# jinlong17/DA-Detect

Hardware: AMD Instinct MI355X
Metric: train images/sec, DA-Faster-RCNN R-50 Cityscapes->Foggy (higher is better)
Workload: dtype f32

## Files before the change

### da_detect_amd/_C.py

```python
import contextlib
import os
import ctypes
import time

import torch

from . import _lib
from . import amax as _amax
from ._lib import ConvDesc

CL = torch.channels_last

NMS_TIE_RULE = 0

PROFILER = None
_KNAME_CACHE = {}


class KernelProfiler(object):

    def __init__(self, pool=0, only=None):
        self.only = only
        self._pool = []
        for _ in range(pool):
# ... 216 lines not shown
                "%s must be a tensor on the HIP device: the da_detect_amd operators have no CPU path" % name)
        if t.dtype != dtype:
            raise _lib.DadetError("%s must be %s, got %s" % (name, dtype, t.dtype))
    det_box, gt_box, gt_area, gt_crowd = det_box.contiguous(), gt_box.contiguous(), gt_area.contiguous(), gt_crowd.contiguous()
    n_det, n_gt = int(det_box.shape[0]), int(gt_box.shape[0])
    if det_box.numel() != 4 * n_det or gt_box.numel() != 4 * n_gt or gt_area.numel() != n_gt or gt_crowd.numel() != n_gt:
        raise _lib.DadetError("coco_match: boxes must be [n, 4], gt_area and gt_crowd [n_gt]")
    d_host, nd = _int_table(det_off)
    g_host, ng = _int_table(gt_off)
    if nd != ng or nd < 1:
        raise _lib.DadetError("coco_match: the offset tables need pairs + 1 entries each, got %d and %d" % (nd, ng))
    pairs = nd - 1
    thr_host, T = _f64_table(iou_thr)
    rng_host, A2 = _f64_table([v for lo_hi in area_rng for v in lo_hi])
    A = A2 // 2
    dev = det_box.device
    nbytes = ctypes.c_size_t(0)
    _lib.call("dadet_coco_match_workspace_bytes", d_host, g_host, pairs, n_det, n_gt, T, A, ctypes.byref(nbytes))
    ws = _workspace(nbytes.value, dev)
    matched = torch.empty((T, A, n_det), dtype=torch.uint8, device=dev)
    ignored = torch.empty((T, A, n_det), dtype=torch.uint8, device=dev)
    npig = torch.empty((pairs, A), dtype=torch.int32, device=dev)
    _lib.call("dadet_coco_match", _p(det_box), _p(gt_box), _p(gt_area), _p(gt_crowd), d_host, g_host, pairs, n_det, n_gt,
              thr_host, T, rng_host, A, _p(ws), ctypes.c_size_t(ws.numel()), _p(matched), _p(ignored), _p(npig), _stream())
    return matched, ignored, npig


def nms(dets, scores, threshold):
    if dets.numel() == 0:
        return torch.empty(0, dtype=torch.int64, device=dets.device)
    keep, count = nms_with_count(dets, scores, threshold)
    return keep[: int(count.item())]


def roi_align_forward(input, rois, spatial_scale, pooled_height, pooled_width, sampling_ratio, bin_stride=1):
    _dev(input, "input"), _dev(rois, "rois")
    B, C, H, W = input.shape
    R = rois.shape[0]
    x = _nhwc(input)
    rois = rois.contiguous()
    if bin_stride != 1:
        s = int(bin_stride)
        out = torch.empty((R, C, -(-pooled_height // s), -(-pooled_width // s)), dtype=torch.float32,
                          device=input.device, memory_format=CL)
        ws = _roi_workspace(B, H, W, R, input.device) if ROI_ALIGN_WORKSPACE else None
        _lib.call("dadet_roi_align_forward_sub", _p(x), _p(rois), _p(out), B, C, H, W, R, pooled_height, pooled_width,
                  float(spatial_scale), int(sampling_ratio), s, _p(ws) if ws is not None else None,
                  ctypes.c_size_t(ws.numel() if ws is not None else 0), _stream())
        return _amax.carry(out, input)
    out = torch.empty((R, C, pooled_height, pooled_width), dtype=torch.float32, device=input.device,
                      memory_format=CL)
    if ROI_ALIGN_WORKSPACE:
        ws = _roi_workspace(B, H, W, R, input.device)
        _lib.call("dadet_roi_align_forward_ws", _p(x), _p(rois), _p(out), B, C, H, W, R, pooled_height, pooled_width,
                  float(spatial_scale), int(sampling_ratio), _p(ws), ctypes.c_size_t(ws.numel()), _stream())
    else:
        _lib.call("dadet_roi_align_forward", _p(x), _p(rois), _p(out), B, C, H, W, R, pooled_height,
                  pooled_width, float(spatial_scale), int(sampling_ratio), _stream())
    return _amax.carry(out, input)


ROI_ALIGN_WORKSPACE = True


def _roi_workspace(B, H, W, R, device):
    nbytes = ctypes.c_size_t(0)
    _lib.call("dadet_roi_align_workspace_bytes", B, H, W, R, ctypes.byref(nbytes))
    return _workspace(nbytes.value, device)


def roi_align_backward(grad, rois, spatial_scale, pooled_height, pooled_width, batch_size, channels,
                       height, width, sampling_ratio, atomic=False, bin_stride=1, live_images=None):
    _dev(grad, "grad"), _dev(rois, "rois")
    g = _nhwc(grad)
    rois = rois.contiguous()
    gin = torch.empty((batch_size, channels, height, width), dtype=torch.float32, device=grad.device,
                      memory_format=CL)
    B = batch_size
    if live_images is not None and 0 < live_images < batch_size and not atomic and rois.shape[0] > 0:
        B = int(live_images)
        gin[B:].zero_()
    if bin_stride != 1:
        if atomic:
            raise ValueError("roi_align_backward: bin_stride needs the gather form")
        _lib.call("dadet_roi_align_backward_sub", _p(g), _p(rois), _p(gin), B, channels, height, width,
                  rois.shape[0], pooled_height, pooled_width, float(spatial_scale), int(sampling_ratio),
                  int(bin_stride), _stream())
        return gin
    batch_size = B
    if atomic:
        gin.zero_()
    _lib.call("dadet_roi_align_backward_atomic" if atomic else "dadet_roi_align_backward", _p(g), _p(rois),
              _p(gin), batch_size, channels, height, width, rois.shape[0], pooled_height, pooled_width,
              float(spatial_scale), int(sampling_ratio), _stream())
    return gin


def roi_align_forward_level(input, rois, levels, level, out, spatial_scale, pooled_height, pooled_width, sampling_ratio):
    _dev(input, "input"), _dev(rois, "rois")
    assert levels.is_cuda and levels.dtype == torch.int64 and levels.is_contiguous() and levels.numel() == rois.shape[0]
    assert out.is_contiguous(memory_format=CL) and out.shape[0] == rois.shape[0]
    B, C, H, W = input.shape
    x = _nhwc(input)
    rois = rois.contiguous()
    ws = _roi_workspace(B, H, W, rois.shape[0], input.device)
    _lib.call("dadet_roi_align_forward_level", _p(x), _p(rois), _p(levels), int(level), _p(out), B, C, H, W, rois.shape[0],
              pooled_height, pooled_width, float(spatial_scale), int(sampling_ratio), _p(ws), ctypes.c_size_t(ws.numel()),
              _stream())
    return out


def roi_align_backward_level(grad, rois, levels, level, spatial_scale, pooled_height, pooled_width, batch_size, channels,
                             height, width, sampling_ratio):
    _dev(grad, "grad"), _dev(rois, "rois")
    assert levels.is_cuda and levels.dtype == torch.int64 and levels.is_contiguous() and levels.numel() == rois.shape[0]
    g = _nhwc(grad)
    gin = torch.empty((batch_size, channels, height, width), dtype=torch.float32, device=grad.device, memory_format=CL)
    _lib.call("dadet_roi_align_backward_level", _p(g), _p(rois.contiguous()), _p(levels), int(level), _p(gin), batch_size,
              channels, height, width, rois.shape[0], pooled_height, pooled_width, float(spatial_scale), int(sampling_ratio),
              _stream())
    return gin


def sigmoid_focalloss_forward(logits, targets, num_classes, gamma, alpha):
    _dev(logits, "logits")
    logits = logits.contiguous()
    targets = targets.contiguous().to(torch.int32)
    out = torch.empty_like(logits)
    _lib.call("dadet_sigmoid_focal_loss_forward", _p(logits), _p(targets), _p(out), logits.shape[0],
              int(num_classes), float(gamma), float(alpha), _stream())
    return out


def sigmoid_focalloss_backward(logits, targets, d_losses, num_classes, gamma, alpha):
    _dev(logits, "logits")
    logits = logits.contiguous()
    targets = targets.contiguous().to(torch.int32)
    d_losses = d_losses.contiguous()
    out = torch.empty_like(logits)
    _lib.call("dadet_sigmoid_focal_loss_backward", _p(logits), _p(targets), _p(d_losses), _p(out),
              logits.shape[0], int(num_classes), float(gamma), float(alpha), _stream())
    return out


def _desc(N, H, W, Cin, Cout, KH, KW, stride, pad, Ho, Wo, OutH=None, OutW=None, os=1, relu_mode=0):
    return ConvDesc(N, H, W, Cin, Cout, KH, KW, stride, pad, Ho, Wo, Ho if OutH is None else OutH,
                    Wo if OutW is None else OutW, os, relu_mode)


def conv_out_size(H, W, KH, KW, stride, pad):
    return (H + 2 * pad - KH) // stride + 1, (W + 2 * pad - KW) // stride + 1


def conv_forward(x, w, scale=None, bias=None, addend=None, mask_ref=None, stride=1, pad=0, relu_mode=0,
                 out=None, out_spatial_stride=1, out_hw=None, out_size=None):
    _dev(x, "x"), _dev(w, "w")
    N, Cin, H, W = x.shape
    Cout, Cin_w, KH, KW = w.shape
    assert Cin == Cin_w, "conv_forward: channel mismatch %d vs %d" % (Cin, Cin_w)
    x = _nhwc(x)
    w = _nhwc(w)
    Ho, Wo = out_size if out_size is not None else conv_out_size(H, W, KH, KW, stride, pad)
    if out_spatial_stride > 1:
        OutH, OutW = out_hw
        if out is None:
            out = torch.empty((N, Cout, OutH, OutW), dtype=torch.float32, device=x.device,
                              memory_format=CL).zero_()
    else:
        OutH, OutW = Ho, Wo
        if out is None:
            out = torch.empty((N, Cout, Ho, Wo), dtype=torch.float32, device=x.device, memory_format=CL)
    if addend is not None:
        addend = _nhwc(addend) if addend is not out else addend
    if mask_ref is not None:
        mask_ref = _nhwc(mask_ref)
    d = _desc(N, H, W, Cin, Cout, KH, KW, stride, pad, Ho, Wo, OutH, OutW, out_spatial_stride, relu_mode)
    ax = aw = None
    if _mode4():
        ax, aw = _amax.ptr(x), _weight_amax(w)
    if PROFILER is not None:
        key = (N * Ho * Wo, Cout, Cin * KH * KW, KH, pad, out_spatial_stride)
        kname = _KNAME_CACHE.get(key)
        if kname is None:
            kname = _plan_name("dadet_conv_forward_plan", d)
            _KNAME_CACHE[key] = kname
        if getattr(PROFILER, "detail", False):
            side = x.is_cuda and torch.cuda.current_stream(x.device) != torch.cuda.default_stream(x.device)
            kname = "%s|M=%d N=%d K=%d k%dx%d s%d%s%s" % (kname, N * Ho * Wo, Cout, Cin * KH * KW, KH, KW, stride,
                                                          " +add" if addend is not None else "", " [side]" if side else "")
        x_read = N * Ho * Wo * Cin if (KH == 1 and KW == 1 and stride > 1) else x.numel()
        with PROFILER.span(kname,
                           2.0 * N * Ho * Wo * Cout * Cin * KH * KW,
                           4.0 * (x_read + w.numel() + out.numel() + (addend.numel() if addend is not None else 0)
                                  + (mask_ref.numel() if mask_ref is not None else 0))):
            _conv_forward_call(d, x, w, scale, bias, addend, mask_ref, out, ax, aw)
        return out
    _conv_forward_call(d, x, w, scale, bias, addend, mask_ref, out, ax, aw)
    return out


def _conv_forward_call(d, x, w, scale, bias, addend, mask_ref, out, ax, aw):
    if ax is None:
        _lib.call("dadet_conv_forward", ctypes.byref(d), _p(x), _p(w), _p(scale), _p(bias), _p(addend),
                  _p(mask_ref), _p(out), _stream())
        return
    slot = _amax.new_slot(out.device)
    _lib.call("dadet_conv_forward_scaled", ctypes.byref(d), _p(x), _p(w), _p(scale), _p(bias), _p(addend),
              _p(mask_ref), _p(out), ax, aw, ctypes.c_void_p(slot[0]), _stream())
    _amax.attach(out, slot)


def _transpose_now(w, scale, wt):
    Cout, Cin, KH, KW = w.shape
    cout_pad = wt.shape[1]
    _lib.call("dadet_conv_weight_transpose_padded", _p(w), _p(scale), _p(wt), Cout, KH, KW, Cin, cout_pad, _stream())
    return wt


class _TransposeCache(object):

    def __init__(self):
        self.entries = {}
        self.epoch = 0
        self.batched_epoch = -1
        self.table = None
        self.ready = None
        self.enabled = True
        self._from_bump = False
        self._trained_only = False

    def bump(self, device=None, trained_only=False):
        self.epoch += 1
        self._trained_only = bool(trained_only)
        if self.enabled and device is not None and self.entries:
            self._from_bump = True
            try:
                self._refresh_all(device)
            finally:
                self._from_bump = False
        elif device is not None and _mode4():
            _amax.WEIGHTS.refresh(device, self.epoch, trained_only=self._trained_only)
        self._trained_only = False

    def _single(self, e, w, scale):
        _transpose_now(w, scale, e["wt"])
        _amax.WEIGHTS.invalidate(e["wt"])
        e["epoch"] = self.epoch
        if w.is_cuda:
            st = torch.cuda.current_stream(w.device)
            e["ev"] = (st, st.record_event())
        return e["wt"]

    def get(self, w, scale, cout_pad=0):
        Cout, Cin, KH, KW = w.shape
        key = (w.data_ptr(), Cout, Cin, KH, KW, scale.data_ptr() if scale is not None else 0, w.device.index, cout_pad)
        e = self.entries.get(key)
        if e is None:
            wt = torch.empty((Cin, max(Cout, cout_pad), KH, KW), dtype=torch.float32, device=w.device, memory_format=CL)
            wt._dadet_persistent = True
            e = self.entries[key] = dict(w=w, scale=scale, wt=wt, version=w._version, epoch=self.epoch, used=self.epoch,
                                         ev=None)
            self.table = None
            return self._single(e, w, scale)
        e["used"] = self.epoch
        if e["version"] != w._version:
            e["w"], e["version"] = w, w._version
            return self._single(e, w, scale)
        if e["epoch"] != self.epoch:
            if self.batched_epoch != self.epoch:
                self._refresh_all(w.device)
            if e["epoch"] != self.epoch:
                return self._single(e, w, scale)
        src = e["ev"] if e["ev"] is not None else self.ready
        if src is not None and w.is_cuda and torch.cuda.current_stream(w.device) != src[0]:
            torch.cuda.current_stream(w.device).wait_event(src[1])
        return e["wt"]

    def _refresh_all(self, device):
        for k in [k for k, e in self.entries.items() if e["used"] < self.epoch - 2]:
            del self.entries[k]
        live = [(k, e) for k, e in self.entries.items() if k[6] == device.index and e["version"] == e["w"]._version]
        if not live:
            self.batched_epoch = self.epoch
            return
        if self.table is None or self.table[3] != [k for k, _ in live]:
            arr = (_lib.TransposeItem * len(live))()
            blocks = 0
            for i, (k, e) in enumerate(live):
                _, Cout, Cin, KH, KW, _, _, cout_pad = k
                it = arr[i]
                it.w, it.scale, it.wt = e["w"].data_ptr(), (e["scale"].data_ptr() if e["scale"] is not None else None), \
                    e["wt"].data_ptr()
                it.Cout, it.KH, it.KW, it.Cin = Cout, KH, KW, Cin
                it.cout_pad = cout_pad
                it.blocks_ci, it.blocks_co = (Cin + 31) // 32, (max(Cout, cout_pad) + 31) // 32
                it.first_block = blocks
                blocks += it.blocks_ci * it.blocks_co * KH * KW
            host = torch.frombuffer(bytearray(bytes(arr)), dtype=torch.uint8).clone()
            self.table = (host.to(device), len(live), blocks, [k for k, _ in live])
        dev_t, n, blocks, _ = self.table
        _lib.call("dadet_conv_weight_transpose_batch", _p(dev_t), n, blocks, _stream())
        for _, e in live:
            e["epoch"] = self.epoch
            e["ev"] = None
        self.batched_epoch = self.epoch
        if _mode4():
            _amax.WEIGHTS.refresh(device, self.epoch, sync=not self._from_bump,
                                  trained_only=self._from_bump and self._trained_only)
        if device.type == "cuda":
            st = torch.cuda.current_stream(device)
            self.ready = (st, st.record_event())


_TRANSPOSES = _TransposeCache()


def weight_epoch():
    return _TRANSPOSES.epoch


def bump_weight_epoch(device=None, trained_only=False):
    _TRANSPOSES.bump(device, trained_only)


def conv_weight_transpose(w, scale=None, cout_pad=0):
    _dev(w, "w")
    Cout, Cin, KH, KW = w.shape
    cout_pad = cout_pad if cout_pad > Cout else 0
    w = _nhwc(w)
    base = w._base if w._base is not None else w
    if _TRANSPOSES.enabled and base.is_leaf and base.requires_grad:
        return _TRANSPOSES.get(w, scale, cout_pad)
    wt = torch.empty((Cin, max(Cout, cout_pad), KH, KW), dtype=torch.float32, device=w.device, memory_format=CL)
    return _transpose_now(w, scale, wt)


class WgradBatch(list):
    """weight gradients whose reduction pass over the split partial results is still to come
    (conv_wgrad(..., pending=batch) ... conv_wgrad_reduce_batch(batch)); keeps their workspaces alive until then"""


def _plan_name(query, d, *args):
    info = _lib.ConvPlanInfo()
    _lib.call(query, ctypes.byref(d), *(args + (ctypes.byref(info),)))
    return info.name.decode()


def _wgrad_kname(d, gy_ld):
    return _plan_name("dadet_conv_wgrad_plan", d, int(gy_ld))


def conv_wgrad_reduce_batch(batch):
    if not batch:
        return
    arr = (_lib.WgradPending * len(batch))(*[item[0] for item in batch])
    _lib.call("dadet_conv_wgrad_reduce_batch", arr, len(batch), _stream())
    del batch[:]


WGRAD_GROUP_MAX = 4


def conv_wgrad_group(requests, pending):
    n = len(requests)
    if not (1 <= n <= WGRAD_GROUP_MAX) or not _mode4() or pending is None:
        return False
    descs = (_lib.ConvDesc * n)()
    xs, gys = [], []
    for i, r in enumerate(requests):
        x, gy = _nhwc(_dev(r["x"], "x")), _nhwc(_dev(r["gy"], "gy"))
        N, Cin, H, W = x.shape
        Cout, Cin_w, KH, KW = r["weight_shape"]
        if Cin != Cin_w or gy.shape[1] != Cout or r["dw"] is None:
            return False
        descs[i] = _desc(N, H, W, Cin, Cout, KH, KW, r.get("stride", 1), r.get("pad", 0), gy.shape[2], gy.shape[3])
        xs.append(x)
        gys.append(gy)
    splits = (ctypes.c_int * n)()
    nbytes = (ctypes.c_size_t * n)()
    kind = _lib.load().dadet_conv_wgrad_group_plan(descs, n, splits, nbytes)
    if not kind:
        return False
    wss = [torch.empty(max(int(b), 16), dtype=torch.uint8, device=xs[0].device) for b in nbytes]
    vp = ctypes.c_void_p * n

    def ptrs(ts):
        return vp(*[(t.data_ptr() if t is not None else None) for t in ts])

    items = (_lib.WgradPending * n)()
    ax = vp(*[_amax.ptr(t).value for t in xs])
    ag = vp(*[_amax.ptr(t).value for t in gys])
    acc = (ctypes.c_int * n)(*[1 if r.get("accumulate", False) else 0 for r in requests])
    sizes = (ctypes.c_size_t * n)(*[w.numel() for w in wss])

    def launch():
        _lib.call("dadet_conv_wgrad_group", descs, n, ptrs(xs), ptrs(gys), ptrs([r.get("out_scale") for r in requests]),
                  ptrs([r["dw"] for r in requests]), acc, ptrs(wss), sizes, items, ax, ag, _stream())

    if PROFILER is not None:
        flops = sum(2.0 * d.N * d.Ho * d.Wo * d.Cout * d.Cin * d.KH * d.KW for d in descs)
        nbytes_alg = sum(4.0 * (x.numel() + g.numel() + r["dw"].numel()) for x, g, r in zip(xs, gys, requests))
        kname = "conv_wgrad_big_group_kernel" if kind == 256 else "conv_wgrad_split_group_kernel"
        if getattr(PROFILER, "detail", False):
            kname += "|" + " + ".join("M=%d N=%d K=%d k%dx%d s%d" % (d.N * d.Ho * d.Wo, d.Cout, d.Cin * d.KH * d.KW, d.KH,
                                                                     d.KW, d.stride) for d in descs)
        with PROFILER.span(kname, flops, nbytes_alg):
            launch()
    else:
        launch()
    for i, r in enumerate(requests):
        if items[i].splits > 1:
            it = _lib.WgradPending()
            ctypes.memmove(ctypes.byref(it), ctypes.byref(items[i]), ctypes.sizeof(it))
            pending.append((it, wss[i], r["dw"], r.get("out_scale")))
    return True


def conv_wgrad(x, gy, weight_shape, stride=1, pad=0, out_scale=None, dw=None, accumulate=False, pending=None):
    _dev(x, "x"), _dev(gy, "gy")
    N, Cin, H, W = x.shape
    Cout, Cin_w, KH, KW = weight_shape
    assert Cin == Cin_w
    x = _nhwc(x)
    gy = _nhwc(gy)
    Ho, Wo = gy.shape[2], gy.shape[3]
    gy_ld = gy.shape[1]
    if gy_ld != Cout and pending is None:
        own = WgradBatch()
        dw = conv_wgrad(x, gy, weight_shape, stride, pad, out_scale, dw, accumulate, pending=own)
        conv_wgrad_reduce_batch(own)
        return dw
    if dw is None:
        dw = torch.empty((Cout, Cin, KH, KW), dtype=torch.float32, device=x.device, memory_format=CL)
        accumulate = False
    d = _desc(N, H, W, Cin, Cout, KH, KW, stride, pad, Ho, Wo)
    nbytes = ctypes.c_size_t(0)
    _lib.call("dadet_conv_wgrad_workspace_bytes", ctypes.byref(d), ctypes.byref(nbytes))
    m4 = _mode4()
    if m4:
        ax, ag = _amax.ptr(x), _amax.ptr(gy)
    if pending is not None:
        ws = torch.empty(max(nbytes.value, 16), dtype=torch.uint8, device=x.device)
        item = _lib.WgradPending()

        def launch():
            if m4:
                _lib.call("dadet_conv_wgrad_scaled", ctypes.byref(d), _p(x), _p(gy), gy_ld, _p(out_scale), _p(dw),
                          1 if accumulate else 0, _p(ws), ctypes.c_size_t(ws.numel()), ctypes.byref(item), ax, ag,
                          _stream())
                return
            _lib.call("dadet_conv_wgrad_partials_ld", ctypes.byref(d), _p(x), _p(gy), gy_ld, _p(out_scale), _p(dw),
                      1 if accumulate else 0, _p(ws), ctypes.c_size_t(ws.numel()), ctypes.byref(item), _stream())

        if PROFILER is not None:
            kname = _wgrad_kname(d, gy_ld)
            if getattr(PROFILER, "detail", False):
                kname = "%s|M=%d N=%d K=%d k%dx%d s%d" % (kname, N * Ho * Wo, Cout, Cin * KH * KW, KH, KW, stride)
            with PROFILER.span(kname, 2.0 * N * Ho * Wo * Cout * Cin * KH * KW,
                               4.0 * (x.numel() + gy.numel() + dw.numel())):
                launch()
        else:
            launch()
        if item.splits > 1:
            pending.append((item, ws, dw, out_scale))
        return dw
    ws = _workspace(nbytes.value, x.device)
    if PROFILER is not None:
        kname = _wgrad_kname(d, gy_ld)
        if getattr(PROFILER, "detail", False):
            kname = "%s|M=%d N=%d K=%d k%dx%d s%d" % (kname, N * Ho * Wo, Cout, Cin * KH * KW, KH, KW, stride)
        with PROFILER.span(kname,
                           2.0 * N * Ho * Wo * Cout * Cin * KH * KW,
                           4.0 * (x.numel() + gy.numel() + dw.numel())):
            _wgrad_call(d, x, gy, gy_ld, out_scale, dw, accumulate, ws, ax if m4 else None, ag if m4 else None)
        return dw
    _wgrad_call(d, x, gy, gy_ld, out_scale, dw, accumulate, ws, ax if m4 else None, ag if m4 else None)
    return dw


def _wgrad_call(d, x, gy, gy_ld, out_scale, dw, accumulate, ws, ax, ag):
    if ax is not None:
        _lib.call("dadet_conv_wgrad_scaled", ctypes.byref(d), _p(x), _p(gy), gy_ld, _p(out_scale), _p(dw),
                  1 if accumulate else 0, _p(ws), ctypes.c_size_t(ws.numel()), None, ax, ag, _stream())
        return
    _lib.call("dadet_conv_wgrad", ctypes.byref(d), _p(x), _p(gy), _p(out_scale), _p(dw),
              1 if accumulate else 0, _p(ws), ctypes.c_size_t(ws.numel()), _stream())


def relu_bn_backward(g, y=None, scale=None, want_unscaled=False):
    _dev(g, "g")
    g = _nhwc(g) if g.dim() == 4 else g.contiguous()
    C = g.shape[1]
    rows = g.numel() // C
    yy = None
    if y is not None:
        yy = _nhwc(y) if y.dim() == 4 else y.contiguous()
    g_out = torch.empty_like(g) if want_unscaled else None
    g_scaled = torch.empty_like(g)
    if not _mode4():
        _lib.call("dadet_relu_bn_backward", _p(g), _p(yy), _p(scale), _p(g_out), _p(g_scaled), rows, C, _stream())
        return g_out, g_scaled
    so = ss = None
    if g_out is not None and _amax.slot_of(_amax.carry(g_out, g)) is None:
        so = _amax.new_slot(g.device)
    if scale is not None or _amax.slot_of(_amax.carry(g_scaled, g)) is None:
        ss = _amax.new_slot(g.device)
    _lib.call("dadet_relu_bn_backward_m", _p(g), _p(yy), _p(scale), _p(g_out), _p(g_scaled), rows, C,
              ctypes.c_void_p(so[0]) if so else None, ctypes.c_void_p(ss[0]) if ss else None, _stream())
    if so:
        _amax.attach(g_out, so)
    if ss:
        _amax.attach(g_scaled, ss)
    return g_out, g_scaled


def colsum(g, out=None, accumulate=False, cols=None):
    _dev(g, "g")
    g = _nhwc(g) if g.dim() == 4 else g.contiguous()
    ld = g.shape[1]
    C = ld if cols is None else int(cols)
    rows = g.numel() // ld
    if out is None:
        out = torch.empty(C, dtype=torch.float32, device=g.device)
        accumulate = False
    assert out.numel() == C and out.is_contiguous() and out.dtype == torch.float32
    nbytes = ctypes.c_size_t(0)
    _lib.call("dadet_colsum_workspace_bytes", rows, C, ctypes.byref(nbytes))
    ws = _workspace(nbytes.value, g.device)
    _lib.call("dadet_colsum_ld", _p(g), ld, _p(out), rows, C, 1 if accumulate else 0, _p(ws), ctypes.c_size_t(ws.numel()),
              _stream())
    return out


def channel_affine(x, scale, bias, relu=False):
    _dev(x, "x")
    x = _nhwc(x)
    C = x.shape[1]
    y = torch.empty_like(x)
    _lib.call("dadet_channel_affine", _p(x), _p(scale), _p(bias), _p(y), x.numel() // C, C,
              1 if relu else 0, _stream())
    return y


def maxpool3x3s2(x):
    _dev(x, "x")
    x = _nhwc(x)
    N, C, H, W = x.shape
    Ho, Wo = (H + 2 - 3) // 2 + 1, (W + 2 - 3) // 2 + 1
    y = torch.empty((N, C, Ho, Wo), dtype=torch.float32, device=x.device, memory_format=CL)
    _lib.call("dadet_maxpool3x3s2_forward", _p(x), _p(y), N, H, W, C, Ho, Wo, _stream())
    return _amax.carry(y, x)


def maxpool3x3s2_relu_backward(y, gp, scale=None):
    _dev(y, "y"), _dev(gp, "gp")
    y, gp = _nhwc(y), _nhwc(gp)
    N, C, H, W = y.shape
    Ho, Wo = (H + 2 - 3) // 2 + 1, (W + 2 - 3) // 2 + 1
    assert tuple(gp.shape) == (N, C, Ho, Wo), "maxpool3x3s2_relu_backward: gp %s for y %s" % (tuple(gp.shape), tuple(y.shape))
    g = torch.empty((N, C, H, W), dtype=torch.float32, device=y.device, memory_format=CL)
    slot = _amax.new_slot(y.device) if _mode4() else None
    _lib.call("dadet_maxpool3x3s2_relu_backward", _p(y), _p(gp), _p(scale), _p(g), N, H, W, C, Ho, Wo,
              ctypes.c_void_p(slot[0]) if slot else None, _stream())
    if slot:
        _amax.attach(g, slot)
    return g


def avgpool_forward(x):
    _dev(x, "x")
    x = _nhwc(x)
    R, C, h, w = x.shape
    y = torch.empty((R, C), dtype=torch.float32, device=x.device)
    _lib.call("dadet_avgpool_forward", _p(x), _p(y), R, h * w, C, _stream())
    return _amax.carry(y, x)


def avgpool_backward(gy, h, w):
    _dev(gy, "gy")
    gy = gy.contiguous()
    R, C = gy.shape
    gx = torch.empty((R, C, h, w), dtype=torch.float32, device=gy.device, memory_format=CL)
    _lib.call("dadet_avgpool_backward", _p(gy), _p(gx), R, h * w, C, _stream())
    return _amax.carry(gx, gy)


def nchw3_to_nhwc4(x):
    _dev(x, "x")
    x = x.contiguous()
    N, C, H, W = x.shape
    assert C == 3
    y = torch.empty((N, 4, H, W), dtype=torch.float32, device=x.device, memory_format=CL)
    _lib.call("dadet_nchw3_to_nhwc4", _p(x), _p(y), N, H, W, _stream())
    if _mode4():
        _amax.ptr(x)
        _amax.carry(y, x)
    return y


def two_image_ends(r_cst, n_src):
    return min(max(int(n_src), 0), int(r_cst)), int(r_cst)


def da_ins_tail_forward(h, w3, b3, labels, means, r_bce, r_cst, n_src):
    return da_ins_tail_forward_n(h, w3, b3, labels, means, r_bce, r_cst, two_image_ends(r_cst, n_src))


def da_ins_tail_backward(h, w3, logits, labels, means, coef, inv_keep, r_bce, r_cst, n_src):
    return da_ins_tail_backward_n(h, w3, logits, labels, means, coef, inv_keep, r_bce, r_cst, two_image_ends(r_cst, n_src))


def _row_ends(row_end):
    ends = [int(e) for e in row_end]
    return (ctypes.c_int * len(ends))(*ends), len(ends)


def da_ins_tail_forward_n(h, w3, b3, labels, means, r_bce, r_cst, row_end):
    _dev(h, "h")
    rows, C = h.shape
    assert rows == r_bce + r_cst
    L = int(means.shape[0]) if means is not None else 0
    ends, n_img = _row_ends(row_end)
    assert means is None or means.shape[1] == n_img
    logits = torch.empty(rows, dtype=torch.float32, device=h.device)
    sums = torch.zeros(2, dtype=torch.float32, device=h.device)
    _lib.call("dadet_da_ins_tail_forward_n", _p(h), _p(w3), _p(b3), _p(labels), _p(means), _p(logits), _p(sums),
              int(r_bce), int(r_cst), ends, n_img, L, C, _stream())
    return logits, sums


def da_ins_tail_backward_n(h, w3, logits, labels, means, coef, inv_keep, r_bce, r_cst, row_end):
    rows, C = h.shape
    L = int(means.shape[0]) if means is not None else 0
    ends, n_img = _row_ends(row_end)
    assert means is None or means.shape[1] == n_img
    g_z = torch.empty_like(h)
    acc = torch.zeros(C + 1 + n_img * L, dtype=torch.float32, device=h.device)
    g_w3, g_b3 = acc[:C], acc[C:C + 1]
    g_means = acc[C + 1:].view(L, n_img) if L else None
    _lib.call("dadet_da_ins_tail_backward_n", _p(h), _p(w3), _p(logits), _p(labels), _p(means), _p(coef), float(inv_keep),
              _p(g_z), _p(g_w3), _p(g_b3), _p(g_means), int(r_bce), int(r_cst), ends, n_img, L, C, _stream())
    return g_z, g_w3, g_b3, g_means


def da_ins_dropout_rows(h1, masks):
    P = masks.shape[0]
    out = torch.empty((P * h1.shape[0], h1.shape[1]), dtype=torch.float32, device=h1.device)
    _lib.call("dadet_da_ins_dropout_rows", _p(h1), _p(masks), _p(out), ctypes.c_int64(h1.numel()), int(P), _stream())
    return out


def da_ins_merge(g, masks, h1, grl, need_x=True):
    P = masks.shape[0]
    g_w = torch.empty_like(h1)
    g_x = torch.empty_like(h1) if need_x else None
    _lib.call("dadet_da_ins_merge", _p(g), _p(masks), _p(h1), _p(grl), _p(g_w), _p(g_x), ctypes.c_int64(h1.numel()),
              int(P), _stream())
    return g_w, g_x


# ... 614 lines not shown
```

### da_detect_amd/_lib.py

```python
import ctypes
import os
from ctypes import POINTER, c_char_p, c_float, c_int, c_int64, c_size_t, c_uint64, c_void_p

_HERE = os.path.dirname(os.path.abspath(__file__))
LIB_PATH = os.environ.get("DADET_LIB") or os.path.join(_HERE, "libdadet_hip.so")
_lib = None
DEFAULT_GEMM_MODE = "4"


class ConvDesc(ctypes.Structure):

    _fields_ = [(n, c_int) for n in (
        "N", "H", "W", "Cin", "Cout", "KH", "KW", "stride", "pad", "Ho", "Wo", "OutH", "OutW",
        "out_spatial_stride", "relu_mode")]


class ConvPlanInfo(ctypes.Structure):

    _fields_ = [(n, c_int) for n in (
        "family", "variant", "tiles_m", "tiles_n", "ksplit", "splits", "rows_per_split", "sk_dp_tiles", "sk_tiles", "sk_units",
        "sk_iters", "sk_max_parts", "big_splits", "big_body", "launches", "grid", "needs_counters")] + [
        ("workspace_bytes", c_size_t), ("name", ctypes.c_char * 64)]


class WgradPending(ctypes.Structure):

    _fields_ = [("partials", c_void_p), ("out_scale", c_void_p), ("dw", c_void_p), ("count", ctypes.c_longlong),
                ("K", c_int), ("splits", c_int), ("accumulate", c_int)]


class TransposeItem(ctypes.Structure):
    _fields_ = [("w", c_void_p), ("scale", c_void_p), ("wt", c_void_p), ("Cout", c_int), ("KH", c_int), ("KW", c_int),
                ("Cin", c_int), ("first_block", c_int), ("blocks_ci", c_int), ("blocks_co", c_int), ("cout_pad", c_int)]


class AmaxItem(ctypes.Structure):

    _fields_ = [("x", c_void_p), ("slot", c_void_p), ("n", ctypes.c_longlong), ("first_block", c_int), ("blocks", c_int)]


class MergeEntry(ctypes.Structure):

    _fields_ = [("boxes", c_void_p), ("scores", c_void_p), ("keep", c_void_p), ("count", c_void_p), ("boxes_out", c_void_p),
                ("scores_out", c_void_p), ("n", c_int), ("cap", c_int)]


class TopkRow(ctypes.Structure):

    _fields_ = [("scores", c_void_p), ("out_scores", c_void_p), ("out_idx", c_void_p), ("n", c_int), ("k", c_int)]


class SgdEntry(ctypes.Structure):

    _fields_ = [("p", c_void_p), ("g", c_void_p), ("buf", c_void_p), ("numel", c_int64),
                ("lr", c_float), ("weight_decay", c_float)]


_P = c_void_p
_SIGNATURES = {
    "dadet_version": [],
    "dadet_device_info": [POINTER(c_int), POINTER(c_int), POINTER(c_size_t), c_char_p, c_int],
    "dadet_nms_workspace_bytes": [c_int, POINTER(c_size_t)],
    "dadet_nms": [_P, _P, c_int, c_float, c_int, c_int, _P, c_size_t, _P, _P, _P],
    "dadet_nms_batch_workspace_bytes": [c_int, c_int, POINTER(c_size_t)],
    "dadet_nms_batch": [_P, POINTER(c_int), c_int, c_int, c_float, c_int, c_int, _P, c_size_t, _P, _P, _P],
    "dadet_detect_post_workspace_bytes": [POINTER(c_int), c_int, c_int, POINTER(c_size_t)],
    "dadet_detect_post": [_P, _P, POINTER(c_int), c_int, c_int, c_float, c_float, c_int, c_int, c_int, _P, c_size_t, _P, _P, _P,
                          _P, _P],
    "dadet_coco_match_workspace_bytes": [POINTER(c_int), POINTER(c_int), c_int, c_int, c_int, c_int, c_int, POINTER(c_size_t)],
    "dadet_coco_match": [_P, _P, _P, _P, POINTER(c_int), POINTER(c_int), c_int, c_int, c_int, POINTER(ctypes.c_double), c_int,
                         POINTER(ctypes.c_double), c_int, _P, c_size_t, _P, _P, _P, _P],
    "dadet_roi_align_forward": [_P, _P, _P, c_int, c_int, c_int, c_int, c_int, c_int, c_int, c_float, c_int, _P],
    "dadet_roi_align_backward": [_P, _P, _P, c_int, c_int, c_int, c_int, c_int, c_int, c_int, c_float, c_int, _P],
    "dadet_roi_align_workspace_bytes": [c_int, c_int, c_int, c_int, POINTER(c_size_t)],
    "dadet_roi_align_forward_ws": [_P, _P, _P, c_int, c_int, c_int, c_int, c_int, c_int, c_int, c_float, c_int, _P, c_size_t, _P],
    "dadet_roi_align_backward_atomic": [_P, _P, _P, c_int, c_int, c_int, c_int, c_int, c_int, c_int, c_float, c_int, _P],
    "dadet_roi_align_forward_sub": [_P, _P, _P, c_int, c_int, c_int, c_int, c_int, c_int, c_int, c_float, c_int, c_int,
                                    _P, c_size_t, _P],
    "dadet_roi_align_forward_level": [_P, _P, _P, c_int, _P, c_int, c_int, c_int, c_int, c_int, c_int, c_int, c_float, c_int, _P,
                                      c_size_t, _P],
    "dadet_roi_align_backward_level": [_P, _P, _P, c_int, _P, c_int, c_int, c_int, c_int, c_int, c_int, c_int, c_float, c_int,
                                       _P],
    "dadet_roi_align_backward_sub": [_P, _P, _P, c_int, c_int, c_int, c_int, c_int, c_int, c_int, c_float, c_int, c_int,
                                     _P],
    "dadet_sigmoid_focal_loss_forward": [_P, _P, _P, c_int, c_int, c_float, c_float, _P],
    "dadet_sigmoid_focal_loss_backward": [_P, _P, _P, _P, c_int, c_int, c_float, c_float, _P],
    "dadet_conv_forward": [POINTER(ConvDesc), _P, _P, _P, _P, _P, _P, _P, _P],
    "dadet_conv_forward_scaled": [POINTER(ConvDesc), _P, _P, _P, _P, _P, _P, _P, _P, _P, _P, _P],
    "dadet_conv_wgrad_scaled": [POINTER(ConvDesc), _P, _P, c_int, _P, _P, c_int, _P, c_size_t, POINTER(WgradPending), _P, _P,
                                _P],
    "dadet_amax": [_P, ctypes.c_longlong, _P, _P],
    "dadet_amax_batch": [_P, c_int, c_int, _P],
    "dadet_conv_forward_variant": [POINTER(ConvDesc)],
    "dadet_conv_forward_plan": [POINTER(ConvDesc), POINTER(ConvPlanInfo)],
    "dadet_conv_wgrad_plan": [POINTER(ConvDesc), c_int, POINTER(ConvPlanInfo)],
    "dadet_set_gemm_mode": [c_int],
    "dadet_get_gemm_mode": [],
    "dadet_conv_wgrad_variant": [POINTER(ConvDesc)],
    "dadet_conv_wgrad_group_plan": [POINTER(ConvDesc), c_int, POINTER(c_int), POINTER(c_size_t)],
    "dadet_conv_wgrad_group": [POINTER(ConvDesc), c_int, POINTER(c_void_p), POINTER(c_void_p), POINTER(c_void_p),
                               POINTER(c_void_p), POINTER(c_int), POINTER(c_void_p), POINTER(c_size_t),
                               POINTER(WgradPending), POINTER(c_void_p), POINTER(c_void_p), _P],
    "dadet_nonfinite_poll": [c_char_p, c_int],
    "dadet_set_big_gemm": [c_int],
    "dadet_get_big_gemm": [],
    "dadet_conv_wgrad_workspace_bytes": [POINTER(ConvDesc), POINTER(c_size_t)],
    "dadet_conv_wgrad": [POINTER(ConvDesc), _P, _P, _P, _P, c_int, _P, c_size_t, _P],
    "dadet_conv_wgrad_partials": [POINTER(ConvDesc), _P, _P, _P, _P, c_int, _P, c_size_t, POINTER(WgradPending), _P],
    "dadet_conv_wgrad_reduce_batch": [POINTER(WgradPending), c_int, _P],
    "dadet_conv_weight_transpose": [_P, _P, _P, c_int, c_int, c_int, c_int, _P],
    "dadet_conv_weight_transpose_padded": [_P, _P, _P, c_int, c_int, c_int, c_int, c_int, _P],
    "dadet_conv_wgrad_partials_ld": [POINTER(ConvDesc), _P, _P, c_int, _P, _P, c_int, _P, c_size_t, POINTER(WgradPending),
                                     _P],
    "dadet_conv_weight_transpose_batch": [_P, c_int, c_int, _P],
    "dadet_deform_sample_forward": [_P, _P, _P, _P] + [c_int] * 12 + [_P],
    "dadet_deform_sample_backward": [_P, _P, _P, _P, _P, _P, _P] + [c_int] * 12 + [_P],
    "dadet_deform_sample_forward_ld": [_P, _P, c_int, _P, c_int, c_int, _P] + [c_int] * 12 + [_P],
    "dadet_deform_sample_backward_ld": [_P, _P, c_int, _P, c_int, c_int, _P, _P, _P, c_int, _P, c_int] + [c_int] * 12
                                       + [_P, c_size_t, _P],
    "dadet_deform_sample_backward_ld_m": [_P, _P, c_int, _P, c_int, c_int, _P, _P, _P, c_int, _P, c_int] + [c_int] * 12
                                         + [_P, c_size_t, _P, ctypes.c_longlong, _P],
    "dadet_deform_sample_backward_workspace_bytes": [c_int, c_int, c_int, c_int, POINTER(c_size_t)],
    "dadet_image_resample_h": [_P, c_int, c_int, _P, _P, c_int, c_int, _P, _P],
    "dadet_image_resample_v_normalize": [_P, c_int, c_int, _P, _P, c_int, c_int, c_int, c_int, POINTER(c_float),
                                         POINTER(c_float), _P, c_int, _P],
    "dadet_rpn_loss": [_P, _P, _P, _P, c_int, _P, _P, c_int, c_float, _P, _P, _P, _P],
    "dadet_fpn_merge_levels": [POINTER(MergeEntry), c_int, _P],
    "dadet_rpn_loss_rows": [_P, _P, _P, _P, c_int, c_int, _P, c_int, c_float, _P, _P, c_int, _P, _P],
    "dadet_rpn_loss_rows_level": [_P, _P, _P, _P, c_int, c_int, _P, c_int, c_float, ctypes.c_longlong, ctypes.c_longlong,
                                  ctypes.c_longlong, c_int, _P, c_int, _P, _P, c_int, _P, _P],
    "dadet_gather_pixel_taps_level": [_P, _P, _P, c_int, c_int, c_int, c_int, c_int, c_int, c_int, c_int, c_int, _P, _P],
    "dadet_scatter_pixel_taps_add_level": [_P, _P, _P, c_int, c_int, c_int, c_int, c_int, c_int, c_int, c_int, c_int, _P,
                                           _P],
    "dadet_gather_pixel_taps": [_P, _P, c_int, c_int, c_int, c_int, c_int, c_int, c_int, c_int, _P, _P],
    "dadet_scatter_pixel_taps_add": [_P, _P, c_int, c_int, c_int, c_int, c_int, c_int, c_int, c_int, _P, _P],
    "dadet_fast_rcnn_loss": [_P, _P, c_int, c_int, _P, _P, c_int, _P, _P, _P, c_int, _P, _P, _P, _P],
    "dadet_fast_rcnn_loss_rows": [_P, _P, c_int, c_int, c_int, _P, _P, _P, _P, _P, _P],
    "dadet_sample_rois": [_P, _P, _P, c_int, c_int, c_int, c_uint64, c_int, _P, _P, _P, _P, _P, _P, _P, _P],
    "dadet_proposals_sample": [_P, _P, _P, _P, c_int, _P, c_int, _P, _P, c_int, c_float, c_float, c_float, c_float, c_float,
                               c_float, c_int, c_int, c_uint64, c_int, _P, _P, _P, _P, _P, _P, _P, _P, _P, _P, _P, _P],
    "dadet_sample_anchors": [_P, _P, c_int, c_int, c_int, c_uint64, c_int64, _P, _P, _P, _P, _P],
    "dadet_topk_sorted": [_P, c_int, c_int, c_int64, c_int, _P, _P, _P],
    "dadet_topk_sorted_rows_workspace_bytes": [c_int, c_int, POINTER(c_size_t)],
    "dadet_topk_sorted_rows": [POINTER(TopkRow), c_int, _P, c_size_t, _P],
    "dadet_rpn_anchor_targets": [_P, _P, c_int, _P, c_int, c_float, c_float, _P, _P, _P, _P],
    "dadet_box_match_encode": [_P, c_int, _P, _P, c_int, c_float, c_float, c_float, c_float, c_float, c_float, _P, _P,
                               _P, _P],
    "dadet_roi_pool_forward": [_P, _P, _P, _P, c_int, c_int, c_int, c_int, c_int, c_int, c_int, c_float, _P],
    "dadet_roi_pool_backward": [_P, _P, _P, _P, c_int, c_int, c_int, c_int, c_int, c_int, c_int, _P],
    "dadet_deform_psroi_pool_forward": [_P, _P, _P, _P, _P, c_int, c_int, c_int, c_int, c_int, c_int, c_float,
                                        c_int, c_int, c_int, c_int, c_int, c_float, c_int, _P],
    "dadet_deform_psroi_pool_backward": [_P, _P, _P, _P, _P, _P, _P, c_int, c_int, c_int, c_int, c_int, c_int,
                                         c_float, c_int, c_int, c_int, c_int, c_int, c_float, c_int, _P],
    "dadet_relu_bn_backward": [_P, _P, _P, _P, _P, c_int64, c_int, _P],
    "dadet_relu_bn_backward_m": [_P, _P, _P, _P, _P, c_int64, c_int, _P, _P, _P],
    "dadet_colsum_workspace_bytes": [c_int64, c_int, POINTER(c_size_t)],
    "dadet_colsum": [_P, _P, c_int64, c_int, _P, c_size_t, _P],
    "dadet_colsum_ld": [_P, c_int, _P, c_int64, c_int, c_int, _P, c_size_t, _P],
    "dadet_channel_affine": [_P, _P, _P, _P, c_int64, c_int, c_int, _P],
    "dadet_maxpool3x3s2_forward": [_P, _P, c_int, c_int, c_int, c_int, c_int, c_int, _P],
    "dadet_maxpool3x3s2_relu_backward": [_P, _P, _P, _P, c_int, c_int, c_int, c_int, c_int, c_int, _P, _P],
    "dadet_avgpool_forward": [_P, _P, c_int, c_int, c_int, _P],
    "dadet_avgpool_backward": [_P, _P, c_int, c_int, c_int, _P],
    "dadet_nchw3_to_nhwc4": [_P, _P, c_int, c_int, c_int, _P],
    "dadet_rpn_decode_clip": [_P, _P, _P, c_int, c_float, c_float, c_float, c_float, c_float, c_float, c_float, _P, _P],
    "dadet_da_img_head_loss_forward": [_P, _P, _P, _P, _P, _P, c_int, c_int, c_int, _P],
    "dadet_da_img_head_loss_backward": [_P, _P, _P, _P, _P, _P, _P, _P, _P, c_int, c_int, c_int, _P],
    "dadet_da_img_head_loss_backward_g": [_P, _P, _P, _P, _P, _P, _P, c_float, c_float, _P, _P, _P, _P, c_int, c_int, c_int,
                                          _P],
    "dadet_da_img_head_loss_backward_gm": [_P, _P, _P, _P, _P, _P, _P, c_float, c_float, _P, _P, _P, _P, c_int, c_int, c_int,
                                          _P, _P, _P],
    "dadet_da_ins_tail_forward": [_P, _P, _P, _P, _P, _P, _P, c_int, c_int, c_int, c_int, c_int, _P],
    "dadet_da_ins_tail_backward": [_P, _P, _P, _P, _P, _P, c_float, _P, _P, _P, _P, c_int, c_int, c_int, c_int, c_int, _P],
    "dadet_da_ins_tail_forward_n": [_P, _P, _P, _P, _P, _P, _P, c_int, c_int, POINTER(c_int), c_int, c_int, c_int, _P],
    "dadet_da_ins_tail_backward_n": [_P, _P, _P, _P, _P, _P, c_float, _P, _P, _P, _P, c_int, c_int, POINTER(c_int), c_int,
                                     c_int, c_int, _P],
    "dadet_da_ins_dropout_rows": [_P, _P, _P, c_int64, c_int, _P],
    "dadet_da_ins_merge": [_P, _P, _P, _P, _P, _P, c_int64, c_int, _P],
    "dadet_triplet_w_forward": [_P, _P, _P, c_int, c_int, c_int, c_float, c_float, _P, _P, _P],
    "dadet_triplet_w_backward": [_P, _P, _P, _P, _P, c_int, c_int, c_int, c_float, c_float, _P, _P, _P, _P],
    "dadet_sgd_step": [_P, c_int, c_int64, c_float, c_int, c_float, _P],
}
_RESTYPES = {"dadet_last_error": c_char_p}
EXPORTED_SYMBOLS = sorted(list(_SIGNATURES) + ["dadet_last_error"])


class DadetError(RuntimeError):
    pass


def load():
    global _lib
    if _lib is not None:
        return _lib
    if not os.path.exists(LIB_PATH):
        raise DadetError(
            "libdadet_hip.so is not built (%s). Run `python -c 'import __graft_entry__ as g; g.build()'` "
            "or `make -C da_detect_amd/csrc`. There is no CPU fallback for the product path." % LIB_PATH)
    import torch

    lib = ctypes.CDLL(LIB_PATH)
    for name, argtypes in _SIGNATURES.items():
        fn = getattr(lib, name)
        fn.argtypes = argtypes
        fn.restype = c_int
    lib.dadet_last_error.argtypes = []
    lib.dadet_last_error.restype = c_char_p
    _lib = lib
    mode = int(os.environ.get("DADET_GEMM_MODE", DEFAULT_GEMM_MODE))
    if lib.dadet_set_gemm_mode(mode) != 0:
        raise DadetError("DADET_GEMM_MODE=%d is not a valid contraction mode (0, 2, 3 or 4)" % mode)
    return lib


def check(rc, what=""):
    if rc != 0:
        msg = load().dadet_last_error()
        raise DadetError("%s failed (status %d): %s" % (what or "dadet call", rc, (msg or b"").decode()))


def call(name, *args):
    check(getattr(load(), name)(*args), name)
```

### da_detect_amd/csrc/conv_common.h

```cpp
#pragma once
#include <cstdlib>
#include "common.h"
#include "conv_plan.h"

namespace dadet {

typedef float f32x16 __attribute__((ext_vector_type(16)));
typedef unsigned int u32x4 __attribute__((ext_vector_type(4)));

constexpr unsigned kOOB = 0xFFFFFFF0u;
__device__ inline __amdgpu_buffer_rsrc_t make_rsrc(const void* p, unsigned bytes) {
  return __builtin_amdgcn_make_buffer_rsrc(const_cast<void*>(p), 0, (int)bytes, 0x00020000);
}
__device__ inline float4 buf_load4(__amdgpu_buffer_rsrc_t r, unsigned byte_off) {
  return __builtin_bit_cast(float4, __builtin_amdgcn_raw_buffer_load_b128(r, (int)byte_off, 0, 0));
}
__device__ inline float buf_load1(__amdgpu_buffer_rsrc_t r, unsigned byte_off) {
  return __builtin_bit_cast(float, __builtin_amdgcn_raw_buffer_load_b32(r, (int)byte_off, 0, 0));
}
__device__ inline void buf_store1(__amdgpu_buffer_rsrc_t r, unsigned byte_off, float v) {
  __builtin_amdgcn_raw_buffer_store_b32(__builtin_bit_cast(unsigned, v), r, (int)byte_off, 0, 0);
}

__device__ inline void buf_store4_wt(__amdgpu_buffer_rsrc_t r, unsigned byte_off, float4 v) {
  __builtin_amdgcn_raw_buffer_store_b128(__builtin_bit_cast(u32x4, v), r, (int)byte_off, 0, 16);
}
__device__ inline float4 buf_load4_sc1(__amdgpu_buffer_rsrc_t r, unsigned byte_off) {
  return __builtin_bit_cast(float4, __builtin_amdgcn_raw_buffer_load_b128(r, (int)byte_off, 0, 16));
}

typedef __bf16 bf16x8 __attribute__((ext_vector_type(8)));


__device__ inline unsigned pack_bf16(float lo, float hi) {
  unsigned r;
  asm("v_cvt_pk_bf16_f32 %0, %1, %2" : "=v"(r) : "v"(lo), "v"(hi));
  return r;
}
__device__ inline float lo_as_float(unsigned p) { return __builtin_bit_cast(float, p << 16); }
__device__ inline float hi_as_float(unsigned p) { return __builtin_bit_cast(float, p & 0xFFFF0000u); }

template <int TERMS>
__device__ inline void split4(const float4 v, uint2 (&out)[TERMS]) {
  float a = v.x, b = v.y, c = v.z, d = v.w;
#pragma unroll
  for (int t = 0; t < TERMS; ++t) {
    const unsigned p0 = pack_bf16(a, b), p1 = pack_bf16(c, d);
    out[t] = make_uint2(p0, p1);
    if (t + 1 < TERMS) {
      a -= lo_as_float(p0); b -= hi_as_float(p0);
      c -= lo_as_float(p1); d -= hi_as_float(p1);
    }
  }
}

typedef _Float16 f16x8 __attribute__((ext_vector_type(8)));
typedef _Float16 f16x2 __attribute__((ext_vector_type(2)));

__device__ inline int fmt4_exp(const float amax) {
  const int be = (int)((__builtin_bit_cast(unsigned, amax) >> 23) & 0xffu);
  if (be == 0 || be == 255) return 0;
  int e = 14 - (be - 127);
  return e > 126 ? 126 : (e < -126 ? -126 : e);
}
__device__ inline float pow2f(const int e) { return __builtin_bit_cast(float, (unsigned)(e + 127) << 23); }

__device__ inline unsigned pack_f16(float lo, float hi) {
  unsigned r;
  asm("v_cvt_pk_f16_f32 %0, %1, %2" : "=v"(r) : "v"(lo), "v"(hi));
  return r;
}
__device__ inline float resid_lo(float x, float s, unsigned h) {
  float r;
  asm("v_fma_mix_f32 %0, %1, %2, -%3 op_sel_hi:[0,0,1]" : "=v"(r) : "v"(x), "v"(s), "v"(h));
  return r;
}
__device__ inline float resid_hi(float x, float s, unsigned h) {
  float r;
  asm("v_fma_mix_f32 %0, %1, %2, -%3 op_sel:[0,0,1] op_sel_hi:[0,0,1]" : "=v"(r) : "v"(x), "v"(s), "v"(h));
  return r;
}
__device__ inline void split4h(const float4 v, const float s, uint2 (&out)[2]) {
  const unsigned h0 = pack_f16(v.x * s, v.y * s), h1 = pack_f16(v.z * s, v.w * s);
  out[0] = make_uint2(h0, h1);
  out[1] = make_uint2(pack_f16(resid_lo(v.x, s, h0), resid_hi(v.y, s, h0)),
                      pack_f16(resid_lo(v.z, s, h1), resid_hi(v.w, s, h1)));
}

template <int FMT> struct Fmt { static constexpr int terms = FMT == 3 ? 3 : 2; static constexpr bool f16 = FMT == 4; };

template <bool F16>
__device__ __forceinline__ f32x16 mfma_32x32x16(const bf16x8 a, const bf16x8 b, const f32x16 c) {
  if constexpr (F16)
    return __builtin_amdgcn_mfma_f32_32x32x16_f16(__builtin_bit_cast(f16x8, a), __builtin_bit_cast(f16x8, b), c, 0, 0, 0);
  else
    return __builtin_amdgcn_mfma_f32_32x32x16_bf16(a, b, c, 0, 0, 0);
}

constexpr int kAmaxStride = DADET_AMAX_STRIDE;
__device__ inline float amax_read(const float* slot) {
  float m = slot[0];
#pragma unroll
  for (int s = 1; s < 8; ++s) m = fmaxf(m, slot[s * kAmaxStride]);
  return m;
}
__device__ inline void amax_publish(unsigned* slot, float m) {
  __shared__ unsigned s_amax;
  unsigned* shard = slot + (size_t)((blockIdx.x + blockIdx.y) & 7) * kAmaxStride;
  unsigned seen = 0;
  if (threadIdx.x == 0) {
    s_amax = 0;
    seen = __hip_atomic_load(shard, __ATOMIC_RELAXED, __HIP_MEMORY_SCOPE_AGENT);
  }
#pragma unroll
  for (int o = 32; o; o >>= 1) m = fmaxf(m, __shfl_xor(m, o));
  __syncthreads();
  if ((threadIdx.x & 63) == 0) atomicMax(&s_amax, __builtin_bit_cast(unsigned, m));
  __syncthreads();
  if (threadIdx.x == 0) {
    const unsigned b = s_amax;
    if (b > seen) __hip_atomic_fetch_max(shard, b, __ATOMIC_RELAXED, __HIP_MEMORY_SCOPE_AGENT);
  }
}

template <int TM, int TN>
__device__ __forceinline__ void nf_check(const f32x16 (&acc)[TM][TN], unsigned* flag, const unsigned id) {
  if (!flag) return;
  bool bad = false;
#pragma unroll
  for (int i = 0; i < TM; ++i)
#pragma unroll
    for (int j = 0; j < TN; ++j)
#pragma unroll
      for (int e = 0; e < 16; ++e)
        bad |= (__builtin_bit_cast(unsigned, acc[i][j][e]) & 0x7f800000u) == 0x7f800000u;
  if (__builtin_amdgcn_ballot_w64(bad) != 0 && (threadIdx.x & 63) == 0) {
    atomicCAS(flag, 0u, id + 1u);
    atomicAdd(flag + 1, 1u);
  }
}
unsigned nf_next_launch(const char* kind, int M, int N, int K, int KH);
unsigned* nf_flag_ptr();

constexpr int PLANE_STRIDE = 40;
constexpr int EPI_STRIDE = 40;

constexpr int BK = plan::kBK;
constexpr int LDS_STRIDE = 36;

struct ConvArgs {
  const float* x;
  const float* w;
  const float* scale;
  const float* bias;
  const float* addend;
  const float* mask_ref;
  float* y;
  int N, H, W, Cin, Cout, KH, KW, stride, pad, Ho, Wo, OutH, OutW, os, relu_mode;
  int M, K;
  int tiles_m, tiles_n;
  unsigned x_bytes, w_bytes, y_bytes;
  int ablate;
  int ws_panel0;
  int epi_v4;
  int ksplit;
  unsigned split_stride;
  int sk_dp_tiles, sk_tiles, sk_units, sk_iters, sk_max_parts;
  float* sk_ws;
  int* sk_counters;
  int big_splits;
  int big_asym;
  int big_body;
  unsigned* nf_flag;
  unsigned launch_id;
  const float* amax_x;
  const float* amax_w;
  unsigned* amax_y;
};

struct WgradArgs {
  const float* x;
  const float* gy;
  const float* out_scale;
  float* out;
  int N, H, W, Cin, Cout, KH, KW, stride, pad, Ho, Wo;
  int M, K;
  int gy_ld;
  int tiles_co, tiles_kc, splits, rows_per_split;
  int direct;
  int accumulate;
  unsigned x_bytes, gy_bytes;
  const float* amax_x;
  const float* amax_gy;
  unsigned* nf_flag;
  unsigned launch_id;
};

constexpr int kWgradGroupMax = plan::kGroupMax;
struct WgradGroup {
  WgradArgs a[kWgradGroupMax];
  int first[kWgradGroupMax + 1];
  int n;
};

static_assert(plan::kCUs == kNumCU, "the plan layer's CU count");

int gemm_mode();

int launch_fwd_exact(ConvArgs& a, const plan::FwdPlan& p, hipStream_t st);
int launch_wgrad_exact(WgradArgs& a, hipStream_t st);
int launch_fwd_split(ConvArgs& a, const plan::FwdPlan& p, int fmt, hipStream_t st);
int launch_fwd_split_sk(ConvArgs& a, int fmt, hipStream_t st);
int launch_wgrad_split(WgradArgs& a, bool small_map, int fmt, hipStream_t st);
int launch_wgrad_split_group(const WgradArgs* a, int n, bool small_map, hipStream_t st);
int launch_fwd_ws(ConvArgs& a, const plan::FwdPlan& p, int fmt, hipStream_t st);
int launch_fwd_big(ConvArgs& a, const plan::FwdPlan& p, hipStream_t st);
int launch_wgrad_big(WgradArgs& a, hipStream_t st);
int launch_wgrad_big_group(const WgradArgs* a, int n, hipStream_t st);

void* stream_scratch(hipStream_t st, size_t bytes);
int* stream_counters(hipStream_t st);
unsigned* stream_amax_slots(hipStream_t st);
hipError_t zero_slots(unsigned* first, int n, hipStream_t st);
int launch_amax(const float* x, int64_t n, unsigned* slot, hipStream_t st);
int launch_splitk_reduce(const float* partial, int splits, const ConvArgs& a, hipStream_t st);
int launch_wgrad_reduce(const float* partials, const float* out_scale, float* dw, int Cout, int K, int splits,
                        int accumulate, hipStream_t st);

}
```

### da_detect_amd/csrc/conv_dispatch.hip

```cpp
#include "conv_common.h"

namespace dadet {

static int g_gemm_mode = 4;
static int g_big_mode = plan::big_gemm_default();
int gemm_mode() { return g_gemm_mode; }

static int conv_desc_check(const dadet_conv_desc* d, const char* who) {
  DADET_REQUIRE(d, "%s: null descriptor", who);
  DADET_REQUIRE(d->N >= 0 && d->H > 0 && d->W > 0 && d->Cin > 0 && d->Cout > 0 && d->KH > 0 && d->KW > 0 &&
                    d->stride > 0 && d->pad >= 0 && d->Ho > 0 && d->Wo > 0,
                "%s: bad dims", who);
  DADET_REQUIRE(d->Cin % 4 == 0, "%s: Cin=%d must be a multiple of 4 (pad the channel axis)", who, d->Cin);
  DADET_REQUIRE((int64_t)d->N * d->H * d->W * d->Cin < (1LL << 31) &&
                    (int64_t)d->N * d->Ho * d->Wo < (1LL << 31),
                "%s: tensor too large for 32-bit pixel indexing", who);
  return DADET_OK;
}

static int extents_check(uint64_t a, uint64_t b, uint64_t c, const char* who) {
  DADET_REQUIRE(a < 0xFFFFFFF0ull && b < 0xFFFFFFF0ull && c < 0xFFFFFFF0ull,
                "%s: tensors of 4 GB or more are not addressable through one buffer descriptor", who);
  return DADET_OK;
}

static bool al16(const void* p) { return (reinterpret_cast<uintptr_t>(p) & 15) == 0; }

static void fill_conv_args(const dadet_conv_desc* d, const plan::Gemm& g, const plan::FwdPlan& p, ConvArgs* a) {
  *a = ConvArgs();
  a->N = d->N; a->H = d->H; a->W = d->W; a->Cin = d->Cin; a->Cout = d->Cout; a->KH = d->KH; a->KW = d->KW;
  a->stride = d->stride; a->pad = d->pad; a->Ho = d->Ho; a->Wo = d->Wo; a->OutH = d->OutH; a->OutW = d->OutW;
  a->os = g.os; a->relu_mode = d->relu_mode;
  a->M = g.M; a->K = g.K;
  a->x_bytes = (unsigned)g.x_bytes; a->w_bytes = (unsigned)g.w_bytes; a->y_bytes = (unsigned)g.y_bytes;
  a->ablate = plan::ablate();
  a->epi_v4 = p.epi_v4;
  a->tiles_m = p.tiles_m; a->tiles_n = p.tiles_n;
  a->sk_dp_tiles = p.sk.dp_tiles; a->sk_tiles = p.sk.sk_tiles; a->sk_units = p.sk.units; a->sk_iters = p.sk.iters;
  a->sk_max_parts = p.sk.max_parts;
  a->big_splits = p.big_splits; a->big_body = p.big_body;
}

static void fill_wgrad_args(const dadet_conv_desc* d, int gy_ld, int tiles_co, int tiles_kc, int splits, int rows,
                            WgradArgs* a) {
  *a = WgradArgs();
  const plan::Gemm g = plan::gemm_of(d);
  a->gy_ld = gy_ld;
  a->N = d->N; a->H = d->H; a->W = d->W; a->Cin = d->Cin; a->Cout = d->Cout; a->KH = d->KH; a->KW = d->KW;
  a->stride = d->stride; a->pad = d->pad; a->Ho = d->Ho; a->Wo = d->Wo;
  a->M = g.M; a->K = g.K;
  a->x_bytes = (unsigned)g.x_bytes; a->gy_bytes = (unsigned)((uint64_t)g.M * gy_ld * 4);
  a->tiles_co = tiles_co; a->tiles_kc = tiles_kc; a->splits = splits; a->rows_per_split = rows;
}

static void fill_pending(dadet_wgrad_pending* p, const void* workspace, const float* out_scale, float* dw, int Cout, int K,
                         int splits, int accumulate) {
  p->partials = static_cast<const float*>(workspace);
  p->out_scale = out_scale;
  p->dw = dw;
  p->count = (long long)Cout * K;
  p->K = K;
  p->splits = splits;
  p->accumulate = accumulate;
}

static int conv_forward_impl(const dadet_conv_desc* d, const float* x, const float* w,
                             const float* scale, const float* bias, const float* addend,
                             const float* mask_ref, float* y, const float* amax_x, const float* amax_w,
                             float* amax_y, void* stream) {
  int rc = conv_desc_check(d, "conv_forward");
  if (rc) return rc;
  if (d->N == 0) return DADET_OK;
  DADET_REQUIRE(x && w && y && al16(x) && al16(w), "conv_forward: x / w must be non-null and 16-byte aligned");
  DADET_REQUIRE(d->relu_mode >= 0 && d->relu_mode <= 2, "conv_forward: relu_mode");
  DADET_REQUIRE(d->relu_mode != 2 || mask_ref, "conv_forward: relu_mode 2 needs mask_ref");
  const plan::Gemm g = plan::gemm_of(d);
  DADET_REQUIRE(g.os == 1 ? (d->OutH == d->Ho && d->OutW == d->Wo)
                          : ((d->Ho - 1) * g.os < d->OutH && (d->Wo - 1) * g.os < d->OutW),
                "conv_forward: OutH/OutW inconsistent with Ho/Wo and out_spatial_stride");
  rc = extents_check(g.x_bytes, g.w_bytes, g.y_bytes, "conv_forward");
  if (rc) return rc;
  const int mode = g_gemm_mode;
  const bool aligned16 = al16(y) && (!addend || al16(addend)) && (!mask_ref || al16(mask_ref)) && (!scale || al16(scale)) &&
                         (!bias || al16(bias));
  const plan::FwdPlan p = plan::plan_forward(d, aligned16, mode, g_big_mode);
  ConvArgs a;
  fill_conv_args(d, g, p, &a);
  a.x = x; a.w = w; a.scale = scale; a.bias = bias; a.addend = addend; a.mask_ref = mask_ref; a.y = y;
  hipStream_t st = as_stream(stream);
  if (mode == 4) {
    if (!amax_x || !amax_w) {
      unsigned* own = stream_amax_slots(st);
      if (!own) { set_error("conv_forward: could not allocate the operand-maximum slots"); return DADET_ELAUNCH; }
      if (zero_slots(own, 2, st) != hipSuccess) return check_launch("conv_forward(amax memset)");
      if (!amax_x) {
        rc = launch_amax(x, (int64_t)(g.x_bytes / 4), own, st);
        if (rc) return rc;
        amax_x = reinterpret_cast<const float*>(own);
      }
      if (!amax_w) {
        rc = launch_amax(w, (int64_t)(g.w_bytes / 4), own + 1, st);
        if (rc) return rc;
        amax_w = reinterpret_cast<const float*>(own + 1);
      }
    }
    a.amax_x = amax_x; a.amax_w = amax_w;
    a.amax_y = reinterpret_cast<unsigned*>(amax_y);
    a.nf_flag = nf_flag_ptr();
    a.launch_id = a.nf_flag ? nf_next_launch("conv_forward", a.M, a.Cout, a.K, a.KH) : 0;
  }
  float* ws = p.workspace_bytes ? static_cast<float*>(stream_scratch(st, p.workspace_bytes)) : nullptr;
  int* counters = p.counters ? stream_counters(st) : nullptr;
  if ((p.workspace_bytes && !ws) || (p.counters && !counters)) {
    set_error("conv_forward: could not allocate %zu bytes of %s scratch", p.workspace_bytes,
              p.family == plan::kFwdSplitSk ? "stream-K" : p.family == plan::kFwdSplitK ? "split-K" : "split-reduction");
    return DADET_ELAUNCH;
  }
  switch (p.family) {
    case plan::kFwdWs: return launch_fwd_ws(a, p, mode, st);
    case plan::kFwdBig256:
    case plan::kFwdBig128:
      a.sk_ws = ws;
      a.sk_counters = counters;
      return launch_fwd_big(a, p, st);
    case plan::kFwdSplitSk:
      a.sk_ws = ws;
      a.sk_counters = counters;
      return launch_fwd_split_sk(a, mode, st);
    case plan::kFwdSplitK: {
      ConvArgs part = a;
      part.scale = part.bias = part.addend = part.mask_ref = nullptr;
      part.amax_y = nullptr;
      part.relu_mode = 0;
      part.y = ws;
      part.ksplit = p.ksplit;
      part.split_stride = (unsigned)((size_t)a.M * a.Cout);
      rc = launch_fwd_split(part, p, mode, st);
      return rc ? rc : launch_splitk_reduce(ws, p.splits, a, st);
    }
    case plan::kFwdSplit: return launch_fwd_split(a, p, mode, st);
    default: return launch_fwd_exact(a, p, st);
  }
}

static int conv_wgrad_impl(const dadet_conv_desc* d, const float* x, const float* gy, const float* out_scale, float* dw,
                           int accumulate, void* workspace, size_t workspace_bytes, dadet_wgrad_pending* pending,
                           void* stream, int gy_ld = 0, const float* amax_x = nullptr, const float* amax_gy = nullptr) {
  if (pending) pending->splits = 0;
  int rc = conv_desc_check(d, "conv_wgrad");
  if (rc) return rc;
  DADET_REQUIRE(dw, "conv_wgrad: null dw");
  hipStream_t st = as_stream(stream);
  const int K = d->KH * d->KW * d->Cin;
  if (d->N == 0) {
    if (!accumulate) (void)hipMemsetAsync(dw, 0, sizeof(float) * (size_t)d->Cout * K, st);
    return check_launch("conv_wgrad(empty)");
  }
  DADET_REQUIRE(x && gy && al16(x) && al16(gy) && al16(dw), "conv_wgrad: pointers must be 16-byte aligned");
  if (gy_ld == 0) gy_ld = d->Cout;
  DADET_REQUIRE(gy_ld % 4 == 0 && gy_ld >= d->Cout && gy_ld - d->Cout < 4,
                "conv_wgrad: gy rows of %d floats for Cout=%d (need a multiple of 4, less than 4 above Cout)", gy_ld, d->Cout);
  DADET_REQUIRE(K % 4 == 0, "conv_wgrad: KH*KW*Cin=%d must be a multiple of 4", K);
  const plan::Gemm g = plan::gemm_of(d);
  const uint64_t gb = (uint64_t)g.M * gy_ld * 4;
  rc = extents_check(g.x_bytes, gb, 0, "conv_wgrad");
  if (rc) return rc;
  const int mode = g_gemm_mode;
  const plan::WgradPlan p = plan::plan_wgrad(d, gy_ld, mode, g_big_mode);
  WgradArgs a;
  fill_wgrad_args(d, gy_ld, p.tiles_co, p.tiles_kc, p.splits, p.rows_per_split, &a);
  a.x = x; a.gy = gy; a.out_scale = out_scale;
  a.accumulate = accumulate;
  if (mode == 4) {
    if (!amax_x || !amax_gy) {
      unsigned* own = stream_amax_slots(st);
      if (!own) { set_error("conv_wgrad: could not allocate the operand-maximum slots"); return DADET_ELAUNCH; }
      if (zero_slots(own + 2, 2, st) != hipSuccess) return check_launch("conv_wgrad(amax memset)");
      if (!amax_x) {
        rc = launch_amax(x, (int64_t)(g.x_bytes / 4), own + 2, st);
        if (rc) return rc;
        amax_x = reinterpret_cast<const float*>(own + 2);
      }
      if (!amax_gy) {
        rc = launch_amax(gy, (int64_t)(gb / 4), own + 3, st);
        if (rc) return rc;
        amax_gy = reinterpret_cast<const float*>(own + 3);
      }
    }
    a.amax_x = amax_x; a.amax_gy = amax_gy;
    a.nf_flag = nf_flag_ptr();
    a.launch_id = a.nf_flag ? nf_next_launch("conv_wgrad", a.M, a.Cout, a.K, a.KH) : 0;
  }
  if (p.splits == 1) {
    a.direct = 1;
    a.out = dw;
  } else {
    if (!workspace || workspace_bytes < p.workspace_bytes) {
      set_error("conv_wgrad: workspace %zu < required %zu", workspace_bytes, p.workspace_bytes);
      return DADET_EWORKSPACE;
    }
    a.direct = 0;
    a.out = static_cast<float*>(workspace);
  }
  switch (p.family) {
    case plan::kWgradBig: rc = launch_wgrad_big(a, st); break;
    case plan::kWgradExact: rc = launch_wgrad_exact(a, st); break;
    default: rc = launch_wgrad_split(a, p.family == plan::kWgradSplitSmallMap, mode, st);
  }
  if (rc || p.splits == 1) return rc;
  if (pending) {
    fill_pending(pending, workspace, out_scale, dw, d->Cout, K, p.splits, accumulate);
    return DADET_OK;
  }
  return launch_wgrad_reduce(static_cast<const float*>(workspace), out_scale, dw, d->Cout, K, p.splits, accumulate, st);
}

static bool group_descs_ok(const dadet_conv_desc* descs, int n) {
  if (n < 1 || n > kWgradGroupMax) return false;
  for (int i = 0; i < n; ++i)
    if (conv_desc_check(&descs[i], "conv_wgrad_group") || descs[i].N == 0) return false;
  return true;
}

}

using namespace dadet;

extern "C" int dadet_set_gemm_mode(int mode) {
  if (mode != 0 && mode != 2 && mode != 3 && mode != 4) {
    set_error("set_gemm_mode: mode must be 0, 2, 3 or 4");
    return DADET_EINVAL;
  }
  g_gemm_mode = mode;
  return DADET_OK;
}
extern "C" int dadet_get_gemm_mode(void) { return g_gemm_mode; }

extern "C" int dadet_set_big_gemm(int mode) {
  if (mode < 0 || mode > 2) {
    set_error("set_big_gemm: mode must be 0 (off), 1 (planned) or 2 (wherever applicable)");
    return DADET_EINVAL;
  }
  g_big_mode = mode;
  return DADET_OK;
}
extern "C" int dadet_get_big_gemm(void) { return g_big_mode; }

extern "C" int dadet_conv_forward(const dadet_conv_desc* d, const float* x, const float* w,
                                  const float* scale, const float* bias, const float* addend,
                                  const float* mask_ref, float* y, void* stream) {
  return conv_forward_impl(d, x, w, scale, bias, addend, mask_ref, y, nullptr, nullptr, nullptr, stream);
}

extern "C" int dadet_conv_forward_scaled(const dadet_conv_desc* d, const float* x, const float* w,
                                         const float* scale, const float* bias, const float* addend,
                                         const float* mask_ref, float* y, const float* amax_x, const float* amax_w,
                                         float* amax_y, void* stream) {
  return conv_forward_impl(d, x, w, scale, bias, addend, mask_ref, y, amax_x, amax_w, amax_y, stream);
}

extern "C" int dadet_conv_forward_plan(const dadet_conv_desc* d, dadet_conv_plan_info* out) {
  int rc = conv_desc_check(d, "conv_forward_plan");
  if (rc) return rc;
  DADET_REQUIRE(out, "conv_forward_plan: null out");
  const plan::Gemm g = plan::gemm_of(d);
  rc = extents_check(g.x_bytes, g.w_bytes, g.y_bytes, "conv_forward_plan");
  if (rc) return rc;
  const plan::FwdPlan p = plan::plan_forward(d, true, g_gemm_mode, g_big_mode);
  plan::fill_info(p, out);
  if (!p.epi_v4 && g.os == 1 && d->Cout % 4 == 0) {
    const plan::FwdPlan label = plan::plan_forward_epi(d, true, true, g_gemm_mode, g_big_mode);
    out->variant = label.variant;
    snprintf(out->name, sizeof(out->name), "%s", label.name);
  }
  return DADET_OK;
}

extern "C" int dadet_conv_forward_variant(const dadet_conv_desc* d) {
  if (!d) return -1;
  const int os = d->out_spatial_stride > 0 ? d->out_spatial_stride : 1;
  return plan::fwd_label(d, plan::gemm_of(d), os == 1 && d->Cout % 4 == 0, g_gemm_mode, g_big_mode);
}

extern "C" int dadet_conv_wgrad_plan(const dadet_conv_desc* d, int gy_ld, dadet_conv_plan_info* out) {
  int rc = conv_desc_check(d, "conv_wgrad_plan");
  if (rc) return rc;
  DADET_REQUIRE(out, "conv_wgrad_plan: null out");
  plan::fill_info(plan::plan_wgrad(d, gy_ld ? gy_ld : d->Cout, g_gemm_mode, g_big_mode), out);
  return DADET_OK;
}

extern "C" int dadet_conv_wgrad_variant(const dadet_conv_desc* d) {
  if (!d) return -1;
  return plan::plan_wgrad(d, d->Cout, g_gemm_mode, g_big_mode).family == plan::kWgradBig ? 1 : 0;
}

extern "C" int dadet_conv_wgrad_workspace_bytes(const dadet_conv_desc* d, size_t* bytes_out) {
  int rc = conv_desc_check(d, "conv_wgrad_workspace_bytes");
  if (rc) return rc;
  DADET_REQUIRE(bytes_out, "conv_wgrad_workspace_bytes: null out");
  if (d->N == 0) { *bytes_out = 0; return DADET_OK; }
  const plan::WgradPlan dense = plan::plan_wgrad(d, d->Cout, g_gemm_mode, g_big_mode);
  *bytes_out = dense.workspace_bytes;
  if (dense.family == plan::kWgradBig) {
    const size_t padded = plan::plan_wgrad(d, d->Cout + 4, g_gemm_mode, g_big_mode).workspace_bytes;
    if (padded > *bytes_out) *bytes_out = padded;
  }
  return DADET_OK;
}

extern "C" int dadet_conv_wgrad(const dadet_conv_desc* d, const float* x, const float* gy,
                                const float* out_scale, float* dw, int accumulate, void* workspace,
                                size_t workspace_bytes, void* stream) {
  return conv_wgrad_impl(d, x, gy, out_scale, dw, accumulate, workspace, workspace_bytes, nullptr, stream);
}

extern "C" int dadet_conv_wgrad_partials(const dadet_conv_desc* d, const float* x, const float* gy,
                                         const float* out_scale, float* dw, int accumulate, void* workspace,
                                         size_t workspace_bytes, dadet_wgrad_pending* pending_out, void* stream) {
  DADET_REQUIRE(pending_out, "conv_wgrad_partials: null pending_out");
  return conv_wgrad_impl(d, x, gy, out_scale, dw, accumulate, workspace, workspace_bytes, pending_out, stream);
}

extern "C" int dadet_conv_wgrad_partials_ld(const dadet_conv_desc* d, const float* x, const float* gy, int gy_ld,
                                            const float* out_scale, float* dw, int accumulate, void* workspace,
                                            size_t workspace_bytes, dadet_wgrad_pending* pending_out, void* stream) {
  DADET_REQUIRE(pending_out, "conv_wgrad_partials_ld: null pending_out");
  return conv_wgrad_impl(d, x, gy, out_scale, dw, accumulate, workspace, workspace_bytes, pending_out, stream, gy_ld);
}

extern "C" int dadet_conv_wgrad_scaled(const dadet_conv_desc* d, const float* x, const float* gy, int gy_ld,
                                       const float* out_scale, float* dw, int accumulate, void* workspace,
                                       size_t workspace_bytes, dadet_wgrad_pending* pending_out, const float* amax_x,
                                       const float* amax_gy, void* stream) {
  return conv_wgrad_impl(d, x, gy, out_scale, dw, accumulate, workspace, workspace_bytes, pending_out, stream, gy_ld,
                         amax_x, amax_gy);
}

extern "C" int dadet_conv_wgrad_group_plan(const dadet_conv_desc* descs, int n, int* splits_out, size_t* workspace_bytes_out) {
  DADET_REQUIRE(descs && n >= 1 && splits_out && workspace_bytes_out, "conv_wgrad_group_plan: bad arguments");
  if (!group_descs_ok(descs, n)) return 0;
  const plan::WgradGroupPlan p = plan::plan_wgrad_group(descs, n, g_gemm_mode, g_big_mode);
  for (int i = 0; i < n && p.kind; ++i) {
    splits_out[i] = p.splits[i];
    workspace_bytes_out[i] = p.workspace_bytes[i];
  }
  return p.kind;
}

extern "C" int dadet_conv_wgrad_group(const dadet_conv_desc* descs, int n, const float* const* x, const float* const* gy,
                                      const float* const* out_scale, float* const* dw, const int* accumulate,
                                      void* const* workspace, const size_t* workspace_bytes,
                                      dadet_wgrad_pending* pending_out, const float* const* amax_x,
                                      const float* const* amax_gy, void* stream) {
  DADET_REQUIRE(descs && n >= 1 && n <= kWgradGroupMax && x && gy && dw && accumulate && workspace && workspace_bytes &&
                    pending_out && amax_x && amax_gy, "conv_wgrad_group: bad arguments (1 - 4 problems, every array non-null)");
  DADET_REQUIRE(g_gemm_mode == 4, "conv_wgrad_group: contraction mode 4 only (mode %d is set)", g_gemm_mode);
  hipStream_t st = as_stream(stream);
  const plan::WgradGroupPlan p = group_descs_ok(descs, n) ? plan::plan_wgrad_group(descs, n, g_gemm_mode, g_big_mode)
                                                           : plan::WgradGroupPlan();
  DADET_REQUIRE(p.kind != 0, "conv_wgrad_group: these problems do not form a grouped launch (dadet_conv_wgrad_group_plan)");
  for (int i = 0; i < n; ++i) {
    DADET_REQUIRE(x[i] && gy[i] && dw[i] && amax_x[i] && amax_gy[i] && al16(x[i]) && al16(gy[i]) && al16(dw[i]),
                  "conv_wgrad_group: problem %d: null or misaligned pointer", i);
    for (int j = 0; j < i; ++j)
      DADET_REQUIRE(dw[i] != dw[j], "conv_wgrad_group: problems %d and %d write the same dw", j, i);
  }
  WgradArgs a[kWgradGroupMax];
  for (int i = 0; i < n; ++i) {
    const dadet_conv_desc* d = &descs[i];
    WgradArgs& w = a[i];
    fill_wgrad_args(d, d->Cout, p.tiles_co[i], p.tiles_kc[i], p.splits[i], p.rows, &w);
    w.x = x[i]; w.gy = gy[i]; w.out_scale = out_scale ? out_scale[i] : nullptr;
    w.accumulate = accumulate[i];
    w.amax_x = amax_x[i]; w.amax_gy = amax_gy[i];
    w.nf_flag = nf_flag_ptr();
    w.launch_id = w.nf_flag ? nf_next_launch("conv_wgrad_group", w.M, w.Cout, w.K, w.KH) : 0;
    pending_out[i].splits = 0;
    if (p.splits[i] == 1) {
      w.direct = 1;
      w.out = dw[i];
    } else {
      if (!workspace[i] || workspace_bytes[i] < p.workspace_bytes[i]) {
        set_error("conv_wgrad_group: problem %d: workspace %zu < required %zu", i, workspace_bytes[i], p.workspace_bytes[i]);
        return DADET_EWORKSPACE;
      }
      w.direct = 0;
      w.out = static_cast<float*>(workspace[i]);
    }
  }
  int rc = p.kind == 256 ? launch_wgrad_big_group(a, n, st) : launch_wgrad_split_group(a, n, p.small_map != 0, st);
  if (rc) return rc;
  for (int i = 0; i < n; ++i)
    if (p.splits[i] > 1)
      fill_pending(&pending_out[i], workspace[i], out_scale ? out_scale[i] : nullptr, dw[i], descs[i].Cout, a[i].K,
                   p.splits[i], accumulate[i]);
  return DADET_OK;
}
```

### da_detect_amd/csrc/conv_ws.hip

```cpp
#include "conv_common.h"
#include <stdlib.h>
#include <type_traits>

namespace dadet {

constexpr unsigned kOOBws = 0x80000000u;
constexpr int WS_ROWS = 256;

template <int N, int I = 0, class F>
__device__ __forceinline__ void ws_unroll(F&& f) {
  if constexpr (I < N) {
    f(std::integral_constant<int, I>{});
    ws_unroll<N, I + 1>(f);
  }
}

template <int K, int BN, int FMT, int EROWS = 32>
__global__ __launch_bounds__(512, 1) void conv1x1_ws_kernel(const ConvArgs a) {
  constexpr int T = Fmt<FMT>::terms;
  constexpr bool F16 = Fmt<FMT>::f16;
  constexpr int NB = BN / 32;
  constexpr int STRIDE = K + 8;
  constexpr int PLANE = BN * STRIDE;
  constexpr int CH = K / 32;
  constexpr int SUPER = CH < 4 ? 4 : CH;
  constexpr int SL = SUPER / CH;
  constexpr int EPB = 2;
  constexpr bool EARLY = NB == 2;

  extern __shared__ __attribute__((aligned(16))) char smem[];
  __bf16* Bs = reinterpret_cast<__bf16*>(smem);
  const int t = threadIdx.x;
  const int lane = t & 63, wave = t >> 6;
  float* tile = reinterpret_cast<float*>(smem + T * PLANE * 2) + wave * (EROWS * EPI_STRIDE);
  float* s_affine = reinterpret_cast<float*>(smem + T * PLANE * 2) + 8 * (EROWS * EPI_STRIDE);
  int ea = 0, eb = 0;
  if (F16) {
    ea = a.amax_x ? fmt4_exp(amax_read(a.amax_x)) : 0;
    eb = a.amax_w ? fmt4_exp(amax_read(a.amax_w)) : 0;
  }
  const float sa = pow2f(ea), sb = pow2f(eb);
  const float u1 = pow2f(-(ea + eb) / 2), u2 = pow2f(-(ea + eb) - (-(ea + eb)) / 2);
  float mx = 0.f;

  const int panels = a.tiles_n;
  const int G = (int)gridDim.x / panels;
  const int xcd = (int)blockIdx.x & 7, j = (int)blockIdx.x >> 3;
  const int panel = j % panels, group = (j / panels) * 8 + xcd;
  const int n0 = (a.ws_panel0 + panel) * BN;
  const int tiles = a.tiles_m;

  const __amdgpu_buffer_rsrc_t xr = make_rsrc(a.x, a.x_bytes);
  const __amdgpu_buffer_rsrc_t wr = make_rsrc(a.w, a.w_bytes);
  const int frow = lane & 31, fh = lane >> 5;
  const int HoWo = a.Ho * a.Wo;
  const bool dense = a.stride == 1;

  auto row_off = [&](int tile_idx) __attribute__((always_inline)) -> unsigned {
    const int m = tile_idx * WS_ROWS + wave * 32 + frow;
    if (tile_idx >= tiles || m >= a.M) return kOOBws;
    int pix = m;
    if (!dense) {
      const int img = m / HoWo;
      const int rem = m - img * HoWo;
      const int ho = rem / a.Wo;
      const int wo = rem - ho * a.Wo;
      pix = (img * a.H + ho * a.stride) * a.W + wo * a.stride;
    }
    return (unsigned)pix * (unsigned)(K * 4) + (unsigned)fh * 64u;
  };

  float4 raw[4][4];
  {
    constexpr int Q = K / 4;
    constexpr int PER = (BN * Q) / 512;
    float4 wv[PER];
#pragma unroll
    for (int i = 0; i < PER; ++i) {
      const int idx = t + i * 512;
      const int n = idx / Q, kq = idx - n * Q;
      wv[i] = buf_load4(wr, (n0 + n < a.Cout) ? (unsigned)(((n0 + n) * K + kq * 4) * 4) : kOOBws);
    }
#pragma unroll
    for (int i = 0; i < PER; ++i) {
      const int idx = t + i * 512;
      const int n = idx / Q, kq = idx - n * Q;
      uint2 p[T];
      if constexpr (F16) split4h(wv[i], sb, p);
      else split4<T>(wv[i], p);
#pragma unroll
      for (int pl = 0; pl < T; ++pl) *reinterpret_cast<uint2*>(Bs + pl * PLANE + n * STRIDE + kq * 4) = p[pl];
    }
  }
  if (t < BN) {
    const int n = n0 + t;
    s_affine[t] = (a.scale && n < a.Cout) ? a.scale[n] : 1.f;
    s_affine[BN + t] = (a.bias && n < a.Cout) ? a.bias[n] : 0.f;
  }
  __syncthreads();
#pragma unroll
  for (int q = 0; q < 4; ++q) {
    const unsigned o = row_off(group + (q / CH) * G);
#pragma unroll
    for (int v = 0; v < 4; ++v) raw[q][v] = buf_load4(xr, o + (unsigned)((q % CH) * 128 + v * 16));
  }
  __builtin_amdgcn_sched_barrier(0);

  f32x16 acc[NB];
#pragma unroll
  for (int nb = 0; nb < NB; ++nb)
#pragma unroll
    for (int e = 0; e < 16; ++e) acc[nb][e] = 0.f;

  auto split8 = [&](const float4 lo, const float4 hi, bf16x8 (&out)[T]) __attribute__((always_inline)) {
    uint2 pl[T], ph[T];
    if constexpr (F16) {
      split4h(lo, sa, pl);
      split4h(hi, sa, ph);
    } else {
      split4<T>(lo, pl);
      split4<T>(hi, ph);
    }
#pragma unroll
    for (int p = 0; p < T; ++p) out[p] = __builtin_bit_cast(bf16x8, make_uint4(pl[p].x, pl[p].y, ph[p].x, ph[p].y));
  };
  const __bf16* Bb = Bs + frow * STRIDE + fh * 16;
  bf16x8 pa[T];

  auto step = [&](auto Q, auto S, const unsigned (&ahead)[4]) __attribute__((always_inline)) {
    constexpr int q = decltype(Q)::value, sidx = decltype(S)::value;
    constexpr int c = q % CH, slot = q & 3;
    if (sidx == 1) {
      constexpr int qa = q + 4;
      const unsigned o = ahead[qa / CH];
#pragma unroll
      for (int v = 0; v < 4; ++v) raw[slot][v] = buf_load4(xr, o + (unsigned)((qa % CH) * 128 + v * 16));
    }
    bf16x8 fb[T][NB];
#pragma unroll
    for (int p = 0; p < T; ++p)
#pragma unroll
      for (int nb = 0; nb < NB; ++nb)
        fb[p][nb] = *reinterpret_cast<const bf16x8*>(Bb + p * PLANE + nb * 32 * STRIDE + c * 32 + sidx * 8);
    bf16x8 pn[T];
    if (sidx == 0) split8(raw[slot][2], raw[slot][3], pn);
    else split8(raw[(q + 1) & 3][0], raw[(q + 1) & 3][1], pn);
#pragma unroll
    for (int order = 2 * (T - 1); order >= 0; --order)
#pragma unroll
      for (int x = 0; x < T; ++x) {
        const int y = order - x;
        if (y < 0 || y >= T || x + y > T - 1) continue;
#pragma unroll
        for (int nb = 0; nb < NB; ++nb) acc[nb] = mfma_32x32x16<F16>(pa[x], fb[y][nb], acc[nb]);
      }
    {
      constexpr int kMfma = (T == 3 ? 6 : 3) * NB;
      constexpr int kValuPerMfma = (T == 3 ? 56 : 28) / kMfma + 1;
      if (sidx == 1) __builtin_amdgcn_sched_group_barrier(0x020, 4, 0);
      __builtin_amdgcn_sched_group_barrier(0x100, T * NB, 0);
#pragma unroll
      for (int m = 0; m < kMfma; ++m) {
        __builtin_amdgcn_sched_group_barrier(0x008, 1, 0);
        __builtin_amdgcn_sched_group_barrier(0x002, kValuPerMfma, 0);
      }
    }
#pragma unroll
    for (int p = 0; p < T; ++p) pa[p] = pn[p];
    __builtin_amdgcn_sched_barrier(0);
  };

  const __amdgpu_buffer_rsrc_t yr = make_rsrc(a.y, a.y_bytes);
  const __amdgpu_buffer_rsrc_t ar = make_rsrc(a.addend ? a.addend : a.y, a.addend ? a.y_bytes : 0u);
  const __amdgpu_buffer_rsrc_t mr = make_rsrc(a.mask_ref ? a.mask_ref : a.y, a.mask_ref ? a.y_bytes : 0u);
  const int col_in = lane & 31, row_hi = 4 * (lane >> 5);
  const int rrow = lane >> 3, c4 = (lane & 7) * 4;

  unsigned e_offs[EPB][4];
  float4 e_ad[EPB][4], e_mk[EPB][4];
  auto epi_issue = [&](int tile_idx, int nb0, unsigned (&offs)[EPB][4], float4 (&ad)[EPB][4], float4 (&mk)[EPB][4])
      __attribute__((always_inline)) {
    const int mbase = tile_idx * WS_ROWS + wave * 32;
#pragma unroll
    for (int e = 0; e < EPB; ++e) {
      const int n = n0 + (nb0 + e) * 32 + c4;
#pragma unroll
      for (int pass = 0; pass < 4; ++pass) {
        const int m = mbase + pass * 8 + rrow;
        offs[e][pass] = (n < a.Cout && tile_idx < tiles && m < a.M) ? ((unsigned)m * (unsigned)a.Cout + (unsigned)n) * 4u : kOOB;
      }
    }
    if (a.addend) {
#pragma unroll
      for (int e = 0; e < EPB; ++e)
#pragma unroll
        for (int pass = 0; pass < 4; ++pass) ad[e][pass] = buf_load4(ar, offs[e][pass]);
    }
    if (a.relu_mode == 2) {
#pragma unroll
      for (int e = 0; e < EPB; ++e)
#pragma unroll
        for (int pass = 0; pass < 4; ++pass) mk[e][pass] = buf_load4(mr, offs[e][pass]);
    }
  };
  auto epi_finish = [&](int nb0, const unsigned (&offs)[EPB][4], const float4 (&ad)[EPB][4], const float4 (&mk)[EPB][4])
      __attribute__((always_inline)) {
#pragma unroll
    for (int e = 0; e < EPB; ++e) {
      const float4 sc = *reinterpret_cast<const float4*>(s_affine + (nb0 + e) * 32 + c4);
      const float4 bi = *reinterpret_cast<const float4*>(s_affine + BN + (nb0 + e) * 32 + c4);
      constexpr int GH = EROWS / 8;
#pragma unroll
      for (int hh = 0; hh < 4 / GH; ++hh) {
#pragma unroll
      for (int g = hh * GH; g < (hh + 1) * GH; ++g)
#pragma unroll
        for (int q = 0; q < 4; ++q)
          tile[(q + 8 * (g - hh * GH) + row_hi) * EPI_STRIDE + col_in] =
              F16 ? acc[nb0 + e][g * 4 + q] * u1 * u2 : acc[nb0 + e][g * 4 + q];
      __builtin_amdgcn_s_waitcnt(0xc07f);
      __builtin_amdgcn_wave_barrier();
#pragma unroll
      for (int pass = hh * GH; pass < (hh + 1) * GH; ++pass) {
        const float4 v4 = *reinterpret_cast<const float4*>(tile + ((pass - hh * GH) * 8 + rrow) * EPI_STRIDE + c4);
        float v[4] = {v4.x, v4.y, v4.z, v4.w};
        const float s4[4] = {sc.x, sc.y, sc.z, sc.w}, b4[4] = {bi.x, bi.y, bi.z, bi.w};
        float adv[4] = {0.f, 0.f, 0.f, 0.f}, mkv[4] = {1.f, 1.f, 1.f, 1.f};
        if (a.addend) {
          const float4 q4 = ad[e][pass];
          adv[0] = q4.x; adv[1] = q4.y; adv[2] = q4.z; adv[3] = q4.w;
        }
        if (a.relu_mode == 2) {
          const float4 q4 = mk[e][pass];
          mkv[0] = q4.x; mkv[1] = q4.y; mkv[2] = q4.z; mkv[3] = q4.w;
        }
#pragma unroll
        for (int k = 0; k < 4; ++k) {
          float x = v[k];
          if (a.scale) x = x * s4[k];
          if (a.bias) x = x + b4[k];
          if (a.addend) x = x + adv[k];
          if (a.relu_mode == 1) x = fmaxf(x, 0.f);
          else if (a.relu_mode == 2) x = (mkv[k] > 0.f) ? x : 0.f;
          v[k] = x;
        }
        __builtin_amdgcn_raw_buffer_store_b128(__builtin_bit_cast(u32x4, make_float4(v[0], v[1], v[2], v[3])), yr,
                                               (int)offs[e][pass], 0, 0);
        if (F16 && a.amax_y && offs[e][pass] != kOOB)
          mx = fmaxf(fmaxf(mx, fmaxf(fabsf(v[0]), fabsf(v[1]))), fmaxf(fabsf(v[2]), fabsf(v[3])));
      }
      __builtin_amdgcn_wave_barrier();
      }
    }
  };
  auto epilogue = [&](int tile_idx) __attribute__((always_inline)) {
    if (F16 && a.nf_flag) {
      bool bad = false;
#pragma unroll
      for (int nb = 0; nb < NB; ++nb)
#pragma unroll
        for (int e = 0; e < 16; ++e) bad |= (__builtin_bit_cast(unsigned, acc[nb][e]) & 0x7f800000u) == 0x7f800000u;
      if (__builtin_amdgcn_ballot_w64(bad) != 0 && (threadIdx.x & 63) == 0) {
        atomicCAS(a.nf_flag, 0u, a.launch_id + 1u);
        atomicAdd(a.nf_flag + 1, 1u);
      }
    }
#pragma unroll
    for (int nb0 = 0; nb0 < NB; nb0 += EPB) {
      if (EARLY && nb0 == 0) {
        epi_finish(nb0, e_offs, e_ad, e_mk);
      } else {
        unsigned offs[EPB][4];
        float4 ad[EPB][4], mk[EPB][4];
        epi_issue(tile_idx, nb0, offs, ad, mk);
        epi_finish(nb0, offs, ad, mk);
      }
    }
#pragma unroll
    for (int nb = 0; nb < NB; ++nb)
#pragma unroll
      for (int e = 0; e < 16; ++e) acc[nb][e] = 0.f;
  };

  split8(raw[0][0], raw[0][1], pa);
  for (int tl = group; tl < tiles; tl += SL * G) {
    unsigned ahead[4];
#pragma unroll
    for (int k = 0; k < 4; ++k) ahead[k] = (k <= (SUPER + 3) / CH) ? row_off(tl + k * G) : kOOBws;
    ws_unroll<SUPER>([&](auto Q) __attribute__((always_inline)) {
      constexpr int q = decltype(Q)::value;
      if (EARLY && (q % CH) == CH / 2) epi_issue(tl + (q / CH) * G, 0, e_offs, e_ad, e_mk);
      step(Q, std::integral_constant<int, 0>{}, ahead);
      step(Q, std::integral_constant<int, 1>{}, ahead);
      if ((q + 1) % CH == 0) epilogue(tl + (q / CH) * G);
    });
  }
  if (F16 && a.amax_y) amax_publish(a.amax_y, mx);
}

template <int K, int BN, int FMT, int EROWS = 32>
static int launch_ws(ConvArgs& a, const plan::FwdPlan& p, hipStream_t st) {
  const size_t lds = (size_t)Fmt<FMT>::terms * BN * (K + 8) * 2 + 8 * EROWS * EPI_STRIDE * 4 + 2 * BN * 4;
  static bool attr_set = false;
  if (!attr_set) {
    hipError_t e = hipFuncSetAttribute(reinterpret_cast<const void*>(conv1x1_ws_kernel<K, BN, FMT, EROWS>),
                                       hipFuncAttributeMaxDynamicSharedMemorySize, (int)lds);
    if (e != hipSuccess) {
      set_error("conv_forward(weight-stationary 1x1): hipFuncSetAttribute: %s", hipGetErrorString(e));
      return DADET_ELAUNCH;
    }
    attr_set = true;
  }
  a.ws_panel0 = 0;
  for (int i = 0; i < p.ws_parts; ++i) {
    a.tiles_n = p.ws_panels[i];
    hipLaunchKernelGGL((conv1x1_ws_kernel<K, BN, FMT, EROWS>), dim3(p.ws_grid[i]), dim3(512), lds, st, a);
    a.ws_panel0 += p.ws_panels[i];
  }
  return check_launch("conv_forward(weight-stationary 1x1)");
}

int launch_fwd_ws(ConvArgs& a, const plan::FwdPlan& p, int fmt, hipStream_t st) {
  static_assert(WS_ROWS == plan::kWsRows, "rows per workgroup pass");
  if (fmt == 4) {
    switch (p.ws_k) {
      case 64: return launch_ws<64, 128, 4>(a, p, st);
      case 128: return launch_ws<128, 128, 4>(a, p, st);
      default: return p.ws_bn == 128 ? launch_ws<256, 128, 4, 16>(a, p, st) : launch_ws<256, 64, 4>(a, p, st);
    }
  }
  switch (p.ws_k) {
    case 64: return launch_ws<64, 128, 3>(a, p, st);
    case 128: return launch_ws<128, 128, 3>(a, p, st);
    default: return launch_ws<256, 64, 3>(a, p, st);
  }
}

}
```

### da_detect_amd/csrc/elementwise.hip

```cpp
#include "box_match.h"
#include "conv_common.h"
#include <float.h>

namespace dadet {

static inline int stream_blocks(int64_t work_items, int threads) {
  int64_t b = ceil_div64(work_items, threads);
  if (b > kMaxStreamBlocks) b = kMaxStreamBlocks;
  if (b < 1) b = 1;
  return (int)b;
}

__global__ void relu_bn_backward_kernel(const float4* __restrict__ g, const float4* __restrict__ y,
                                        const float4* __restrict__ scale, float4* __restrict__ g_out,
                                        float4* __restrict__ g_scaled, int64_t total4, int C4,
                                        unsigned* __restrict__ amax_out, unsigned* __restrict__ amax_scaled) {
  float mo = 0.f, ms = 0.f;
  for (int64_t i = (int64_t)blockIdx.x * blockDim.x + threadIdx.x; i < total4;
       i += (int64_t)gridDim.x * blockDim.x) {
    const float4 gv = g[i];
    float4 r = gv;
    if (y) {
      const float4 yv = y[i];
      r.x = yv.x > 0.f ? gv.x : 0.f;
      r.y = yv.y > 0.f ? gv.y : 0.f;
      r.z = yv.z > 0.f ? gv.z : 0.f;
      r.w = yv.w > 0.f ? gv.w : 0.f;
    }
    if (g_out) g_out[i] = r;
    mo = fmaxf(fmaxf(mo, fmaxf(fabsf(r.x), fabsf(r.y))), fmaxf(fabsf(r.z), fabsf(r.w)));
    if (g_scaled) {
      float4 s = r;
      if (scale) {
        const float4 sc = scale[i % C4];
        s.x *= sc.x; s.y *= sc.y; s.z *= sc.z; s.w *= sc.w;
      }
      g_scaled[i] = s;
      ms = fmaxf(fmaxf(ms, fmaxf(fabsf(s.x), fabsf(s.y))), fmaxf(fabsf(s.z), fabsf(s.w)));
    }
  }
  if (amax_out) amax_publish(amax_out, mo);
  if (amax_scaled) amax_publish(amax_scaled, ms);
}

__global__ __launch_bounds__(256) void colsum_partial_kernel(const float* __restrict__ g,
                                                             float* __restrict__ partial, int64_t rows,
                                                             int C, int64_t rows_per_split, int cb, int ld) {
  __shared__ float red[256];
  const int lanes = 256 / cb;
  const int cl = threadIdx.x % cb, rl = threadIdx.x / cb;
  const int col = blockIdx.x * cb + cl;
  const int64_t r0 = (int64_t)blockIdx.y * rows_per_split;
  int64_t r1 = r0 + rows_per_split;
  if (r1 > rows) r1 = rows;
  float acc = 0.f;
  if (col < C)
    for (int64_t r = r0 + rl; r < r1; r += lanes) acc += g[r * ld + col];
  red[threadIdx.x] = acc;
  __syncthreads();
  for (int half = lanes / 2; half > 0; half >>= 1) {
    if (rl < half) red[threadIdx.x] += red[threadIdx.x + half * cb];
    __syncthreads();
  }
  if (rl == 0 && col < C) partial[(size_t)blockIdx.y * C + col] = red[cl];
}
__global__ __launch_bounds__(64) void colsum_final_kernel(const float* __restrict__ partial, float* __restrict__ out, int C,
                                                          int splits, int accumulate) {
  const int c = blockIdx.x;
  float acc = 0.f;
  for (int s = threadIdx.x; s < splits; s += 64) acc += partial[(size_t)s * C + c];
#pragma unroll
  for (int off = 32; off > 0; off >>= 1) acc += __shfl_xor(acc, off, 64);
  if (threadIdx.x == 0) out[c] = accumulate ? out[c] + acc : acc;
}
static int colsum_cb(int C) { return C > 32 ? 64 : (C > 16 ? 32 : 16); }
static int colsum_splits(int64_t rows, int C) {
  const int col_blocks = ceil_div(C, colsum_cb(C));
  int64_t want = ceil_div64(kNumCU * 4, col_blocks);
  int64_t max_by_rows = ceil_div64(rows, 64);
  if (want > max_by_rows) want = max_by_rows;
  if (want < 1) want = 1;
  if (want > 1024) want = 1024;
  return (int)want;
}

__global__ void channel_affine_kernel(const float4* __restrict__ x, const float4* __restrict__ scale,
                                      const float4* __restrict__ bias, float4* __restrict__ y,
                                      int64_t total4, int C4, int relu) {
  for (int64_t i = (int64_t)blockIdx.x * blockDim.x + threadIdx.x; i < total4;
       i += (int64_t)gridDim.x * blockDim.x) {
    const int c = (int)(i % C4);
    const float4 xv = x[i], s = scale[c], b = bias[c];
    float4 r;
    r.x = xv.x * s.x + b.x; r.y = xv.y * s.y + b.y; r.z = xv.z * s.z + b.z; r.w = xv.w * s.w + b.w;
    if (relu) {
      r.x = fmaxf(r.x, 0.f); r.y = fmaxf(r.y, 0.f); r.z = fmaxf(r.z, 0.f); r.w = fmaxf(r.w, 0.f);
    }
    y[i] = r;
  }
}

__global__ void maxpool3x3s2_kernel(const float4* __restrict__ x, float4* __restrict__ y, int N, int H,
                                    int W, int C4, int Ho, int Wo) {
  const int64_t total = (int64_t)N * Ho * Wo * C4;
  for (int64_t i = (int64_t)blockIdx.x * blockDim.x + threadIdx.x; i < total;
       i += (int64_t)gridDim.x * blockDim.x) {
    const int c = (int)(i % C4);
    int64_t p = i / C4;
    const int wo = (int)(p % Wo);
    p /= Wo;
    const int ho = (int)(p % Ho);
    const int n = (int)(p / Ho);
    float4 m = make_float4(-FLT_MAX, -FLT_MAX, -FLT_MAX, -FLT_MAX);
#pragma unroll
    for (int r = 0; r < 3; ++r) {
      const int hi = ho * 2 - 1 + r;
      if (hi < 0 || hi >= H) continue;
#pragma unroll
      for (int s = 0; s < 3; ++s) {
        const int wi = wo * 2 - 1 + s;
        if (wi < 0 || wi >= W) continue;
        const float4 v = x[((int64_t)(n * H + hi) * W + wi) * C4 + c];
        m.x = fmaxf(m.x, v.x); m.y = fmaxf(m.y, v.y); m.z = fmaxf(m.z, v.z); m.w = fmaxf(m.w, v.w);
      }
    }
    y[i] = m;
  }
}

__global__ void maxpool3x3s2_relu_backward_kernel(const float4* __restrict__ y, const float4* __restrict__ gp,
                                                  const float4* __restrict__ scale, float4* __restrict__ g, int N, int H,
                                                  int W, int C4, int Ho, int Wo, unsigned* __restrict__ amax_out) {
  const int64_t total = (int64_t)N * H * W * C4;
  float mo = 0.f;
  for (int64_t i = (int64_t)blockIdx.x * blockDim.x + threadIdx.x; i < total;
       i += (int64_t)gridDim.x * blockDim.x) {
    const int c = (int)(i % C4);
    int64_t p = i / C4;
    const int w = (int)(p % W);
    p /= W;
    const int h = (int)(p % H);
    const int n = (int)(p / H);
    const float4 yv = y[i];
    float4 a = make_float4(0.f, 0.f, 0.f, 0.f);
    if (yv.x > 0.f || yv.y > 0.f || yv.z > 0.f || yv.w > 0.f) {
      const int ho0 = h >> 1, ho1 = min((h + 1) >> 1, Ho - 1);
      const int wo0 = w >> 1, wo1 = min((w + 1) >> 1, Wo - 1);
      for (int ho = ho0; ho <= ho1; ++ho) {
        for (int wo = wo0; wo <= wo1; ++wo) {
          bool fx = true, fy = true, fz = true, fw = true;
#pragma unroll
          for (int r = 0; r < 3; ++r) {
            const int hi = ho * 2 - 1 + r;
            if (hi < 0 || hi >= H) continue;
#pragma unroll
            for (int s = 0; s < 3; ++s) {
              const int wi = wo * 2 - 1 + s;
              if (wi < 0 || wi >= W || (hi == h && wi == w)) continue;
              const float4 v = y[((int64_t)(n * H + hi) * W + wi) * C4 + c];
              if (hi < h || (hi == h && wi < w)) {
                fx = fx && yv.x > v.x; fy = fy && yv.y > v.y; fz = fz && yv.z > v.z; fw = fw && yv.w > v.w;
              } else {
                fx = fx && yv.x >= v.x; fy = fy && yv.y >= v.y; fz = fz && yv.z >= v.z; fw = fw && yv.w >= v.w;
              }
            }
          }
          const float4 gv = gp[((int64_t)(n * Ho + ho) * Wo + wo) * C4 + c];
          a.x += fx ? gv.x : 0.f; a.y += fy ? gv.y : 0.f; a.z += fz ? gv.z : 0.f; a.w += fw ? gv.w : 0.f;
        }
      }
    }
    float4 r;
    r.x = yv.x > 0.f ? a.x : 0.f; r.y = yv.y > 0.f ? a.y : 0.f;
    r.z = yv.z > 0.f ? a.z : 0.f; r.w = yv.w > 0.f ? a.w : 0.f;
    if (scale) {
// ... 140 lines not shown
    if (v > best) {
      best = v;
      arg = g;
    }
    low_quality = low_quality || (v == g_best[g]);
  }
  int m = arg;
  if (best < low) m = -1;
  else if (best < high) m = -2;
  if (low_quality) m = arg;
  float lab = m >= 0 ? 1.f : 0.f;
  if (m == -1) lab = 0.f;
  if (!visible[i]) lab = -1.f;
  if (m == -2) lab = -1.f;
  labels[i] = lab;
  const float4 r = g_box[m < 0 ? 0 : m];
  const float ew = p.z - p.x + 1.f, eh = p.w - p.y + 1.f;
  const float ecx = p.x + 0.5f * ew, ecy = p.y + 0.5f * eh;
  const float gw = r.z - r.x + 1.f, gh = r.w - r.y + 1.f;
  const float gcx = r.x + 0.5f * gw, gcy = r.y + 0.5f * gh;
  targets[i] = make_float4((gcx - ecx) / ew, (gcy - ecy) / eh, logf(gw / ew), logf(gh / eh));
}

__global__ void box_match_encode_kernel(const float4* __restrict__ props, int P, const float4* __restrict__ gts,
                                        const int64_t* __restrict__ gt_labels, int G, float high, float low,
                                        float wx, float wy, float ww, float wh, int64_t* __restrict__ matched,
                                        int64_t* __restrict__ labels, float4* __restrict__ targets) {
  extern __shared__ __attribute__((aligned(16))) char smem[];
  float4* g_box = reinterpret_cast<float4*>(smem);
  float* g_area = reinterpret_cast<float*>(g_box + G);
  for (int g = threadIdx.x; g < G; g += blockDim.x) {
    const float4 b = gts[g];
    g_box[g] = b;
    g_area[g] = (b.z - b.x + 1.f) * (b.w - b.y + 1.f);
  }
  __syncthreads();
  const int i = blockIdx.x * blockDim.x + threadIdx.x;
  if (i >= P) return;
  float4 reg;
  int64_t m;
  labels[i] = match_encode_one(props[i], g_box, g_area, gt_labels, G, high, low, wx, wy, ww, wh, &reg, &m);
  matched[i] = m;
  targets[i] = reg;
}

__global__ void focal_fwd_kernel(const float* __restrict__ logits, const int* __restrict__ targets,
                                 float* __restrict__ losses, int64_t total, int C, float gamma,
                                 float alpha) {
  for (int64_t i = (int64_t)blockIdx.x * blockDim.x + threadIdx.x; i < total;
       i += (int64_t)gridDim.x * blockDim.x) {
    const int n = (int)(i / C), d = (int)(i % C);
    const int t = targets[n];
    const float c1 = (t == (d + 1)) ? 1.f : 0.f;
    const float c2 = ((t >= 0) & (t != (d + 1))) ? 1.f : 0.f;
    const float zn = 1.f - alpha, zp = alpha;
    const float x = logits[i];
    const float p = 1.f / (1.f + expf(-x));
    const float term1 = powf(1.f - p, gamma) * logf(fmaxf(p, FLT_MIN));
    const float xpos = (x >= 0.f) ? 1.f : 0.f;
    const float term2 = powf(p, gamma) * (-1.f * x * xpos - logf(1.f + expf(x - 2.f * x * xpos)));
    float l = 0.f;
    l += -c1 * term1 * zp;
    l += -c2 * term2 * zn;
    losses[i] = l;
  }
}
__global__ void focal_bwd_kernel(const float* __restrict__ logits, const int* __restrict__ targets,
                                 const float* __restrict__ d_losses, float* __restrict__ d_logits,
                                 int64_t total, int C, float gamma, float alpha) {
  for (int64_t i = (int64_t)blockIdx.x * blockDim.x + threadIdx.x; i < total;
       i += (int64_t)gridDim.x * blockDim.x) {
    const int n = (int)(i / C), d = (int)(i % C);
    const int t = targets[n];
    const float c1 = (t == (d + 1)) ? 1.f : 0.f;
    const float c2 = ((t >= 0) & (t != (d + 1))) ? 1.f : 0.f;
    const float zn = 1.f - alpha, zp = alpha;
    const float x = logits[i];
    const float p = 1.f / (1.f + expf(-x));
    const float term1 = powf(1.f - p, gamma) * (1.f - p - (p * gamma * logf(fmaxf(p, FLT_MIN))));
    const float xpos = (x >= 0.f) ? 1.f : 0.f;
    const float term2 =
        powf(p, gamma) * ((-1.f * x * xpos - logf(1.f + expf(x - 2.f * x * xpos))) * (1.f - p) * gamma - p);
    float g = 0.f;
    g += -c1 * term1 * zp;
    g += -c2 * term2 * zn;
    d_logits[i] = g * d_losses[i];
  }
}

__global__ __launch_bounds__(256) void sgd_kernel(const dadet_sgd_entry* __restrict__ table, float momentum, int first_step,
                                                  float grad_scale) {
  const dadet_sgd_entry e = table[blockIdx.y];
  const int64_t n = e.numel;
  const bool vec = ((reinterpret_cast<uintptr_t>(e.p) | reinterpret_cast<uintptr_t>(e.g) |
                     reinterpret_cast<uintptr_t>(e.buf)) & 15) == 0;
  const int64_t n4 = vec ? n / 4 : 0;
  if ((int64_t)blockIdx.x * 1024 >= n4 && ((int64_t)blockIdx.x * 256 >= n - n4 * 4)) return;
  const float lr = e.lr, wd = e.weight_decay;
  float4* p4 = reinterpret_cast<float4*>(e.p);
  const float4* g4 = reinterpret_cast<const float4*>(e.g);
  float4* b4 = reinterpret_cast<float4*>(e.buf);
  for (int64_t base = (int64_t)blockIdx.x * 1024; base < n4; base += (int64_t)gridDim.x * 1024) {
    float4 p[4], g[4], b[4];
#pragma unroll
    for (int u = 0; u < 4; ++u) {
      const int64_t i = base + u * 256 + threadIdx.x;
      if (i < n4) {
        p[u] = p4[i];
        g[u] = g4[i];
        if (!first_step) b[u] = b4[i];
      }
    }
#pragma unroll
    for (int u = 0; u < 4; ++u) {
      const int64_t i = base + u * 256 + threadIdx.x;
      if (i >= n4) continue;
      float4 d;
      d.x = g[u].x * grad_scale + wd * p[u].x; d.y = g[u].y * grad_scale + wd * p[u].y;
      d.z = g[u].z * grad_scale + wd * p[u].z; d.w = g[u].w * grad_scale + wd * p[u].w;
      float4 nb;
      if (first_step) {
        nb = d;
      } else {
        nb.x = momentum * b[u].x + d.x; nb.y = momentum * b[u].y + d.y;
        nb.z = momentum * b[u].z + d.z; nb.w = momentum * b[u].w + d.w;
      }
      b4[i] = nb;
      float4 q = p[u];
      q.x -= lr * nb.x; q.y -= lr * nb.y; q.z -= lr * nb.z; q.w -= lr * nb.w;
      p4[i] = q;
    }
  }
  for (int64_t i = n4 * 4 + (int64_t)blockIdx.x * blockDim.x + threadIdx.x; i < n;
       i += (int64_t)gridDim.x * blockDim.x) {
    float p = e.p[i];
    const float d = e.g[i] * grad_scale + wd * p;
    const float b = first_step ? d : momentum * e.buf[i] + d;
    e.buf[i] = b;
    e.p[i] = p - lr * b;
  }
}

}

using namespace dadet;

static bool aligned16(const void* p) { return (reinterpret_cast<uintptr_t>(p) & 15) == 0; }

extern "C" int dadet_relu_bn_backward(const float* g, const float* y, const float* scale, float* g_out,
                                      float* g_scaled, int64_t rows, int C, void* stream) {
  return dadet_relu_bn_backward_m(g, y, scale, g_out, g_scaled, rows, C, nullptr, nullptr, stream);
}

extern "C" int dadet_relu_bn_backward_m(const float* g, const float* y, const float* scale, float* g_out,
                                        float* g_scaled, int64_t rows, int C, float* amax_out, float* amax_scaled,
                                        void* stream) {
  DADET_REQUIRE(rows >= 0 && C > 0 && C % 4 == 0, "relu_bn_backward: C=%d must be a multiple of 4", C);
  if (rows == 0) return DADET_OK;
  DADET_REQUIRE(g && (g_out || g_scaled), "relu_bn_backward: null pointer");
  DADET_REQUIRE(aligned16(g) && aligned16(y) && aligned16(scale) && aligned16(g_out) && aligned16(g_scaled),
                "relu_bn_backward: pointers must be 16-byte aligned");
  const int64_t total4 = rows * (C / 4);
  hipLaunchKernelGGL(relu_bn_backward_kernel, dim3(stream_blocks(total4, 256)), dim3(256), 0,
                     as_stream(stream), reinterpret_cast<const float4*>(g),
                     reinterpret_cast<const float4*>(y), reinterpret_cast<const float4*>(scale),
                     reinterpret_cast<float4*>(g_out), reinterpret_cast<float4*>(g_scaled), total4, C / 4,
                     reinterpret_cast<unsigned*>(g_out ? amax_out : nullptr),
                     reinterpret_cast<unsigned*>(g_scaled ? amax_scaled : nullptr));
  return check_launch("relu_bn_backward");
}

extern "C" int dadet_colsum_workspace_bytes(int64_t rows, int C, size_t* bytes_out) {
  DADET_REQUIRE(rows >= 0 && C > 0 && bytes_out, "colsum_workspace_bytes: bad args");
  *bytes_out = rows == 0 ? 0 : sizeof(float) * (size_t)colsum_splits(rows, C) * C;
  return DADET_OK;
}

extern "C" int dadet_colsum_ld(const float* g, int ld, float* out, int64_t rows, int C, int accumulate, void* workspace,
                               size_t workspace_bytes, void* stream) {
  DADET_REQUIRE(rows >= 0 && C > 0 && ld >= C && out, "colsum: bad args (rows=%lld C=%d ld=%d)", (long long)rows, C, ld);
  hipStream_t st = as_stream(stream);
  if (rows == 0) {
    if (!accumulate) (void)hipMemsetAsync(out, 0, sizeof(float) * C, st);
    return check_launch("colsum(empty)");
  }
  DADET_REQUIRE(g, "colsum: null input");
  const int splits = colsum_splits(rows, C);
  if (workspace_bytes < sizeof(float) * (size_t)splits * C || !workspace) {
    set_error("colsum: workspace too small");
    return DADET_EWORKSPACE;
  }
  const int64_t rps = ceil_div64(rows, splits);
  const int cb = colsum_cb(C);
  hipLaunchKernelGGL(colsum_partial_kernel, dim3(ceil_div(C, cb), splits), dim3(256), 0, st, g,
                     static_cast<float*>(workspace), rows, C, rps, cb, ld);
  hipLaunchKernelGGL(colsum_final_kernel, dim3(C), dim3(64), 0, st, static_cast<const float*>(workspace), out, C,
                     splits, accumulate);
  return check_launch("colsum");
}

extern "C" int dadet_colsum(const float* g, float* out, int64_t rows, int C, void* workspace,
                            size_t workspace_bytes, void* stream) {
  return dadet_colsum_ld(g, C, out, rows, C, 0, workspace, workspace_bytes, stream);
}

extern "C" int dadet_channel_affine(const float* x, const float* scale, const float* bias, float* y,
                                    int64_t rows, int C, int relu, void* stream) {
  DADET_REQUIRE(rows >= 0 && C > 0 && C % 4 == 0, "channel_affine: C=%d must be a multiple of 4", C);
  if (rows == 0) return DADET_OK;
  DADET_REQUIRE(x && scale && bias && y, "channel_affine: null pointer");
  DADET_REQUIRE(aligned16(x) && aligned16(scale) && aligned16(bias) && aligned16(y),
                "channel_affine: pointers must be 16-byte aligned");
  const int64_t total4 = rows * (C / 4);
  hipLaunchKernelGGL(channel_affine_kernel, dim3(stream_blocks(total4, 256)), dim3(256), 0,
                     as_stream(stream), reinterpret_cast<const float4*>(x),
                     reinterpret_cast<const float4*>(scale), reinterpret_cast<const float4*>(bias),
                     reinterpret_cast<float4*>(y), total4, C / 4, relu);
  return check_launch("channel_affine");
}

extern "C" int dadet_maxpool3x3s2_forward(const float* x, float* y, int N, int H, int W, int C, int Ho,
                                          int Wo, void* stream) {
  DADET_REQUIRE(N >= 0 && H > 0 && W > 0 && C > 0 && C % 4 == 0, "maxpool: bad dims");
  DADET_REQUIRE(Ho == (H + 2 - 3) / 2 + 1 && Wo == (W + 2 - 3) / 2 + 1, "maxpool: Ho/Wo mismatch");
  if (N == 0) return DADET_OK;
  DADET_REQUIRE(x && y && aligned16(x) && aligned16(y), "maxpool: bad pointers");
  const int64_t total = (int64_t)N * Ho * Wo * (C / 4);
  hipLaunchKernelGGL(maxpool3x3s2_kernel, dim3(stream_blocks(total, 256)), dim3(256), 0, as_stream(stream),
                     reinterpret_cast<const float4*>(x), reinterpret_cast<float4*>(y), N, H, W, C / 4, Ho,
                     Wo);
  return check_launch("maxpool3x3s2");
}

extern "C" int dadet_maxpool3x3s2_relu_backward(const float* y, const float* gp, const float* scale, float* g, int N,
                                                int H, int W, int C, int Ho, int Wo, float* amax_out, void* stream) {
  DADET_REQUIRE(N >= 0 && H > 0 && W > 0 && C > 0 && C % 4 == 0, "maxpool_relu_backward: bad dims");
  DADET_REQUIRE(Ho == (H + 2 - 3) / 2 + 1 && Wo == (W + 2 - 3) / 2 + 1, "maxpool_relu_backward: Ho/Wo mismatch");
  if (N == 0) return DADET_OK;
  DADET_REQUIRE(y && gp && g && aligned16(y) && aligned16(gp) && aligned16(scale) && aligned16(g),
                "maxpool_relu_backward: bad pointers");
  DADET_REQUIRE((int64_t)N * H * W < (1LL << 31), "maxpool_relu_backward: tensor too large for 32-bit pixel indexing");
  const int64_t total = (int64_t)N * H * W * (C / 4);
  hipLaunchKernelGGL(maxpool3x3s2_relu_backward_kernel, dim3(stream_blocks(total, 256)), dim3(256), 0, as_stream(stream),
                     reinterpret_cast<const float4*>(y), reinterpret_cast<const float4*>(gp),
                     reinterpret_cast<const float4*>(scale), reinterpret_cast<float4*>(g), N, H, W, C / 4, Ho, Wo,
                     reinterpret_cast<unsigned*>(amax_out));
  return check_launch("maxpool3x3s2_relu_backward");
}

extern "C" int dadet_avgpool_forward(const float* x, float* y, int R, int HW, int C, void* stream) {
  DADET_REQUIRE(R >= 0 && HW > 0 && C > 0 && C % 4 == 0, "avgpool: bad dims");
  if (R == 0) return DADET_OK;
  DADET_REQUIRE(x && y && aligned16(x) && aligned16(y), "avgpool: bad pointers");
  hipLaunchKernelGGL(avgpool_fwd_kernel, dim3(stream_blocks((int64_t)R * (C / 4), 256)), dim3(256), 0,
                     as_stream(stream), reinterpret_cast<const float4*>(x), reinterpret_cast<float4*>(y), R,
                     HW, C / 4);
  return check_launch("avgpool_forward");
}
extern "C" int dadet_avgpool_backward(const float* gy, float* gx, int R, int HW, int C, void* stream) {
  DADET_REQUIRE(R >= 0 && HW > 0 && C > 0 && C % 4 == 0, "avgpool_backward: bad dims");
  if (R == 0) return DADET_OK;
  DADET_REQUIRE(gy && gx && aligned16(gy) && aligned16(gx), "avgpool_backward: bad pointers");
  hipLaunchKernelGGL(avgpool_bwd_kernel, dim3(stream_blocks((int64_t)R * HW * (C / 4), 256)), dim3(256), 0,
                     as_stream(stream), reinterpret_cast<const float4*>(gy), reinterpret_cast<float4*>(gx),
                     R, HW, C / 4);
  return check_launch("avgpool_backward");
}

extern "C" int dadet_nchw3_to_nhwc4(const float* x, float* y, int N, int H, int W, void* stream) {
  DADET_REQUIRE(N >= 0 && H > 0 && W > 0, "nchw3_to_nhwc4: bad dims");
  if (N == 0) return DADET_OK;
  DADET_REQUIRE(x && y && aligned16(y), "nchw3_to_nhwc4: bad pointers");
  const int64_t HW = (int64_t)H * W;
  hipLaunchKernelGGL(nchw3_to_nhwc4_kernel, dim3(stream_blocks((int64_t)N * HW, 256)), dim3(256), 0,
                     as_stream(stream), x, reinterpret_cast<float4*>(y), N, HW);
  return check_launch("nchw3_to_nhwc4");
}

extern "C" int dadet_rpn_decode_clip(const float* deltas, const float* anchors, const int64_t* topk_idx,
                                     int K, float wx, float wy, float ww, float wh, float xform_clip,
                                     float im_w, float im_h, float* boxes_out, void* stream) {
  DADET_REQUIRE(K >= 0, "rpn_decode_clip: K < 0");
  if (K == 0) return DADET_OK;
  DADET_REQUIRE(deltas && anchors && topk_idx && boxes_out, "rpn_decode_clip: null pointer");
  DADET_REQUIRE(aligned16(deltas) && aligned16(anchors) && aligned16(boxes_out),
                "rpn_decode_clip: pointers must be 16-byte aligned");
  hipLaunchKernelGGL(rpn_decode_clip_kernel, dim3(ceil_div(K, 256)), dim3(256), 0, as_stream(stream),
                     reinterpret_cast<const float4*>(deltas), reinterpret_cast<const float4*>(anchors),
                     topk_idx, K, wx, wy, ww, wh, xform_clip, im_w, im_h,
                     reinterpret_cast<float4*>(boxes_out));
  return check_launch("rpn_decode_clip");
}

extern "C" int dadet_rpn_anchor_targets(const float* anchors, const unsigned char* visible, int A,
                                        const float* gt_boxes, int G, float high_threshold, float low_threshold,
                                        unsigned* workspace_G, float* labels, float* regression_targets,
                                        void* stream) {
  DADET_REQUIRE(A >= 0 && G > 0, "rpn_anchor_targets: needs A >= 0 anchors and G > 0 ground-truth boxes");
  if (A == 0) return DADET_OK;
  DADET_REQUIRE(anchors && visible && gt_boxes && workspace_G && labels && regression_targets,
                "rpn_anchor_targets: null pointer");
  DADET_REQUIRE(aligned16(anchors) && aligned16(gt_boxes) && aligned16(regression_targets),
                "rpn_anchor_targets: box pointers must be 16-byte aligned");
  DADET_REQUIRE(G <= 3000, "rpn_anchor_targets: G=%d ground-truth boxes exceed the LDS table", G);
  hipStream_t st = as_stream(stream);
  (void)hipMemsetAsync(workspace_G, 0, sizeof(unsigned) * (size_t)G, st);
  int blocks = ceil_div(A, 256);
  if (blocks > kNumCU * 2) blocks = kNumCU * 2;
  hipLaunchKernelGGL(rpn_gt_best_kernel, dim3(blocks), dim3(256), (size_t)G * 24, st,
                     reinterpret_cast<const float4*>(anchors), A, reinterpret_cast<const float4*>(gt_boxes), G,
                     workspace_G);
  hipLaunchKernelGGL(rpn_anchor_targets_kernel, dim3(ceil_div(A, 256)), dim3(256), (size_t)G * 24, st,
                     reinterpret_cast<const float4*>(anchors), visible, A, reinterpret_cast<const float4*>(gt_boxes),
                     G, workspace_G, high_threshold, low_threshold, labels,
                     reinterpret_cast<float4*>(regression_targets));
  return check_launch("rpn_anchor_targets");
}

extern "C" int dadet_box_match_encode(const float* proposals, int P, const float* gt_boxes, const int64_t* gt_labels,
                                      int G, float high_threshold, float low_threshold, float wx, float wy, float ww,
                                      float wh, int64_t* matched_idxs, int64_t* labels, float* regression_targets,
// ... 51 lines not shown
```

### da_detect_amd/modeling/backbone/resnet.py

```python
from collections import namedtuple

import torch
import torch.nn.functional as F
from torch import nn

from ... import _C
from ...layers import Conv2d, FrozenBatchNorm2d, conv2d_affine_act
from ...utils.registry import Registry
from ...utils import streams
from ...utils.streams import WgradLane

StageSpec = namedtuple("StageSpec", ["index", "block_count", "return_features"])


def _specs(*rows):
    return tuple(StageSpec(index=i, block_count=c, return_features=r) for (i, c, r) in rows)


ResNet50StagesTo5 = _specs((1, 3, False), (2, 4, False), (3, 6, False), (4, 3, True))
ResNet50StagesTo4 = _specs((1, 3, False), (2, 4, False), (3, 6, True))
ResNet101StagesTo5 = _specs((1, 3, False), (2, 4, False), (3, 23, False), (4, 3, True))
ResNet101StagesTo4 = _specs((1, 3, False), (2, 4, False), (3, 23, True))
ResNet50FPNStagesTo5 = _specs((1, 3, True), (2, 4, True), (3, 6, True), (4, 3, True))
ResNet101FPNStagesTo5 = _specs((1, 3, True), (2, 4, True), (3, 23, True), (4, 3, True))
ResNet152FPNStagesTo5 = _specs((1, 3, True), (2, 8, True), (3, 36, True), (4, 3, True))


_WGRAD_BATCH = True
_WGRAD_GROUP = __import__("os").environ.get("DADET_WGRAD_GROUP", "1") == "1"


class _WgradGroup(object):

    _known = {}

    def __init__(self, lane, batch, weights):
        self.lane, self.batch, self.reqs = lane, batch, []
        self.on = (_WGRAD_GROUP and batch is not None and _C._mode4() and 2 <= len(weights) <= _C.WGRAD_GROUP_MAX
                   and all(streams.direct_grad_target(w) is not None for w in weights))
        self.key = None
        if self.on:
            self.key = tuple(tuple(w.shape) for w in weights) + (lane.on,)
            self.on = self._known.get(self.key, True) is not False

    def take(self, w, xin, gout, stride, pad, scale, shape=None):
        if not self.on:
            return False
        self.reqs.append(dict(x=xin, gy=gout, weight_shape=tuple(w.shape) if shape is None else shape, stride=stride,
                              pad=pad, out_scale=scale, dw=streams.direct_grad_target(w), accumulate=True))
        return True

    def issue(self):
        if not self.reqs:
            return
        reqs, batch = self.reqs, self.batch
        key = self.key + tuple((tuple(r["x"].shape), r["stride"]) for r in reqs)

        def run():
            ok = self._known.get(key, True) and _C.conv_wgrad_group(reqs, batch)
            if not ok:
                self._known[key] = self._known[self.key] = False
                for r in reqs:
                    _C.conv_wgrad(r["x"], r["gy"], r["weight_shape"], r["stride"], r["pad"], out_scale=r["out_scale"],
                                  dw=r["dw"], accumulate=True, pending=batch)

        self.lane.run_group(run, *[t for r in reqs for t in (r["x"], r["gy"])])
        self.reqs = []


class _BlockBackward(object):

    def __init__(self, needs, x, w1, wd, s1, sd, stride):
        self.need_x, self.n1, self.n2, self.n3, nd = needs
        self.nd = nd and wd is not None
        self.x, self.w1, self.wd, self.s1, self.sd, self.stride = x, w1, wd, s1, sd, stride

    def open(self, G, out, out_private, y2, w2, w3, s3):
        self.S3 = G.contiguous(memory_format=torch.channels_last) if out_private else _C.relu_bn_backward(G, out, None)[1]
        self.lane = WgradLane(G.device, rows=G.shape[0] * G.shape[2] * G.shape[3])
        self.batch = _C.WgradBatch() if _WGRAD_BATCH else None
        weights = ((w3, self.n3), (w2, self.n2), (self.w1, self.n1), (self.wd, self.nd))
        self.group = _WgradGroup(self.lane, self.batch, [w for w, need in weights if need])
        dw3 = self.wgrad(w3, y2, self.S3, 1, 0, s3) if self.n3 else None
        return _C.conv_forward(self.S3, _C.conv_weight_transpose(w3, s3), relu_mode=2, mask_ref=y2), dw3

    def wgrad(self, w, xin, gout, st, pd, sc, shape=None, grouped=True):
        shape = tuple(w.shape) if shape is None else shape
        batch = self.batch
        if grouped and self.group.take(w, xin, gout, st, pd, sc, shape=shape):
            return None
        return self.lane.run_into(w, lambda acc: _C.conv_wgrad(xin, gout, shape, st, pd, out_scale=sc, dw=acc,
                                                               accumulate=True, pending=batch),
                                  lambda: _C.conv_wgrad(xin, gout, shape, st, pd, out_scale=sc, pending=batch),
                                  xin, gout)

    def close(self, S1, in_relu):
        x, w1, wd, s1, sd, stride, S3 = self.x, self.w1, self.wd, self.s1, self.sd, self.stride, self.S3
        dw1 = dwd = dx = None
        if self.n1:
            dw1 = self.wgrad(w1, x, S1, stride, 0, s1)
        if self.nd:
            dwd = self.wgrad(wd, x, S3, stride, 0, sd)
        self.group.issue()
        self.lane.reduce_batch(self.batch)
        if self.need_x:
            gate = dict(relu_mode=2, mask_ref=x) if in_relu else {}
            hw = tuple(x.shape[2:])
            if wd is None:
                dx = _C.conv_forward(S1, _C.conv_weight_transpose(w1, s1), addend=S3, **gate)
            elif stride == 1:
                t = _C.conv_forward(S3, _C.conv_weight_transpose(wd, sd))
                dx = _C.conv_forward(S1, _C.conv_weight_transpose(w1, s1), addend=t, out=t, **gate)
            else:
                t = _C.conv_forward(S3, _C.conv_weight_transpose(wd, sd), out_spatial_stride=stride, out_hw=hw)
                dx = _C.conv_forward(S1, _C.conv_weight_transpose(w1, s1), addend=t, out=t,
                                     out_spatial_stride=stride, out_hw=hw, **gate)
        self.lane.join()
        return dx, dw1, dwd


class _BottleneckFn(torch.autograd.Function):

    @staticmethod
    def forward(ctx, x, w1, w2, w3, wd, s1, b1, s2, b2, s3, b3, sd, bd, stride, in_relu, out_private):
        y1 = _C.conv_forward(x, w1, s1, b1, stride=stride, relu_mode=1)
        y2 = _C.conv_forward(y1, w2, s2, b2, pad=1, relu_mode=1)
        idn = x if wd is None else _C.conv_forward(x, wd, sd, bd, stride=stride)
        out = _C.conv_forward(y2, w3, s3, b3, addend=idn, relu_mode=1)
        ctx.stride, ctx.in_relu, ctx.out_private = stride, in_relu, out_private
        ctx.save_for_backward(x, y1, y2, out, w1, w2, w3, wd, s1, s2, s3, sd)
        return out

    @staticmethod
    @torch.autograd.function.once_differentiable
    def backward(ctx, G):
        x, y1, y2, out, w1, w2, w3, wd, s1, s2, s3, sd = ctx.saved_tensors
        need_x, n1, n2 = ctx.needs_input_grad[:3]
        b = _BlockBackward(ctx.needs_input_grad[:5], x, w1, wd, s1, sd, ctx.stride)
        S2, dw3 = b.open(G, out, ctx.out_private, y2, w2, w3, s3)
        dw2 = S1 = None
        if n2:
            dw2 = b.wgrad(w2, y1, S2, 1, 1, s2)
        if n1 or need_x:
            S1 = _C.conv_forward(S2, _C.conv_weight_transpose(w2, s2), pad=1, relu_mode=2, mask_ref=y1)
        dx, dw1, dwd = b.close(S1, ctx.in_relu)
        return (dx, dw1, dw2, dw3, dwd) + (None,) * 11


class _DCNBottleneckFn(torch.autograd.Function):

    @staticmethod
    def forward(ctx, x, w1, w2, w3, wd, w_off, b_off, s1, b1, s2, b2, s3, b3, sd, bd, stride, in_relu, out_private,
                modulated, dg):
        cout2, cin2, kh, kw = w2.shape
        y1 = _C.conv_forward(x, w1, s1, b1, stride=stride, relu_mode=1)
        wo4, bo4 = _pad_out_channels(w_off, b_off)
        om = _C.conv_forward(y1, wo4, None, bo4, pad=kh // 2)
        cols = _C.deform_sample_forward_om(y1, om, kh, kw, 1, kh // 2, 1, dg, modulated)
        y2 = _C.conv_forward(cols, _as_1x1(w2), s2, b2, relu_mode=1)
        idn = x if wd is None else _C.conv_forward(x, wd, sd, bd, stride=stride)
        out = _C.conv_forward(y2, w3, s3, b3, addend=idn, relu_mode=1)
        ctx.conf = (stride, in_relu, out_private, modulated, dg, kh, kw, w_off.shape[0], wo4.shape[0])
        ctx.b_off = b_off
        ctx.save_for_backward(x, y1, om, cols, y2, out, w1, w2, w3, wd, w_off, s1, s2, s3, sd)
        return out

    @staticmethod
    @torch.autograd.function.once_differentiable
    def backward(ctx, G):
        x, y1, om, cols, y2, out, w1, w2, w3, wd, w_off, s1, s2, s3, sd = ctx.saved_tensors
        stride, in_relu, out_private, modulated, dg, kh, kw, n_offch, n_offpad = ctx.conf
        n2, n_off, n_boff = ctx.needs_input_grad[2], ctx.needs_input_grad[5], ctx.needs_input_grad[6]
        cout2, cin2 = w2.shape[0], w2.shape[1]
        b = _BlockBackward(ctx.needs_input_grad[:5], x, w1, wd, s1, sd, stride)
        S2, dw3 = b.open(G, out, out_private, y2, w2, w3, s3)
        dw2 = dwo = dbo = None
        w2_1x1 = _as_1x1(w2)
        if n2:
            dw2 = b.wgrad(w2, cols, S2, 1, 0, s2, shape=(cout2, kh * kw * cin2, 1, 1))
        gcols = _C.conv_forward(S2, _C.conv_weight_transpose(w2_1x1, s2))
        gy1, gom = _C.deform_sample_backward_om(y1, om, gcols, kh, kw, 1, kh // 2, 1, dg, modulated)
        if n_off:
            dwo = b.wgrad(w_off, y1, gom, 1, kh // 2, None, grouped=False)
        if n_boff:
            dbo = streams.bias_grad(ctx.b_off, gom, cols=n_offch)
        S1 = _C.conv_forward(gom, _C.conv_weight_transpose(w_off, cout_pad=n_offpad), pad=kh // 2, addend=gy1, out=gy1,
                             relu_mode=2, mask_ref=y1)
        dx, dw1, dwd = b.close(S1, in_relu)
        if dw2 is not None:
            dw2 = torch.as_strided(dw2, (cout2, cin2, kh, kw), (kh * kw * cin2, 1, kw * cin2, cin2))
        return (dx, dw1, dw2, dw3, dwd, dwo, dbo) + (None,) * 13


def _as_1x1(weight):
    cout, cin, kh, kw = weight.shape
    return weight.contiguous(memory_format=torch.channels_last).permute(0, 2, 3, 1).reshape(cout, kh * kw * cin, 1, 1)


class _PaddedWeights(object):

    def __init__(self):
        self.entries = {}
        self.stamp = None

    def _stamp(self):
        ws = [e["w"]() for e in self.entries.values()]
        bs = [e["b"]() for e in self.entries.values() if e["b"] is not None]
        if any(t is None for t in ws) or any(t is None for t in bs):
            return None
        return (_C.weight_epoch(), tuple(t._version for t in ws), tuple(t._version for t in bs))

    def _fresh(self):
        stamp = self._stamp()
        if stamp is not None and stamp == self.stamp:
            return
        for k in [k for k, e in self.entries.items() if e["w"]() is None or (e["b"] is not None and e["b"]() is None)]:
            del self.entries[k]
        dst, src = [], []
        for e in self.entries.values():
            w = e["w"]()
            dst.append(e["wp"][:w.shape[0]])
            src.append(w.detach())
            if e["b"] is not None:
                dst.append(e["bp"][:w.shape[0]])
                src.append(e["b"]().detach())
        if dst:
            torch._foreach_copy_(dst, src)
        self.stamp = self._stamp()

    def get(self, weight, bias, pad):
        import weakref

        e = self.entries.get(id(weight))
        if e is None or e["w"]() is not weight or (bias is not None) != (e["b"] is not None) \
                or (bias is not None and e["b"]() is not bias):
            cout, cin, kh, kw = weight.shape
            wp = torch.zeros((cout + pad, cin, kh, kw), dtype=weight.dtype, device=weight.device).contiguous(
                memory_format=torch.channels_last)
            bp = torch.zeros(cout + pad, dtype=bias.dtype, device=bias.device) if bias is not None else None
            wp._dadet_amax_like = weakref.ref(weight)
            self.entries[id(weight)] = dict(w=weakref.ref(weight), b=weakref.ref(bias) if bias is not None else None,
                                            wp=wp, bp=bp)
            self.stamp = None
        self._fresh()
        e = self.entries[id(weight)]
        return e["wp"], e["bp"]


_PADDED = _PaddedWeights()


def _pad_out_channels(weight, bias):
    pad = (-weight.shape[0]) % 4
    if pad == 0:
        return weight, bias
    if weight.is_cuda and weight.is_leaf and weight.requires_grad and (bias is None or bias.is_leaf):
        return _PADDED.get(weight, bias, pad)
    w = F.pad(weight, (0, 0, 0, 0, 0, 0, 0, pad)).contiguous(memory_format=torch.channels_last)
    return w, (F.pad(bias, (0, pad)) if bias is not None else None)


_DCN_FUSED = __import__("os").environ.get("DADET_DCN_FUSED", "1") == "1"


class Bottleneck(nn.Module):

    def __init__(self, in_channels, bottleneck_channels, out_channels, num_groups, stride_in_1x1, stride,
                 dilation, norm_func, dcn_config=None):
        super(Bottleneck, self).__init__()
        dcn_config = dcn_config or {}
        if num_groups != 1 or dilation != 1:
            raise NotImplementedError("grouped / dilated bottlenecks are outside the DA Faster R-CNN path")
        self.downsample = None
        if in_channels != out_channels:
            self.downsample = nn.Sequential(
                Conv2d(in_channels, out_channels, kernel_size=1, stride=stride, bias=False),
                norm_func(out_channels))
            nn.init.kaiming_uniform_(self.downsample[0].weight, a=1)
        stride_1x1, stride_3x3 = (stride, 1) if stride_in_1x1 else (1, stride)
        self.conv1 = Conv2d(in_channels, bottleneck_channels, kernel_size=1, stride=stride_1x1, bias=False)
        self.bn1 = norm_func(bottleneck_channels)
        self.with_dcn = bool(dcn_config.get("stage_with_dcn", False))
        if self.with_dcn:
            from ...layers.dcn import DFConv2d
            self.conv2 = DFConv2d(bottleneck_channels, bottleneck_channels,
                                  with_modulated_dcn=dcn_config.get("with_modulated_dcn", False), kernel_size=3,
                                  stride=stride_3x3, groups=num_groups, dilation=dilation,
                                  deformable_groups=dcn_config.get("deformable_groups", 1), bias=False)
        else:
            self.conv2 = Conv2d(bottleneck_channels, bottleneck_channels, kernel_size=3, stride=stride_3x3,
                                padding=1, bias=False)
        self.bn2 = norm_func(bottleneck_channels)
        self.conv3 = Conv2d(bottleneck_channels, out_channels, kernel_size=1, bias=False)
        self.bn3 = norm_func(out_channels)
        for l in (self.conv1, self.conv3) + (() if self.with_dcn else (self.conv2,)):
            nn.init.kaiming_uniform_(l.weight, a=1)

    def forward(self, x, in_relu=False, out_private=False, stride=None):
        if self.with_dcn:
            assert stride is None
            if self._dcn_fusable(x):
                c2 = self.conv2
                wd = sd = bd = None
                if self.downsample is not None:
                    wd, (sd, bd) = self.downsample[0].weight, self.downsample[1].folded()
                return _DCNBottleneckFn.apply(x, self.conv1.weight, c2.conv.weight, self.conv3.weight, wd,
                                              c2.offset.weight, c2.offset.bias, *self.bn1.folded(), *self.bn2.folded(),
                                              *self.bn3.folded(), sd, bd, self.conv1.stride[0], in_relu, out_private,
                                              c2.with_modulated_dcn, c2.conv.deformable_groups)
            return self._forward_dcn(x)
        if self.conv2.stride[0] == 1:
            if x.shape[0] == 0 and stride is None:
                return self._forward_per_conv(x)
            wd = sd = bd = None
            if self.downsample is not None:
                wd, (sd, bd) = self.downsample[0].weight, self.downsample[1].folded()
            return _BottleneckFn.apply(x, self.conv1.weight, self.conv2.weight, self.conv3.weight, wd,
                                       *self.bn1.folded(), *self.bn2.folded(), *self.bn3.folded(), sd, bd,
                                       self.conv1.stride[0] if stride is None else stride, in_relu, out_private)
        assert stride is None
        return self._forward_per_conv(x)

    def input_is_strided_1x1(self):
        s = self.conv1.stride[0]
        if (self.uses_fused_path() and s > 1 and self.downsample is not None and self.conv1.kernel_size == (1, 1)
                and self.downsample[0].kernel_size == (1, 1) and self.downsample[0].stride[0] == s):
            return s
        return 1

    def uses_fused_path(self):
        if self.with_dcn:
            return self._dcn_fusable(None)
        return self.conv2.stride[0] == 1

    def _dcn_fusable(self, x):
        c = self.conv2.conv
        ok = (_DCN_FUSED and c.stride == 1 and c.dilation == 1 and c.groups == 1 and c.bias is None
              and c.kernel_size == (3, 3) and c.in_channels % (4 * c.deformable_groups) == 0)
        return ok and (x is None or (x.is_cuda and x.shape[0] > 0))

    def _forward_dcn(self, x):
        out = self.conv1(x, *self.bn1.folded(), relu=True)
        out = F.relu(self.bn2(self.conv2(out)))
        identity = x if self.downsample is None else self.downsample[0](x, *self.downsample[1].folded())
        return self.conv3(out, *self.bn3.folded(), residual=identity, relu=True)

    def _forward_per_conv(self, x):
        out = self.conv1(x, *self.bn1.folded(), relu=True)
        out = self.conv2(out, *self.bn2.folded(), relu=True)
        identity = x if self.downsample is None else self.downsample[0](x, *self.downsample[1].folded())
        return self.conv3(out, *self.bn3.folded(), residual=identity, relu=True)


class BottleneckWithFixedBatchNorm(Bottleneck):
    def __init__(self, in_channels, bottleneck_channels, out_channels, num_groups=1, stride_in_1x1=True,
                 stride=1, dilation=1, dcn_config=None):
        super(BottleneckWithFixedBatchNorm, self).__init__(
            in_channels, bottleneck_channels, out_channels, num_groups, stride_in_1x1, stride, dilation,
            norm_func=FrozenBatchNorm2d, dcn_config=dcn_config)


class _StemFn(torch.autograd.Function):

    @staticmethod
    def forward(ctx, x4, w4, scale, shift, out_size):
        y = _C.conv_forward(x4, w4, scale, shift, stride=2, pad=3, relu_mode=1, out_size=out_size)
        ctx.w_shape = tuple(w4.shape)
        ctx.save_for_backward(x4, y, scale)
        return _C.maxpool3x3s2(y)

    @staticmethod
    @torch.autograd.function.once_differentiable
    def backward(ctx, gp):
        x4, y, scale = ctx.saved_tensors
        g = _C.maxpool3x3s2_relu_backward(y, gp, scale)
        lane = WgradLane(gp.device)
        dw4 = lane.run(lambda: _C.conv_wgrad(x4, g, ctx.w_shape, 2, 3), x4, g)
        lane.join()
        return None, dw4, None, None, None


class BaseStem(nn.Module):

    def __init__(self, cfg, norm_func):
        super(BaseStem, self).__init__()
        out_channels = cfg.MODEL.RESNETS.STEM_OUT_CHANNELS
        self.conv1 = Conv2d(3, out_channels, kernel_size=7, stride=2, padding=3, bias=False)
        self.bn1 = norm_func(out_channels)
        nn.init.kaiming_uniform_(self.conv1.weight, a=1)
        self._w4 = None

    def _padded_weight(self):
        w = self.conv1.weight
        if w.requires_grad and torch.is_grad_enabled():
            return F.pad(w, (0, 1, 0, 0, 0, 1)).contiguous(memory_format=torch.channels_last)
        key = (w._version, w.device, _C.weight_epoch() if w.requires_grad else 0)
        if self._w4 is None or self._w4[0] != key:
            with torch.no_grad():
                self._w4 = (key, F.pad(w, (0, 1, 0, 0, 0, 1)).contiguous(memory_format=torch.channels_last))
        return self._w4[1]

    def forward(self, x):
        N, C, H, W = x.shape
        assert C == 3, "the stem expects BGR images [N,3,H,W]"
        x4 = _C.nchw3_to_nhwc4(x)
        out_size = _C.conv_out_size(H, W, 7, 7, 2, 3)
        scale, shift = self.bn1.folded()
        w4 = self._padded_weight()
        if N > 0 and torch.is_grad_enabled() and w4.requires_grad:
            return _StemFn.apply(x4, w4, scale, shift, out_size)
        y = conv2d_affine_act(x4, w4, scale, shift, None, 2, 3, True, out_size)
        return _C.maxpool3x3s2(y)


class StemWithFixedBatchNorm(BaseStem):
    def __init__(self, cfg):
        super(StemWithFixedBatchNorm, self).__init__(cfg, norm_func=FrozenBatchNorm2d)


def _make_stage(block, in_channels, bottleneck_channels, out_channels, block_count, num_groups,
                stride_in_1x1, first_stride, dilation=1, dcn_config=None):
    blocks, stride = [], first_stride
    for _ in range(block_count):
        blocks.append(block(in_channels, bottleneck_channels, out_channels, num_groups, stride_in_1x1, stride,
                            dilation=dilation, dcn_config=dcn_config))
        stride = 1
        in_channels = out_channels
    return _Stage(*blocks)


class _Stage(nn.Sequential):

    input_is_relu = False

    def forward(self, x, first_stride=None):
        n = len(self)
        blocks = list(self)
        for i, block in enumerate(blocks):
            private = i < n - 1 and blocks[i + 1].uses_fused_path()
            if i == 0 and first_stride is not None:
                x = block(x, in_relu=self.input_is_relu, out_private=private, stride=first_stride)
            else:
                x = block(x, in_relu=(i > 0 or self.input_is_relu), out_private=private)
        return x


class ResNet(nn.Module):
    def __init__(self, cfg):
        super(ResNet, self).__init__()
        stem_module = _STEM_MODULES[cfg.MODEL.RESNETS.STEM_FUNC]
        stage_specs = _STAGE_SPECS[cfg.MODEL.BACKBONE.CONV_BODY]
        block = _TRANSFORMATION_MODULES[cfg.MODEL.RESNETS.TRANS_FUNC]
        self.stem = stem_module(cfg)
        num_groups = cfg.MODEL.RESNETS.NUM_GROUPS
        in_channels = cfg.MODEL.RESNETS.STEM_OUT_CHANNELS
        stage2_bottleneck = num_groups * cfg.MODEL.RESNETS.WIDTH_PER_GROUP
        stage2_out = cfg.MODEL.RESNETS.RES2_OUT_CHANNELS
        self.stages, self.return_features = [], {}
        for spec in stage_specs:
            name = "layer" + str(spec.index)
            factor = 2 ** (spec.index - 1)
            out_channels = stage2_out * factor
            self.add_module(name, _make_stage(block, in_channels, stage2_bottleneck * factor, out_channels,
                                              spec.block_count, num_groups, cfg.MODEL.RESNETS.STRIDE_IN_1X1,
                                              first_stride=int(spec.index > 1) + 1,
                                              dcn_config={
                                                  "stage_with_dcn": cfg.MODEL.RESNETS.STAGE_WITH_DCN[spec.index - 1],
                                                  "with_modulated_dcn": cfg.MODEL.RESNETS.WITH_MODULATED_DCN,
                                                  "deformable_groups": cfg.MODEL.RESNETS.DEFORMABLE_GROUPS}))
            in_channels = out_channels
            getattr(self, name).input_is_relu = spec.index > 1
            self.stages.append(name)
# ... 61 lines not shown
```

### include/dadet.h

```cpp
#ifndef DADET_H_
#define DADET_H_

#include <stddef.h>
#include <stdint.h>

#ifdef __cplusplus
extern "C" {
#endif

#define DADET_OK 0
#define DADET_EINVAL (-1)
#define DADET_ELAUNCH (-2)
#define DADET_EWORKSPACE (-3)
#define DADET_EUNSUPPORTED (-4)

const char* dadet_last_error(void);
int dadet_version(void);
int dadet_device_info(int* cu_count, int* clock_khz, size_t* hbm_bytes, char* arch_name, int arch_name_len);

int dadet_nms_workspace_bytes(int n, size_t* bytes_out);
int dadet_nms(const float* boxes_xyxy, const float* scores, int n, float thresh, int tie_rule,
              int max_keep, void* workspace, size_t workspace_bytes, int64_t* keep_out,
              int* num_keep_out, void* stream);
int dadet_nms_batch_workspace_bytes(int batch, int n_max, size_t* bytes_out);
int dadet_nms_batch(const float* boxes_xyxy, const int* n_host, int batch, int n_max, float thresh, int tie_rule,
                    int max_keep, void* workspace, size_t workspace_bytes, int64_t* keep_out, int* num_keep_out,
                    void* stream);

int dadet_detect_post_workspace_bytes(const int* rows_host, int batch, int num_classes, size_t* bytes_out);
int dadet_detect_post(const float* boxes, const float* scores, const int* rows_host, int batch, int num_classes,
                      float score_thresh, float nms_thresh, int tie_rule, int detections_per_img, int read_counts,
                      void* workspace, size_t workspace_bytes, float* out_boxes, float* out_scores, int64_t* out_labels,
                      int* out_counts, void* stream);

int dadet_coco_match_workspace_bytes(const int* det_off_host, const int* gt_off_host, int pairs, int n_det, int n_gt, int n_thr,
                                     int n_area, size_t* bytes_out);
int dadet_coco_match(const double* det_box, const double* gt_box, const double* gt_area, const int* gt_crowd,
                     const int* det_off_host, const int* gt_off_host, int pairs, int n_det, int n_gt,
                     const double* iou_thr_host, int n_thr, const double* area_rng_host, int n_area, void* workspace,
                     size_t workspace_bytes, unsigned char* matched_out, unsigned char* ignored_out, int* npig_out,
                     void* stream);

int dadet_roi_align_forward(const float* input, const float* rois, float* output, int B, int C, int H,
                            int W, int R, int pooled_h, int pooled_w, float spatial_scale,
                            int sampling_ratio, void* stream);
int dadet_roi_align_backward(const float* grad_output, const float* rois, float* grad_input, int B,
                             int C, int H, int W, int R, int pooled_h, int pooled_w,
                             float spatial_scale, int sampling_ratio, void* stream);
int dadet_roi_align_workspace_bytes(int B, int H, int W, int R, size_t* bytes);
int dadet_roi_align_forward_ws(const float* input, const float* rois, float* output, int B, int C, int H, int W, int R,
                               int pooled_h, int pooled_w, float spatial_scale, int sampling_ratio, void* workspace,
                               size_t workspace_bytes, void* stream);
int dadet_roi_align_backward_atomic(const float* grad_output, const float* rois, float* grad_input, int B,
                                    int C, int H, int W, int R, int pooled_h, int pooled_w,
                                    float spatial_scale, int sampling_ratio, void* stream);
int dadet_roi_align_forward_sub(const float* input, const float* rois, float* output, int B, int C, int H, int W, int R,
                                int pooled_h, int pooled_w, float spatial_scale, int sampling_ratio, int bin_stride,
                                void* workspace, size_t workspace_bytes, void* stream);
int dadet_roi_align_backward_sub(const float* grad_output, const float* rois, float* grad_input, int B, int C, int H,
                                 int W, int R, int pooled_h, int pooled_w, float spatial_scale, int sampling_ratio,
                                 int bin_stride, void* stream);
int dadet_roi_align_forward_level(const float* input, const float* rois, const int64_t* levels, int level, float* output,
                                  int B, int C, int H, int W, int R, int pooled_h, int pooled_w, float spatial_scale,
                                  int sampling_ratio, void* workspace, size_t workspace_bytes, void* stream);
int dadet_roi_align_backward_level(const float* grad_output, const float* rois, const int64_t* levels, int level,
                                   float* grad_input, int B, int C, int H, int W, int R, int pooled_h, int pooled_w,
                                   float spatial_scale, int sampling_ratio, void* stream);

int dadet_sigmoid_focal_loss_forward(const float* logits, const int32_t* targets, float* losses, int N,
                                     int C, float gamma, float alpha, void* stream);
int dadet_sigmoid_focal_loss_backward(const float* logits, const int32_t* targets,
                                      const float* d_losses, float* d_logits, int N, int C,
                                      float gamma, float alpha, void* stream);

typedef struct dadet_conv_desc {
  int N, H, W, Cin;
  int Cout, KH, KW;
  int stride, pad;
  int Ho, Wo;
  int OutH, OutW;
  int out_spatial_stride;
  int relu_mode;
} dadet_conv_desc;

int dadet_conv_forward(const dadet_conv_desc* d, const float* x, const float* w, const float* scale,
                       const float* bias, const float* addend, const float* mask_ref, float* y,
                       void* stream);

int dadet_set_gemm_mode(int mode);
int dadet_get_gemm_mode(void);

int dadet_set_big_gemm(int mode);
int dadet_get_big_gemm(void);

int dadet_nonfinite_poll(char* msg, int cap);

#define DADET_AMAX_STRIDE 65536
typedef struct dadet_amax_item {
  const void* x;
  void* slot;
  long long n;
  int first_block, blocks;
} dadet_amax_item;
int dadet_amax(const float* x, long long n, float* slot, void* stream);
int dadet_amax_batch(const dadet_amax_item* items_dev, int n, int total_blocks, void* stream);

int dadet_conv_forward_scaled(const dadet_conv_desc* d, const float* x, const float* w, const float* scale,
                              const float* bias, const float* addend, const float* mask_ref, float* y,
                              const float* amax_x, const float* amax_w, float* amax_y, void* stream);

int dadet_conv_forward_variant(const dadet_conv_desc* d);

typedef struct dadet_conv_plan_info {
  int family, variant;
  int tiles_m, tiles_n;
  int ksplit, splits;
  int rows_per_split;
  int sk_dp_tiles, sk_tiles, sk_units, sk_iters, sk_max_parts;
  int big_splits, big_body;
  int launches, grid;
  int needs_counters;
  size_t workspace_bytes;
  char name[64];
} dadet_conv_plan_info;
int dadet_conv_forward_plan(const dadet_conv_desc* d, dadet_conv_plan_info* out);
int dadet_conv_wgrad_plan(const dadet_conv_desc* d, int gy_ld, dadet_conv_plan_info* out);

int dadet_conv_wgrad_workspace_bytes(const dadet_conv_desc* d, size_t* bytes_out);
int dadet_conv_wgrad_variant(const dadet_conv_desc* d);
int dadet_conv_wgrad(const dadet_conv_desc* d, const float* x, const float* gy, const float* out_scale,
                     float* dw, int accumulate, void* workspace, size_t workspace_bytes, void* stream);
typedef struct dadet_wgrad_pending {
  const float* partials;
  const float* out_scale;
  float* dw;
  long long count;
  int K, splits, accumulate;
} dadet_wgrad_pending;
int dadet_conv_wgrad_partials(const dadet_conv_desc* d, const float* x, const float* gy, const float* out_scale,
                              float* dw, int accumulate, void* workspace, size_t workspace_bytes,
                              dadet_wgrad_pending* pending_out, void* stream);
int dadet_conv_wgrad_reduce_batch(const dadet_wgrad_pending* items, int n, void* stream);
int dadet_conv_wgrad_partials_ld(const dadet_conv_desc* d, const float* x, const float* gy, int gy_ld,
                                 const float* out_scale, float* dw, int accumulate, void* workspace,
                                 size_t workspace_bytes, dadet_wgrad_pending* pending_out, void* stream);

int dadet_conv_wgrad_scaled(const dadet_conv_desc* d, const float* x, const float* gy, int gy_ld,
                            const float* out_scale, float* dw, int accumulate, void* workspace,
                            size_t workspace_bytes, dadet_wgrad_pending* pending_out, const float* amax_x,
                            const float* amax_gy, void* stream);

int dadet_conv_wgrad_group_plan(const dadet_conv_desc* descs, int n, int* splits_out, size_t* workspace_bytes_out);
int dadet_conv_wgrad_group(const dadet_conv_desc* descs, int n, const float* const* x, const float* const* gy,
                           const float* const* out_scale, float* const* dw, const int* accumulate,
                           void* const* workspace, const size_t* workspace_bytes, dadet_wgrad_pending* pending_out,
                           const float* const* amax_x, const float* const* amax_gy, void* stream);

int dadet_conv_weight_transpose(const float* w, const float* scale, float* wt, int Cout, int KH, int KW,
                                int Cin, void* stream);
int dadet_conv_weight_transpose_padded(const float* w, const float* scale, float* wt, int Cout, int KH, int KW,
                                       int Cin, int cout_pad, void* stream);

typedef struct dadet_transpose_item {
  const float* w;
  const float* scale;
  float* wt;
  int Cout, KH, KW, Cin;
  int first_block, blocks_ci, blocks_co;
  int cout_pad;
} dadet_transpose_item;
int dadet_conv_weight_transpose_batch(const dadet_transpose_item* items_dev, int n, int total_blocks, void* stream);

int dadet_deform_sample_forward(const float* x, const float* offset, const float* mask, float* cols, int N,
                                int H, int W, int C, int KH, int KW, int stride, int pad, int dil,
                                int deformable_groups, int Ho, int Wo, void* stream);
int dadet_deform_sample_backward(const float* x, const float* offset, const float* mask, const float* gcols,
                                 float* gx, float* goffset, float* gmask, int N, int H, int W, int C, int KH,
                                 int KW, int stride, int pad, int dil, int deformable_groups, int Ho, int Wo,
                                 void* stream);
int dadet_deform_sample_forward_ld(const float* x, const float* offset, int offset_ld, const float* mask, int mask_ld,
                                   int mask_is_logit, float* cols, int N, int H, int W, int C, int KH, int KW, int stride,
                                   int pad, int dil, int deformable_groups, int Ho, int Wo, void* stream);
int dadet_deform_sample_backward_ld(const float* x, const float* offset, int offset_ld, const float* mask, int mask_ld,
                                    int mask_is_logit, const float* gcols, float* gx, float* goffset, int goffset_ld,
                                    float* gmask, int gmask_ld, int N, int H, int W, int C, int KH, int KW, int stride,
                                    int pad, int dil, int deformable_groups, int Ho, int Wo, void* workspace,
                                    size_t workspace_bytes, void* stream);
int dadet_deform_sample_backward_ld_m(const float* x, const float* offset, int offset_ld, const float* mask, int mask_ld,
                                      int mask_is_logit, const float* gcols, float* gx, float* goffset, int goffset_ld,
                                      float* gmask, int gmask_ld, int N, int H, int W, int C, int KH, int KW, int stride,
                                      int pad, int dil, int deformable_groups, int Ho, int Wo, void* workspace,
                                      size_t workspace_bytes, float* amax_gom, long long gom_floats, void* stream);
int dadet_deform_sample_backward_workspace_bytes(int N, int H, int W, int deformable_groups, size_t* bytes_out);

int dadet_roi_pool_forward(const float* input, const float* rois, float* output, int* argmax, int B, int C, int H,
                           int W, int R, int pooled_h, int pooled_w, float spatial_scale, void* stream);
int dadet_roi_pool_backward(const float* grad_output, const int* argmax, const float* rois, float* grad_input, int B,
                            int C, int H, int W, int R, int pooled_h, int pooled_w, void* stream);

int dadet_image_resample_h(const unsigned char* image_hwc, int H, int W, const int* bounds, const int* coeffs,
                           int ksize, int out_w, unsigned char* out_hwc, void* stream);
int dadet_image_resample_v_normalize(const unsigned char* image_hwc, int in_h, int w, const int* bounds,
                                     const int* coeffs, int ksize, int out_h, int flip, int to_bgr255,
                                     const float* mean3, const float* std3, float* out_hw3, int out_row_stride,
                                     void* stream);

int dadet_rpn_loss(const float* objectness, const float* box_regression, const int64_t* sampled_inds,
                   const float* labels_sampled, int num_sampled, const int64_t* pos_inds,
                   const float* regression_targets_pos, int num_pos, float beta, float* losses_out,
                   float* grad_objectness, float* grad_box_regression, void* stream);
int dadet_rpn_loss_rows(const float* objectness, const float* box_regression, const int64_t* sampled_inds,
                        const float* labels_sampled, int num_sampled, int num_pos, const float* regression_targets_pos,
                        int anchors_per_location, float beta, float* losses_out, float* grad_rows, int ldg,
                        int* pixels_out, void* stream);
int dadet_rpn_loss_rows_level(const float* objectness, const float* box_regression, const int64_t* sampled_inds,
                              const float* labels_sampled, int num_sampled, int num_pos,
                              const float* regression_targets_pos, int anchors_per_location, float beta,
                              int64_t anchors_per_image, int64_t level_offset, int64_t level_anchors, int level_id,
                              int* row_level_out, int shared_rows, float* losses_out, float* grad_rows, int ldg,
                              int* pixels_out, void* stream);
int dadet_gather_pixel_taps_level(const float* x, const int* pixels, const int* row_level, int level, int num_rows, int N,
                                  int H, int W, int C, int KH, int KW, int pad, float* out, void* stream);
int dadet_scatter_pixel_taps_add_level(const float* y, const int* pixels, const int* row_level, int level, int num_rows,
                                       int N, int H, int W, int C, int KH, int KW, int pad, float* dx, void* stream);
int dadet_gather_pixel_taps(const float* x, const int* pixels, int num_rows, int N, int H, int W, int C, int KH, int KW,
                            int pad, float* out, void* stream);
int dadet_scatter_pixel_taps_add(const float* y, const int* pixels, int num_rows, int N, int H, int W, int C, int KH,
                                 int KW, int pad, float* dx, void* stream);
int dadet_fast_rcnn_loss(const float* class_logits, const float* box_regression, int num_classes, int reg_cols,
                         const int64_t* src_rows, const int64_t* labels_src, int num_src, const int64_t* rows_pos,
                         const int64_t* map_inds, const float* regression_targets_pos, int num_pos,
                         float* losses_out, float* grad_class_logits, float* grad_box_regression, void* stream);

int dadet_fast_rcnn_loss_rows(const float* class_logits, const float* box_regression, int num_rows, int num_classes,
                              int reg_cols, const int64_t* loss_labels, const float* regression_targets,
                              float* losses_out, float* grad_class_logits, float* grad_box_regression, void* stream);

int dadet_sample_rois(const float* boxes, const int64_t* labels, const float* regression_targets, int n, int cap,
                      int max_pos, uint64_t seed, int is_source, int64_t* idx_out, float* boxes_out,
                      int64_t* labels_out, float* regression_targets_out, int64_t* loss_labels_out,
                      unsigned char* domain_out, int* counts_out, void* stream);

typedef struct dadet_merge_entry {
  const float* boxes;
  const float* scores;
  const int64_t* keep;
  const int* count;
  float* boxes_out;
  float* scores_out;
  int n, cap;
} dadet_merge_entry;
int dadet_fpn_merge_levels(const dadet_merge_entry* entries, int n, void* stream);

int dadet_proposals_sample(const float* sorted_boxes, const float* sorted_scores, const int64_t* keep,
                           const int* count_dev, int post_n, const float* appended_boxes, int num_appended,
                           const float* gt_boxes, const int64_t* gt_labels, int G, float high_threshold,
                           float low_threshold, float wx, float wy, float ww, float wh, int cap, int max_pos, uint64_t seed,
                           int is_source, float* prop_boxes, float* prop_scores, int* n_props, int64_t* idx_out,
                           float* boxes_out, int64_t* labels_out, float* regression_targets_out, int64_t* loss_labels_out,
                           unsigned char* domain_out, float* objectness_out, int* counts_out, void* stream);

int dadet_sample_anchors(const float* labels, const float* regression_targets, int A, int cap, int max_pos,
                         uint64_t seed, int64_t index_offset, int64_t* pos_inds_out, int64_t* neg_inds_out,
                         float* regression_targets_pos_out, int* counts_out, void* stream);

int dadet_topk_sorted(const float* scores, int rows, int n, int64_t row_stride, int k, float* out_scores,
                      int64_t* out_idx, void* stream);

typedef struct dadet_topk_row {
  const float* scores;
  float* out_scores;
  int64_t* out_idx;
  int n, k;
} dadet_topk_row;
int dadet_topk_sorted_rows_workspace_bytes(int rows, int k_max, size_t* bytes_out);
int dadet_topk_sorted_rows(const dadet_topk_row* rows_in, int rows, void* workspace, size_t workspace_bytes, void* stream);

int dadet_rpn_anchor_targets(const float* anchors, const unsigned char* visible, int A, const float* gt_boxes, int G,
                             float high_threshold, float low_threshold, unsigned* workspace_G, float* labels,
                             float* regression_targets, void* stream);

int dadet_box_match_encode(const float* proposals, int P, const float* gt_boxes, const int64_t* gt_labels, int G,
                           float high_threshold, float low_threshold, float wx, float wy, float ww, float wh,
                           int64_t* matched_idxs, int64_t* labels, float* regression_targets, void* stream);

int dadet_deform_psroi_pool_forward(const float* data, const float* rois, const float* trans, float* out,
                                    float* top_count, int B, int H, int W, int C, int R, int no_trans,
                                    float spatial_scale, int output_dim, int group_size, int pooled_size,
                                    int part_size, int sample_per_part, float trans_std, int num_classes,
                                    void* stream);
int dadet_deform_psroi_pool_backward(const float* grad_out, const float* top_count, const float* data,
                                     const float* rois, const float* trans, float* grad_data, float* grad_trans,
                                     int B, int H, int W, int C, int R, int no_trans, float spatial_scale,
                                     int output_dim, int group_size, int pooled_size, int part_size,
                                     int sample_per_part, float trans_std, int num_classes, void* stream);

int dadet_relu_bn_backward(const float* g, const float* y, const float* scale, float* g_out,
                           float* g_scaled, int64_t rows, int C, void* stream);
int dadet_relu_bn_backward_m(const float* g, const float* y, const float* scale, float* g_out, float* g_scaled,
                             int64_t rows, int C, float* amax_out, float* amax_scaled, void* stream);
int dadet_colsum_workspace_bytes(int64_t rows, int C, size_t* bytes_out);
int dadet_colsum_ld(const float* g, int ld, float* out, int64_t rows, int C, int accumulate, void* workspace,
                    size_t workspace_bytes, void* stream);
int dadet_colsum(const float* g, float* out, int64_t rows, int C, void* workspace, size_t workspace_bytes,
                 void* stream);
int dadet_channel_affine(const float* x, const float* scale, const float* bias, float* y, int64_t rows,
                         int C, int relu, void* stream);
int dadet_maxpool3x3s2_forward(const float* x, float* y, int N, int H, int W, int C, int Ho, int Wo,
                               void* stream);
int dadet_maxpool3x3s2_relu_backward(const float* y, const float* gp, const float* scale, float* g, int N, int H,
                                     int W, int C, int Ho, int Wo, float* amax_out, void* stream);
int dadet_avgpool_forward(const float* x, float* y, int R, int HW, int C, void* stream);
int dadet_avgpool_backward(const float* gy, float* gx, int R, int HW, int C, void* stream);
int dadet_nchw3_to_nhwc4(const float* x, float* y, int N, int H, int W, void* stream);

int dadet_rpn_decode_clip(const float* deltas, const float* anchors, const int64_t* topk_idx, int K,
                          float wx, float wy, float ww, float wh, float xform_clip, float im_w,
                          float im_h, float* boxes_out, void* stream);

int dadet_da_img_head_loss_forward(const float* t, const float* w2, const float* b2, const float* labels,
                                   float* logits_out, float* sums_out, int num_images,
                                   int rows_per_image, int C1, void* stream);
int dadet_da_img_head_loss_backward(const float* t, const float* w2, const float* logits,
                                    const float* labels, const float* coef, float* g_t_w, float* g_t_x,
                                    float* g_w2, float* g_b2, int num_images, int rows_per_image, int C1,
                                    void* stream);
int dadet_da_img_head_loss_backward_g(const float* t, const float* w2, const float* logits, const float* labels,
                                      const float* g_bce, const float* g_mean_sig, const float* w_adv_dev, float w_adv,
                                      float w_cst, float* g_t_w, float* g_t_x, float* g_w2, float* g_b2, int num_images,
                                      int rows_per_image, int C1, void* stream);
int dadet_da_img_head_loss_backward_gm(const float* t, const float* w2, const float* logits, const float* labels,
                                       const float* g_bce, const float* g_mean_sig, const float* w_adv_dev, float w_adv,
                                       float w_cst, float* g_t_w, float* g_t_x, float* g_w2, float* g_b2, int num_images,
                                       int rows_per_image, int C1, float* amax_w, float* amax_x, void* stream);
int dadet_da_ins_tail_forward(const float* h, const float* w3, const float* b3, const float* labels,
                              const float* means, float* logits, float* sums, int R_bce, int R_cst, int n_src,
                              int levels, int C, void* stream);
int dadet_da_ins_tail_backward(const float* h, const float* w3, const float* logits, const float* labels,
                               const float* means, const float* coef, float inv_keep, float* g_z, float* g_w3,
                               float* g_b3, float* g_means, int R_bce, int R_cst, int n_src, int levels, int C,
                               void* stream);
int dadet_da_ins_tail_forward_n(const float* h, const float* w3, const float* b3, const float* labels,
                                const float* means, float* logits, float* sums, int R_bce, int R_cst,
                                const int* row_end, int num_images, int levels, int C, void* stream);
int dadet_da_ins_tail_backward_n(const float* h, const float* w3, const float* logits, const float* labels,
                                 const float* means, const float* coef, float inv_keep, float* g_z, float* g_w3,
                                 float* g_b3, float* g_means, int R_bce, int R_cst, const int* row_end, int num_images,
                                 int levels, int C, void* stream);
int dadet_da_ins_dropout_rows(const float* h1, const float* masks, float* out, int64_t numel_per_pass, int passes,
                              void* stream);
int dadet_da_ins_merge(const float* g, const float* masks, const float* h1, const float* grl, float* g_w, float* g_x,
                       int64_t numel_per_pass, int passes, void* stream);

int dadet_triplet_w_forward(const float* anchor, const float* positive, const float* negative, int H,
                            int W, int C, float margin, float eps, float* dist_out, float* loss_sum,
                            void* stream);
int dadet_triplet_w_backward(const float* anchor, const float* positive, const float* negative,
                             const float* dist, const float* g_scale, int H, int W, int C, float margin,
                             float eps, float* g_anchor, float* g_positive, float* g_negative,
                             void* stream);

typedef struct dadet_sgd_entry {
  float* p; const float* g; float* buf; int64_t numel; float lr; float weight_decay;
} dadet_sgd_entry;
int dadet_sgd_step(const dadet_sgd_entry* table_dev, int num_tensors, int64_t max_numel, float momentum,
                   int first_step, float grad_scale, void* stream);

#ifdef __cplusplus
}
#endif
#endif
```

Baseline: 162.3.

## Pack ReLU sign bits in forward conv epilogue to gate backward passes

The weight-stationary 1x1 conv epilogue can now write a packed 1-bit-per-element sign plane of the block output. Backward ReLU gating (relu_bn_backward and the dx conv's relu_mode 2) reads that bitmask instead of the full float32 activation tensor. This cuts activation reads in the backward pass by about 32x for these gates. In exchange it adds an extra store plus DPP lane reductions in the forward epilogue, a second kernel template instantiation, and plan-lookup overhead on the Python side.

```diff
diff --git a/da_detect_amd/_C.py b/da_detect_amd/_C.py
--- a/da_detect_amd/_C.py
+++ b/da_detect_amd/_C.py
@@ -392,8 +392,42 @@
     return (H + 2 * pad - KH) // stride + 1, (W + 2 * pad - KW) // stride + 1
 
 
+SIGN_PLANES = 0
+SIGN_GATES = 0
+_WS_PLAN_CACHE = {}
+
+
+def sign_bits_on():
+    return os.environ.get("DADET_SIGN_BITS", "1") != "0"
+
+
+def sign_plane(t):
+    a = t.__dict__.get("_dadet_sign_bits") if t is not None else None
+    return a[0] if a is not None and a[1] == t._version else None
+
+
+def pack_sign_bits(y):
+    M, C = y.shape
+    assert C % 32 == 0, "sign planes hold whole words per row: C=%d" % C
+    b = (y > 0).reshape(M, C // 32, 32).to(torch.int64)
+    words = (b << torch.arange(32, dtype=torch.int64, device=y.device)).sum(dim=2)
+    return (words - ((words >> 31) << 32)).to(torch.int32)
+
+
+def _ws_serves(d):
+    _mode4()
+    key = (d.N, d.H, d.W, d.Cin, d.Cout, d.KH, d.KW, d.stride, d.pad, d.Ho, d.Wo, d.out_spatial_stride, _MODE,
+           os.environ.get("DADET_WS_1X1"), os.environ.get("DADET_EPILOGUE_V4"))
+    hit = _WS_PLAN_CACHE.get(key)
+    if hit is None:
+        info = _lib.ConvPlanInfo()
+        _lib.call("dadet_conv_forward_plan", ctypes.byref(d), ctypes.byref(info))
+        hit = _WS_PLAN_CACHE[key] = info.family == 4 and d.Cout % 32 == 0
+    return hit
+
+
 def conv_forward(x, w, scale=None, bias=None, addend=None, mask_ref=None, stride=1, pad=0, relu_mode=0,
-                 out=None, out_spatial_stride=1, out_hw=None, out_size=None):
+                 out=None, out_spatial_stride=1, out_hw=None, out_size=None, sign_out=False, gate_bits=None):
     _dev(x, "x"), _dev(w, "w")
     N, Cin, H, W = x.shape
     Cout, Cin_w, KH, KW = w.shape
@@ -415,6 +449,21 @@
     if mask_ref is not None:
         mask_ref = _nhwc(mask_ref)
     d = _desc(N, H, W, Cin, Cout, KH, KW, stride, pad, Ho, Wo, OutH, OutW, out_spatial_stride, relu_mode)
+    bits = None
+    if relu_mode == 2 and gate_bits is None:
+        sign_out = False
+    if (sign_out or gate_bits is not None) and N > 0 and sign_bits_on() and _ws_serves(d):
+        global SIGN_PLANES, SIGN_GATES
+        plane = None
+        if sign_out:
+            plane = torch.empty((N * Ho * Wo, Cout // 32), dtype=torch.int32, device=x.device)
+            SIGN_PLANES += 1
+        if gate_bits is not None:
+            assert relu_mode == 2 and gate_bits.dtype == torch.int32 and gate_bits.is_contiguous() \
+                and gate_bits.numel() * 32 == out.numel(), "conv_forward: gate_bits is not the plane of this output's shape"
+            mask_ref = None
+            SIGN_GATES += 1
+        bits = (plane, gate_bits)
     ax = aw = None
     if _mode4():
         ax, aw = _amax.ptr(x), _weight_amax(w)
@@ -432,14 +481,25 @@
         with PROFILER.span(kname,
                            2.0 * N * Ho * Wo * Cout * Cin * KH * KW,
                            4.0 * (x_read + w.numel() + out.numel() + (addend.numel() if addend is not None else 0)
-                                  + (mask_ref.numel() if mask_ref is not None else 0))):
-            _conv_forward_call(d, x, w, scale, bias, addend, mask_ref, out, ax, aw)
+                                  + (mask_ref.numel() if mask_ref is not None else 0)
+                                  + sum(b.numel() for b in (bits or ()) if b is not None))):
+            _conv_forward_call(d, x, w, scale, bias, addend, mask_ref, out, ax, aw, bits)
         return out
-    _conv_forward_call(d, x, w, scale, bias, addend, mask_ref, out, ax, aw)
+    _conv_forward_call(d, x, w, scale, bias, addend, mask_ref, out, ax, aw, bits)
     return out
 
 
-def _conv_forward_call(d, x, w, scale, bias, addend, mask_ref, out, ax, aw):
+def _conv_forward_call(d, x, w, scale, bias, addend, mask_ref, out, ax, aw, bits=None):
+    if bits is not None:
+        slot = _amax.new_slot(out.device) if ax is not None else None
+        _lib.call("dadet_conv_forward_bits", ctypes.byref(d), _p(x), _p(w), _p(scale), _p(bias), _p(addend),
+                  _p(mask_ref), _p(out), ax, aw, ctypes.c_void_p(slot[0]) if slot else None, _p(bits[0]), _p(bits[1]),
+                  _stream())
+        if slot:
+            _amax.attach(out, slot)
+        if bits[0] is not None:
+            out._dadet_sign_bits = (bits[0], out._version)
+        return
     if ax is None:
         _lib.call("dadet_conv_forward", ctypes.byref(d), _p(x), _p(w), _p(scale), _p(bias), _p(addend),
                   _p(mask_ref), _p(out), _stream())
@@ -727,17 +787,29 @@
               1 if accumulate else 0, _p(ws), ctypes.c_size_t(ws.numel()), _stream())
 
 
-def relu_bn_backward(g, y=None, scale=None, want_unscaled=False):
+def relu_bn_backward(g, y=None, scale=None, want_unscaled=False, y_bits=None):
     _dev(g, "g")
     g = _nhwc(g) if g.dim() == 4 else g.contiguous()
     C = g.shape[1]
     rows = g.numel() // C
+    if y_bits is not None and not (sign_bits_on() and C % 32 == 0):
+        y_bits = None
     yy = None
-    if y is not None:
+    if y is not None and y_bits is None:
         yy = _nhwc(y) if y.dim() == 4 else y.contiguous()
     g_out = torch.empty_like(g) if want_unscaled else None
     g_scaled = torch.empty_like(g)
+    if y_bits is not None:
+        assert y_bits.dtype == torch.int32 and y_bits.is_contiguous() and y_bits.numel() * 32 == g.numel(), \
+            "relu_bn_backward: y_bits is not the plane of a tensor of g's shape"
+        yy = y_bits
+        global SIGN_GATES
+        SIGN_GATES += 1
+    entry = "dadet_relu_bn_backward_bits" if y_bits is not None else "dadet_relu_bn_backward_m"
     if not _mode4():
+        if y_bits is not None:
+            _lib.call(entry, _p(g), _p(yy), _p(scale), _p(g_out), _p(g_scaled), rows, C, None, None, _stream())
+            return g_out, g_scaled
         _lib.call("dadet_relu_bn_backward", _p(g), _p(yy), _p(scale), _p(g_out), _p(g_scaled), rows, C, _stream())
         return g_out, g_scaled
     so = ss = None
@@ -745,7 +817,7 @@
         so = _amax.new_slot(g.device)
     if scale is not None or _amax.slot_of(_amax.carry(g_scaled, g)) is None:
         ss = _amax.new_slot(g.device)
-    _lib.call("dadet_relu_bn_backward_m", _p(g), _p(yy), _p(scale), _p(g_out), _p(g_scaled), rows, C,
+    _lib.call(entry, _p(g), _p(yy), _p(scale), _p(g_out), _p(g_scaled), rows, C,
               ctypes.c_void_p(so[0]) if so else None, ctypes.c_void_p(ss[0]) if ss else None, _stream())
     if so:
         _amax.attach(g_out, so)
diff --git a/da_detect_amd/_lib.py b/da_detect_amd/_lib.py
--- a/da_detect_amd/_lib.py
+++ b/da_detect_amd/_lib.py
@@ -87,6 +87,7 @@
     "dadet_sigmoid_focal_loss_backward": [_P, _P, _P, _P, c_int, c_int, c_float, c_float, _P],
     "dadet_conv_forward": [POINTER(ConvDesc), _P, _P, _P, _P, _P, _P, _P, _P],
     "dadet_conv_forward_scaled": [POINTER(ConvDesc), _P, _P, _P, _P, _P, _P, _P, _P, _P, _P, _P],
+    "dadet_conv_forward_bits": [POINTER(ConvDesc), _P, _P, _P, _P, _P, _P, _P, _P, _P, _P, _P, _P, _P],
     "dadet_conv_wgrad_scaled": [POINTER(ConvDesc), _P, _P, c_int, _P, _P, c_int, _P, c_size_t, POINTER(WgradPending), _P, _P,
                                 _P],
     "dadet_amax": [_P, ctypes.c_longlong, _P, _P],
@@ -154,6 +155,7 @@
                                          c_float, c_int, c_int, c_int, c_int, c_int, c_float, c_int, _P],
     "dadet_relu_bn_backward": [_P, _P, _P, _P, _P, c_int64, c_int, _P],
     "dadet_relu_bn_backward_m": [_P, _P, _P, _P, _P, c_int64, c_int, _P, _P, _P],
+    "dadet_relu_bn_backward_bits": [_P, _P, _P, _P, _P, c_int64, c_int, _P, _P, _P],
     "dadet_colsum_workspace_bytes": [c_int64, c_int, POINTER(c_size_t)],
     "dadet_colsum": [_P, _P, c_int64, c_int, _P, c_size_t, _P],
     "dadet_colsum_ld": [_P, c_int, _P, c_int64, c_int, c_int, _P, c_size_t, _P],
diff --git a/da_detect_amd/csrc/conv_common.h b/da_detect_amd/csrc/conv_common.h
--- a/da_detect_amd/csrc/conv_common.h
+++ b/da_detect_amd/csrc/conv_common.h
@@ -176,6 +176,8 @@
   const float* amax_x;
   const float* amax_w;
   unsigned* amax_y;
+  unsigned* sign_out;
+  const unsigned* gate_bits;
 };
 
 struct WgradArgs {
diff --git a/da_detect_amd/csrc/conv_dispatch.hip b/da_detect_amd/csrc/conv_dispatch.hip
--- a/da_detect_amd/csrc/conv_dispatch.hip
+++ b/da_detect_amd/csrc/conv_dispatch.hip
@@ -67,13 +67,17 @@
 static int conv_forward_impl(const dadet_conv_desc* d, const float* x, const float* w,
                              const float* scale, const float* bias, const float* addend,
                              const float* mask_ref, float* y, const float* amax_x, const float* amax_w,
-                             float* amax_y, void* stream) {
+                             float* amax_y, void* stream, unsigned* sign_out = nullptr,
+                             const unsigned* gate_bits = nullptr) {
   int rc = conv_desc_check(d, "conv_forward");
   if (rc) return rc;
   if (d->N == 0) return DADET_OK;
   DADET_REQUIRE(x && w && y && al16(x) && al16(w), "conv_forward: x / w must be non-null and 16-byte aligned");
   DADET_REQUIRE(d->relu_mode >= 0 && d->relu_mode <= 2, "conv_forward: relu_mode");
-  DADET_REQUIRE(d->relu_mode != 2 || mask_ref, "conv_forward: relu_mode 2 needs mask_ref");
+  DADET_REQUIRE(d->relu_mode != 2 || mask_ref || gate_bits, "conv_forward: relu_mode 2 needs mask_ref");
+  DADET_REQUIRE(!gate_bits || d->relu_mode == 2, "conv_forward: gate_bits are the gate of relu_mode 2");
+  DADET_REQUIRE(!sign_out || d->relu_mode != 2 || gate_bits,
+                "conv_forward: a launch that writes sign_out takes its relu_mode 2 gate from gate_bits, not from mask_ref");
   const plan::Gemm g = plan::gemm_of(d);
   DADET_REQUIRE(g.os == 1 ? (d->OutH == d->Ho && d->OutW == d->Wo)
                           : ((d->Ho - 1) * g.os < d->OutH && (d->Wo - 1) * g.os < d->OutW),
@@ -84,9 +88,15 @@
   const bool aligned16 = al16(y) && (!addend || al16(addend)) && (!mask_ref || al16(mask_ref)) && (!scale || al16(scale)) &&
                          (!bias || al16(bias));
   const plan::FwdPlan p = plan::plan_forward(d, aligned16, mode, g_big_mode);
+  DADET_REQUIRE((!sign_out && !gate_bits) || p.family == plan::kFwdWs,
+                "conv_forward: sign_out / gate_bits need the weight-stationary 1x1 kernel; this launch (M=%d N=%d K=%d) "
+                "runs plan family %d (dadet_conv_forward_plan)", g.M, d->Cout, g.K, p.family);
+  DADET_REQUIRE((reinterpret_cast<uintptr_t>(sign_out) & 3) == 0 && (reinterpret_cast<uintptr_t>(gate_bits) & 3) == 0,
+                "conv_forward: sign_out / gate_bits must be 4-byte aligned");
   ConvArgs a;
   fill_conv_args(d, g, p, &a);
   a.x = x; a.w = w; a.scale = scale; a.bias = bias; a.addend = addend; a.mask_ref = mask_ref; a.y = y;
+  a.sign_out = sign_out; a.gate_bits = gate_bits;
   hipStream_t st = as_stream(stream);
   if (mode == 4) {
     if (!amax_x || !amax_w) {
@@ -259,6 +269,13 @@
   return conv_forward_impl(d, x, w, scale, bias, addend, mask_ref, y, amax_x, amax_w, amax_y, stream);
 }
 
+extern "C" int dadet_conv_forward_bits(const dadet_conv_desc* d, const float* x, const float* w,
+                                       const float* scale, const float* bias, const float* addend,
+                                       const float* mask_ref, float* y, const float* amax_x, const float* amax_w,
+                                       float* amax_y, unsigned* sign_out, const unsigned* gate_bits, void* stream) {
+  return conv_forward_impl(d, x, w, scale, bias, addend, mask_ref, y, amax_x, amax_w, amax_y, stream, sign_out, gate_bits);
+}
+
 extern "C" int dadet_conv_forward_plan(const dadet_conv_desc* d, dadet_conv_plan_info* out) {
   int rc = conv_desc_check(d, "conv_forward_plan");
   if (rc) return rc;
diff --git a/da_detect_amd/csrc/conv_ws.hip b/da_detect_amd/csrc/conv_ws.hip
--- a/da_detect_amd/csrc/conv_ws.hip
+++ b/da_detect_amd/csrc/conv_ws.hip
@@ -15,7 +15,7 @@
   }
 }
 
-template <int K, int BN, int FMT, int EROWS = 32>
+template <int K, int BN, int FMT, int EROWS = 32, bool BITS = false>
 __global__ __launch_bounds__(512, 1) void conv1x1_ws_kernel(const ConvArgs a) {
   constexpr int T = Fmt<FMT>::terms;
   constexpr bool F16 = Fmt<FMT>::f16;
@@ -172,13 +172,20 @@
 
   const __amdgpu_buffer_rsrc_t yr = make_rsrc(a.y, a.y_bytes);
   const __amdgpu_buffer_rsrc_t ar = make_rsrc(a.addend ? a.addend : a.y, a.addend ? a.y_bytes : 0u);
-  const __amdgpu_buffer_rsrc_t mr = make_rsrc(a.mask_ref ? a.mask_ref : a.y, a.mask_ref ? a.y_bytes : 0u);
+  const void* const gate_p = BITS ? (const void*)a.gate_bits : (const void*)a.mask_ref;
+  const __amdgpu_buffer_rsrc_t mr = make_rsrc(gate_p ? gate_p : a.y, gate_p ? (BITS ? a.y_bytes / 32u : a.y_bytes) : 0u);
+  const __amdgpu_buffer_rsrc_t sr = make_rsrc(a.sign_out ? (void*)a.sign_out : a.y, a.sign_out ? a.y_bytes / 32u : 0u);
+  auto bits_off = [](const unsigned off) __attribute__((always_inline)) -> unsigned {
+    return off == kOOB ? kOOB : (off >> 5) & ~3u;
+  };
   const int col_in = lane & 31, row_hi = 4 * (lane >> 5);
   const int rrow = lane >> 3, c4 = (lane & 7) * 4;
 
   unsigned e_offs[EPB][4];
-  float4 e_ad[EPB][4], e_mk[EPB][4];
-  auto epi_issue = [&](int tile_idx, int nb0, unsigned (&offs)[EPB][4], float4 (&ad)[EPB][4], float4 (&mk)[EPB][4])
+  using MkT = std::conditional_t<BITS, unsigned, float4>;
+  float4 e_ad[EPB][4];
+  MkT e_mk[EPB][4];
+  auto epi_issue = [&](int tile_idx, int nb0, unsigned (&offs)[EPB][4], float4 (&ad)[EPB][4], MkT (&mk)[EPB][4])
       __attribute__((always_inline)) {
     const int mbase = tile_idx * WS_ROWS + wave * 32;
 #pragma unroll
@@ -200,10 +207,13 @@
 #pragma unroll
       for (int e = 0; e < EPB; ++e)
 #pragma unroll
-        for (int pass = 0; pass < 4; ++pass) mk[e][pass] = buf_load4(mr, offs[e][pass]);
-    }
-  };
-  auto epi_finish = [&](int nb0, const unsigned (&offs)[EPB][4], const float4 (&ad)[EPB][4], const float4 (&mk)[EPB][4])
+        for (int pass = 0; pass < 4; ++pass) {
+          if constexpr (BITS) mk[e][pass] = __builtin_amdgcn_raw_buffer_load_b32(mr, (int)bits_off(offs[e][pass]), 0, 0);
+          else mk[e][pass] = buf_load4(mr, offs[e][pass]);
+        }
+    }
+  };
+  auto epi_finish = [&](int nb0, const unsigned (&offs)[EPB][4], const float4 (&ad)[EPB][4], const MkT (&mk)[EPB][4])
       __attribute__((always_inline)) {
 #pragma unroll
     for (int e = 0; e < EPB; ++e) {
@@ -231,8 +241,14 @@
           adv[0] = q4.x; adv[1] = q4.y; adv[2] = q4.z; adv[3] = q4.w;
         }
         if (a.relu_mode == 2) {
-          const float4 q4 = mk[e][pass];
-          mkv[0] = q4.x; mkv[1] = q4.y; mkv[2] = q4.z; mkv[3] = q4.w;
+          if constexpr (BITS) {
+            const unsigned nib = mk[e][pass] >> c4;
+#pragma unroll
+            for (int k = 0; k < 4; ++k) mkv[k] = ((nib >> k) & 1u) ? 1.f : 0.f;
+          } else {
+            const float4 q4 = mk[e][pass];
+            mkv[0] = q4.x; mkv[1] = q4.y; mkv[2] = q4.z; mkv[3] = q4.w;
+          }
         }
 #pragma unroll
         for (int k = 0; k < 4; ++k) {
@@ -248,6 +264,13 @@
                                                (int)offs[e][pass], 0, 0);
         if (F16 && a.amax_y && offs[e][pass] != kOOB)
           mx = fmaxf(fmaxf(mx, fmaxf(fabsf(v[0]), fabsf(v[1]))), fmaxf(fabsf(v[2]), fabsf(v[3])));
+        if (BITS && a.sign_out) {
+          unsigned wd = ((v[0] > 0.f ? 1u : 0u) | (v[1] > 0.f ? 2u : 0u) | (v[2] > 0.f ? 4u : 0u) | (v[3] > 0.f ? 8u : 0u)) << c4;
+          wd |= (unsigned)__builtin_amdgcn_update_dpp(0, (int)wd, 0xB1, 0xf, 0xf, true);
+          wd |= (unsigned)__builtin_amdgcn_update_dpp(0, (int)wd, 0x4E, 0xf, 0xf, true);
+          wd |= (unsigned)__builtin_amdgcn_update_dpp(0, (int)wd, 0x141, 0xf, 0xf, true);
+          __builtin_amdgcn_raw_buffer_store_b32(wd, sr, (int)(c4 == 0 ? bits_off(offs[e][pass]) : kOOB), 0, 0);
+        }
       }
       __builtin_amdgcn_wave_barrier();
       }
@@ -271,7 +294,8 @@
         epi_finish(nb0, e_offs, e_ad, e_mk);
       } else {
         unsigned offs[EPB][4];
-        float4 ad[EPB][4], mk[EPB][4];
+        float4 ad[EPB][4];
+        MkT mk[EPB][4];
         epi_issue(tile_idx, nb0, offs, ad, mk);
         epi_finish(nb0, offs, ad, mk);
       }
@@ -298,12 +322,15 @@
   if (F16 && a.amax_y) amax_publish(a.amax_y, mx);
 }
 
-template <int K, int BN, int FMT, int EROWS = 32>
+template <int K, int BN, int FMT, int EROWS = 32, bool BITS = false>
 static int launch_ws(ConvArgs& a, const plan::FwdPlan& p, hipStream_t st) {
+  if constexpr (!BITS) {
+    if (a.sign_out || a.gate_bits) return launch_ws<K, BN, FMT, EROWS, true>(a, p, st);
+  }
   const size_t lds = (size_t)Fmt<FMT>::terms * BN * (K + 8) * 2 + 8 * EROWS * EPI_STRIDE * 4 + 2 * BN * 4;
   static bool attr_set = false;
   if (!attr_set) {
-    hipError_t e = hipFuncSetAttribute(reinterpret_cast<const void*>(conv1x1_ws_kernel<K, BN, FMT, EROWS>),
+    hipError_t e = hipFuncSetAttribute(reinterpret_cast<const void*>(conv1x1_ws_kernel<K, BN, FMT, EROWS, BITS>),
                                        hipFuncAttributeMaxDynamicSharedMemorySize, (int)lds);
     if (e != hipSuccess) {
       set_error("conv_forward(weight-stationary 1x1): hipFuncSetAttribute: %s", hipGetErrorString(e));
@@ -314,7 +341,7 @@
   a.ws_panel0 = 0;
   for (int i = 0; i < p.ws_parts; ++i) {
     a.tiles_n = p.ws_panels[i];
-    hipLaunchKernelGGL((conv1x1_ws_kernel<K, BN, FMT, EROWS>), dim3(p.ws_grid[i]), dim3(512), lds, st, a);
+    hipLaunchKernelGGL((conv1x1_ws_kernel<K, BN, FMT, EROWS, BITS>), dim3(p.ws_grid[i]), dim3(512), lds, st, a);
     a.ws_panel0 += p.ws_panels[i];
   }
   return check_launch("conv_forward(weight-stationary 1x1)");
diff --git a/da_detect_amd/csrc/elementwise.hip b/da_detect_amd/csrc/elementwise.hip
--- a/da_detect_amd/csrc/elementwise.hip
+++ b/da_detect_amd/csrc/elementwise.hip
@@ -14,13 +14,20 @@
 __global__ void relu_bn_backward_kernel(const float4* __restrict__ g, const float4* __restrict__ y,
                                         const float4* __restrict__ scale, float4* __restrict__ g_out,
                                         float4* __restrict__ g_scaled, int64_t total4, int C4,
-                                        unsigned* __restrict__ amax_out, unsigned* __restrict__ amax_scaled) {
+                                        unsigned* __restrict__ amax_out, unsigned* __restrict__ amax_scaled,
+                                        const unsigned* __restrict__ y_bits) {
   float mo = 0.f, ms = 0.f;
   for (int64_t i = (int64_t)blockIdx.x * blockDim.x + threadIdx.x; i < total4;
        i += (int64_t)gridDim.x * blockDim.x) {
     const float4 gv = g[i];
     float4 r = gv;
-    if (y) {
+    if (y_bits) {
+      const unsigned nib = y_bits[i >> 3] >> (4 * (int)(i & 7));
+      r.x = (nib & 1u) ? gv.x : 0.f;
+      r.y = (nib & 2u) ? gv.y : 0.f;
+      r.z = (nib & 4u) ? gv.z : 0.f;
+      r.w = (nib & 8u) ? gv.w : 0.f;
+    } else if (y) {
       const float4 yv = y[i];
       r.x = yv.x > 0.f ? gv.x : 0.f;
       r.y = yv.y > 0.f ? gv.y : 0.f;
@@ -467,9 +474,27 @@
   return dadet_relu_bn_backward_m(g, y, scale, g_out, g_scaled, rows, C, nullptr, nullptr, stream);
 }
 
+static int relu_bn_backward_launch(const float* g, const float* y, const unsigned* y_bits, const float* scale,
+                                   float* g_out, float* g_scaled, int64_t rows, int C, float* amax_out,
+                                   float* amax_scaled, void* stream);
+
 extern "C" int dadet_relu_bn_backward_m(const float* g, const float* y, const float* scale, float* g_out,
                                         float* g_scaled, int64_t rows, int C, float* amax_out, float* amax_scaled,
                                         void* stream) {
+  return relu_bn_backward_launch(g, y, nullptr, scale, g_out, g_scaled, rows, C, amax_out, amax_scaled, stream);
+}
+
+extern "C" int dadet_relu_bn_backward_bits(const float* g, const unsigned* y_bits, const float* scale, float* g_out,
+                                           float* g_scaled, int64_t rows, int C, float* amax_out, float* amax_scaled,
+                                           void* stream) {
+  DADET_REQUIRE(y_bits && (reinterpret_cast<uintptr_t>(y_bits) & 3) == 0, "relu_bn_backward_bits: null or misaligned plane");
+  DADET_REQUIRE(C > 0 && C % 32 == 0, "relu_bn_backward_bits: C=%d must be a multiple of 32 (whole plane words per row)", C);
+  return relu_bn_backward_launch(g, nullptr, y_bits, scale, g_out, g_scaled, rows, C, amax_out, amax_scaled, stream);
+}
+
+static int relu_bn_backward_launch(const float* g, const float* y, const unsigned* y_bits, const float* scale,
+                                   float* g_out, float* g_scaled, int64_t rows, int C, float* amax_out,
+                                   float* amax_scaled, void* stream) {
   DADET_REQUIRE(rows >= 0 && C > 0 && C % 4 == 0, "relu_bn_backward: C=%d must be a multiple of 4", C);
   if (rows == 0) return DADET_OK;
   DADET_REQUIRE(g && (g_out || g_scaled), "relu_bn_backward: null pointer");
@@ -481,7 +506,7 @@
                      reinterpret_cast<const float4*>(y), reinterpret_cast<const float4*>(scale),
                      reinterpret_cast<float4*>(g_out), reinterpret_cast<float4*>(g_scaled), total4, C / 4,
                      reinterpret_cast<unsigned*>(g_out ? amax_out : nullptr),
-                     reinterpret_cast<unsigned*>(g_scaled ? amax_scaled : nullptr));
+                     reinterpret_cast<unsigned*>(g_scaled ? amax_scaled : nullptr), y_bits);
   return check_launch("relu_bn_backward");
 }
 
diff --git a/da_detect_amd/modeling/backbone/resnet.py b/da_detect_amd/modeling/backbone/resnet.py
--- a/da_detect_amd/modeling/backbone/resnet.py
+++ b/da_detect_amd/modeling/backbone/resnet.py
@@ -70,13 +70,15 @@
 
 class _BlockBackward(object):
 
-    def __init__(self, needs, x, w1, wd, s1, sd, stride):
+    def __init__(self, needs, x, w1, wd, s1, sd, stride, bits=(None, None)):
         self.need_x, self.n1, self.n2, self.n3, nd = needs
         self.nd = nd and wd is not None
         self.x, self.w1, self.wd, self.s1, self.sd, self.stride = x, w1, wd, s1, sd, stride
+        self.x_bits, self.out_bits = bits
 
     def open(self, G, out, out_private, y2, w2, w3, s3):
-        self.S3 = G.contiguous(memory_format=torch.channels_last) if out_private else _C.relu_bn_backward(G, out, None)[1]
+        self.S3 = G.contiguous(memory_format=torch.channels_last) if out_private \
+            else _C.relu_bn_backward(G, out, None, y_bits=self.out_bits)[1]
         self.lane = WgradLane(G.device, rows=G.shape[0] * G.shape[2] * G.shape[3])
         self.batch = _C.WgradBatch() if _WGRAD_BATCH else None
         weights = ((w3, self.n3), (w2, self.n2), (self.w1, self.n1), (self.wd, self.nd))
@@ -107,7 +109,8 @@
             gate = dict(relu_mode=2, mask_ref=x) if in_relu else {}
             hw = tuple(x.shape[2:])
             if wd is None:
-                dx = _C.conv_forward(S1, _C.conv_weight_transpose(w1, s1), addend=S3, **gate)
+                dx = _C.conv_forward(S1, _C.conv_weight_transpose(w1, s1), addend=S3,
+                                     gate_bits=self.x_bits if in_relu else None, **gate)
             elif stride == 1:
                 t = _C.conv_forward(S3, _C.conv_weight_transpose(wd, sd))
                 dx = _C.conv_forward(S1, _C.conv_weight_transpose(w1, s1), addend=t, out=t, **gate)
@@ -122,11 +125,12 @@
 class _BottleneckFn(torch.autograd.Function):
 
     @staticmethod
-    def forward(ctx, x, w1, w2, w3, wd, s1, b1, s2, b2, s3, b3, sd, bd, stride, in_relu, out_private):
+    def forward(ctx, x, w1, w2, w3, wd, s1, b1, s2, b2, s3, b3, sd, bd, stride, in_relu, out_private, want_bits=False):
         y1 = _C.conv_forward(x, w1, s1, b1, stride=stride, relu_mode=1)
         y2 = _C.conv_forward(y1, w2, s2, b2, pad=1, relu_mode=1)
         idn = x if wd is None else _C.conv_forward(x, wd, sd, bd, stride=stride)
-        out = _C.conv_forward(y2, w3, s3, b3, addend=idn, relu_mode=1)
+        out = _C.conv_forward(y2, w3, s3, b3, addend=idn, relu_mode=1, sign_out=want_bits and any(ctx.needs_input_grad[:5]))
+        ctx.bits = (_C.sign_plane(x), _C.sign_plane(out))
         ctx.stride, ctx.in_relu, ctx.out_private = stride, in_relu, out_private
         ctx.save_for_backward(x, y1, y2, out, w1, w2, w3, wd, s1, s2, s3, sd)
         return out
@@ -136,7 +140,7 @@
     def backward(ctx, G):
         x, y1, y2, out, w1, w2, w3, wd, s1, s2, s3, sd = ctx.saved_tensors
         need_x, n1, n2 = ctx.needs_input_grad[:3]
-        b = _BlockBackward(ctx.needs_input_grad[:5], x, w1, wd, s1, sd, ctx.stride)
+        b = _BlockBackward(ctx.needs_input_grad[:5], x, w1, wd, s1, sd, ctx.stride, ctx.bits)
         S2, dw3 = b.open(G, out, ctx.out_private, y2, w2, w3, s3)
         dw2 = S1 = None
         if n2:
@@ -144,14 +148,14 @@
         if n1 or need_x:
             S1 = _C.conv_forward(S2, _C.conv_weight_transpose(w2, s2), pad=1, relu_mode=2, mask_ref=y1)
         dx, dw1, dwd = b.close(S1, ctx.in_relu)
-        return (dx, dw1, dw2, dw3, dwd) + (None,) * 11
+        return (dx, dw1, dw2, dw3, dwd) + (None,) * 12
 
 
 class _DCNBottleneckFn(torch.autograd.Function):
 
     @staticmethod
     def forward(ctx, x, w1, w2, w3, wd, w_off, b_off, s1, b1, s2, b2, s3, b3, sd, bd, stride, in_relu, out_private,
-                modulated, dg):
+                modulated, dg, want_bits=False):
         cout2, cin2, kh, kw = w2.shape
         y1 = _C.conv_forward(x, w1, s1, b1, stride=stride, relu_mode=1)
         wo4, bo4 = _pad_out_channels(w_off, b_off)
@@ -159,7 +163,8 @@
         cols = _C.deform_sample_forward_om(y1, om, kh, kw, 1, kh // 2, 1, dg, modulated)
         y2 = _C.conv_forward(cols, _as_1x1(w2), s2, b2, relu_mode=1)
         idn = x if wd is None else _C.conv_forward(x, wd, sd, bd, stride=stride)
-        out = _C.conv_forward(y2, w3, s3, b3, addend=idn, relu_mode=1)
+        out = _C.conv_forward(y2, w3, s3, b3, addend=idn, relu_mode=1, sign_out=want_bits and any(ctx.needs_input_grad[:5]))
+        ctx.bits = (_C.sign_plane(x), _C.sign_plane(out))
         ctx.conf = (stride, in_relu, out_private, modulated, dg, kh, kw, w_off.shape[0], wo4.shape[0])
         ctx.b_off = b_off
         ctx.save_for_backward(x, y1, om, cols, y2, out, w1, w2, w3, wd, w_off, s1, s2, s3, sd)
@@ -172,7 +177,7 @@
         stride, in_relu, out_private, modulated, dg, kh, kw, n_offch, n_offpad = ctx.conf
         n2, n_off, n_boff = ctx.needs_input_grad[2], ctx.needs_input_grad[5], ctx.needs_input_grad[6]
         cout2, cin2 = w2.shape[0], w2.shape[1]
-        b = _BlockBackward(ctx.needs_input_grad[:5], x, w1, wd, s1, sd, stride)
+        b = _BlockBackward(ctx.needs_input_grad[:5], x, w1, wd, s1, sd, stride, ctx.bits)
         S2, dw3 = b.open(G, out, out_private, y2, w2, w3, s3)
         dw2 = dwo = dbo = None
         w2_1x1 = _as_1x1(w2)
@@ -189,7 +194,7 @@
         dx, dw1, dwd = b.close(S1, in_relu)
         if dw2 is not None:
             dw2 = torch.as_strided(dw2, (cout2, cin2, kh, kw), (kh * kw * cin2, 1, kw * cin2, cin2))
-        return (dx, dw1, dw2, dw3, dwd, dwo, dbo) + (None,) * 13
+        return (dx, dw1, dw2, dw3, dwd, dwo, dbo) + (None,) * 14
 
 
 def _as_1x1(weight):
@@ -307,7 +312,7 @@
                 return _DCNBottleneckFn.apply(x, self.conv1.weight, c2.conv.weight, self.conv3.weight, wd,
                                               c2.offset.weight, c2.offset.bias, *self.bn1.folded(), *self.bn2.folded(),
                                               *self.bn3.folded(), sd, bd, self.conv1.stride[0], in_relu, out_private,
-                                              c2.with_modulated_dcn, c2.conv.deformable_groups)
+                                              c2.with_modulated_dcn, c2.conv.deformable_groups, torch.is_grad_enabled())
             return self._forward_dcn(x)
         if self.conv2.stride[0] == 1:
             if x.shape[0] == 0 and stride is None:
@@ -317,7 +322,8 @@
                 wd, (sd, bd) = self.downsample[0].weight, self.downsample[1].folded()
             return _BottleneckFn.apply(x, self.conv1.weight, self.conv2.weight, self.conv3.weight, wd,
                                        *self.bn1.folded(), *self.bn2.folded(), *self.bn3.folded(), sd, bd,
-                                       self.conv1.stride[0] if stride is None else stride, in_relu, out_private)
+                                       self.conv1.stride[0] if stride is None else stride, in_relu, out_private,
+                                       torch.is_grad_enabled())
         assert stride is None
         return self._forward_per_conv(x)
 
diff --git a/include/dadet.h b/include/dadet.h
--- a/include/dadet.h
+++ b/include/dadet.h
@@ -108,6 +108,11 @@
 int dadet_conv_forward_scaled(const dadet_conv_desc* d, const float* x, const float* w, const float* scale,
                               const float* bias, const float* addend, const float* mask_ref, float* y,
                               const float* amax_x, const float* amax_w, float* amax_y, void* stream);
+
+int dadet_conv_forward_bits(const dadet_conv_desc* d, const float* x, const float* w, const float* scale,
+                            const float* bias, const float* addend, const float* mask_ref, float* y,
+                            const float* amax_x, const float* amax_w, float* amax_y, unsigned* sign_out,
+                            const unsigned* gate_bits, void* stream);
 
 int dadet_conv_forward_variant(const dadet_conv_desc* d);
 
@@ -299,6 +304,8 @@
                            float* g_scaled, int64_t rows, int C, void* stream);
 int dadet_relu_bn_backward_m(const float* g, const float* y, const float* scale, float* g_out, float* g_scaled,
                              int64_t rows, int C, float* amax_out, float* amax_scaled, void* stream);
+int dadet_relu_bn_backward_bits(const float* g, const unsigned* y_bits, const float* scale, float* g_out, float* g_scaled,
+                                int64_t rows, int C, float* amax_out, float* amax_scaled, void* stream);
 int dadet_colsum_workspace_bytes(int64_t rows, int C, size_t* bytes_out);
 int dadet_colsum_ld(const float* g, int ld, float* out, int64_t rows, int C, int accumulate, void* workspace,
                     size_t workspace_bytes, void* stream);
```

Result: no change. 163.0, median of 6 (+0.4%).
